# fzi-forschungszentrum-informatik/muvo

Hardware: AMD Instinct MI355X
Metric: world-model training samples/sec (seq_len=10) (higher is better)
Workload: dtype f32 storage/accumulate; large contractions (convolutions, transformer Linear) as bf16x3 split products

## Files before the change

include/muvo_hip.h:

```cpp
#ifndef MUVO_HIP_H
#define MUVO_HIP_H
#include <stdint.h>

#ifdef __cplusplus
extern "C" {
#endif

#define MUVO_OK 0
#define MUVO_ERR_INVALID_ARG (-1)
#define MUVO_ERR_HIP (-2)

#define MUVO_ACT_NONE 0
#define MUVO_ACT_RELU 1
#define MUVO_ACT_LEAKY 2
#define MUVO_ACT_ELU 3
#define MUVO_ACT_TANH 4
#define MUVO_ACT_SIGMOID 5

const char* muvo_last_error(void);
int muvo_abi_version(void);
int muvo_selftest_mfma(void* stream);
int muvo_set_deterministic(int on);
int muvo_reset_accumulators(void);
int muvo_get_deterministic(void);

typedef struct muvo_conv_desc {
  int32_t nd;
  int32_t transposed;
  int32_t N, Cin, Cout;
  int32_t in_sz[3], out_sz[3];
  int32_t ksz[3], stride[3], pad[3], dil[3];
} muvo_conv_desc;

#define MUVO_CONV_F32 0
#define MUVO_CONV_BF16X3 1
#define MUVO_CONV_MODE_DEFAULT MUVO_CONV_BF16X3
int muvo_conv_set_products(int n);
int muvo_conv_get_products(void);
int muvo_conv_set_mode(int mode);
int muvo_conv_get_mode(void);
int muvo_conv_set_bf16x3_min_gflop(double gflop_per_item);
int muvo_linear_bf16x3_pack_floats(int in_f, int out_f, int64_t* fwd_floats, int64_t* dgrad_floats);
int muvo_linear_bf16x3_pack(int in_f, int out_f, const float* w, float* wp_fwd, float* wp_dgrad, void* stream);
int64_t muvo_linear_bf16x3_workspace_bytes(int64_t rows, int features);
int muvo_linear_bf16x3_split(const float* x, int64_t rows, int features, void* ws, void* stream);
int muvo_linear_bf16x3_forward(int64_t rows, int in_f, int out_f, const void* ws_x, const float* wp_fwd, const float* bias,
                               float* y, int act, float slope, void* stream);
int muvo_linear_bf16x3_dgrad(int64_t rows, int in_f, int out_f, const void* ws_dz, const float* wp_dgrad, float* dx,
                             void* stream);
int muvo_linear_bf16x3_wgrad(int64_t rows, int in_f, int out_f, const void* ws_x, const void* ws_dz, float* scratch,
                             float* dw, void* stream);
int64_t muvo_pack_table_item_bytes(void);
int muvo_conv_pack_table_add(void* host_items, int capacity, int* n_items, int64_t* n_blocks, const muvo_conv_desc* d,
                             const float* w, float* wp_fwd, float* wp_dgrad);
int muvo_linear_bf16x3_pack_table_add(void* host_items, int capacity, int* n_items, int64_t* n_blocks, int in_f, int out_f,
                                      const float* w, float* wp_fwd, float* wp_dgrad);
int muvo_pack_table_run(const void* dev_items, int n_items, int64_t n_blocks, void* stream);
int muvo_conv_pack_sizes(const muvo_conv_desc* d, int64_t* fwd_floats, int64_t* dgrad_floats);
int muvo_conv_pack_weights(const muvo_conv_desc* d, const float* w, float* wp_fwd, float* wp_dgrad, void* stream);
int64_t muvo_conv_workspace_bytes(const muvo_conv_desc* d, int op);
int muvo_conv_kernel_family(const muvo_conv_desc* d, int op);
int muvo_conv_kernel_variant(const muvo_conv_desc* d, int op);
int muvo_conv_forward(const muvo_conv_desc* d, const float* x, const float* wp_fwd, const float* bias, float* y, int act,
                      float slope, void* ws, void* stream);
int muvo_conv_dgrad(const muvo_conv_desc* d, const float* dy, const float* wp_dgrad, float* dx, void* ws, int ws_valid,
                    void* stream);
int muvo_conv_forward_head_supported(const muvo_conv_desc* d, int CO);
int muvo_conv_forward_head(const muvo_conv_desc* d, const float* x, const float* wp_fwd, const float* bias, float* y, int act,
                           float slope, void* ws, const float* head_w, const float* head_b, int CO, float* logits, void* stream);
int muvo_conv_forward_moments_supported(const muvo_conv_desc* d);
int muvo_conv_forward_moments(const muvo_conv_desc* d, const float* x, const float* wp_fwd, const float* bias, float* y, int act,
                              float slope, double* moments, void* stream);
int muvo_adain_fwd_moments(const float* x, const float* style, float* y, float* save_mean, float* save_rstd, double* moments,
                           int N, int C, int64_t S, float eps, void* stream);
int muvo_adain_affine(const float* style, double* moments, float* save_mean, float* save_rstd, float* aff, int N, int C, int64_t S,
                      float eps, void* stream);
int muvo_conv_affine_supported(const muvo_conv_desc* d);
int muvo_conv_forward_affine(const muvo_conv_desc* d, const float* x, const float* aff, const float* wp_fwd, const float* bias,
                             float* y, int act, float slope, double* moments, void* stream);
int muvo_conv_wgrad_affine(const muvo_conv_desc* d, const float* x, const float* aff, const float* dy, float* dw, float* dbias,
                           void* stream);
int muvo_grouped_linear_fwd(const float* x, int M, int K, int L, const float* const* W, const float* const* b, float* const* Y,
                            const int* N, void* stream);
int muvo_grouped_linear_bwd(const float* x, int M, int K, int L, const float* const* W, float* const* dY, float* dx,
                            float* const* dW, float* const* db, const int* N, void* stream);
int muvo_bf3_loop_clock(double* shader_mhz, double* us_per_k_step);
int muvo_adain_head_supported(int C, int CO, int64_t S);
int muvo_adain_head_fwd(const float* x, const float* style, float* save_mean, float* save_rstd, double* moments, const float* head_w,
                        const float* head_b, float* logits, int N, int C, int CO, int64_t S, float eps, void* stream);
int muvo_adain_head_bwd(const float* x, const float* style, const float* save_mean, const float* save_rstd, const float* head_w,
                        const float* dlogits, float* dx, float* dstyle, float* dhead_w, float* dhead_b, double* ws, int N, int C,
                        int CO, int64_t S, int act, float slope, void* stream);
int muvo_conv_dgrad_accumulate(const muvo_conv_desc* d, const float* dy, const float* wp_dgrad, float* dx, void* stream);
int muvo_conv_prepare_dy(const muvo_conv_desc* d, const float* y, const float* dy, int act, float slope, void* ws_dy,
                         float* dbias, void* stream);
int muvo_conv_prepare_dy_head_supported(const muvo_conv_desc* d, int CO);
int muvo_conv_prepare_dy_head(const muvo_conv_desc* d, const float* y, const float* dy, const float* dhead, const float* head_w,
                              int CO, int act, float slope, void* ws_dy, float* dbias, float* dhead_w, float* dhead_b, void* stream);
int64_t muvo_split_planes_bytes(int N, int C, int64_t S);
int muvo_split_planes(const float* x, void* ws, int N, int C, int64_t S, const float* y, int act, float slope, float* dbias,
                      void* stream);
int muvo_conv_wgrad(const muvo_conv_desc* d, const float* x, const float* dy, float* dwp_scratch, float* dw, float* dbias,
                    void* ws_x, void* ws_dy, int flags, void* stream);

int muvo_bias_grad_nchw(const float* dy, float* db, int N, int M, int64_t S, void* stream);

typedef struct muvo_gemm_desc {
  int32_t M, N, K;
  int64_t sam, sak, sbk, sbn, scm;
  int32_t B1, B2;
  int64_t a_b1, a_b2, b_b1, b_b2, c_b1, c_b2;
  float alpha;
  int32_t bias_div;
  int32_t act;
  float slope;
  int32_t mode;
} muvo_gemm_desc;
int muvo_gemm(const muvo_gemm_desc* d, const float* A, const float* B, float* C, const float* bias, void* stream);

int muvo_bn_train_fwd(const float* x, const float* gamma, const float* beta, const float* residual, float* y,
                      float* save_mean, float* save_rstd, float* running_mean, float* running_var, double* ws, int N, int C,
                      int64_t S, float eps, float momentum, int res_mode, int relu, void* stream);
int muvo_bn_train_bwd(const float* x, const float* y, const float* dy, const float* gamma, const float* beta,
                      const float* save_mean, const float* save_rstd, float* dx, float* dres, float* dgamma, float* dbeta,
                      double* ws, int N, int C, int64_t S, int mask_mode, void* stream);
int muvo_adain_fwd(const float* x, const float* style, float* y, float* save_mean, float* save_rstd, double* ws, int N,
                   int C, int64_t S, int64_t x_batch_stride, float eps, void* stream);
int muvo_adain_bwd(const float* x, const float* style, const float* dy, const float* save_mean, const float* save_rstd,
                   float* dx, float* dstyle, double* ws, int N, int C, int64_t S, int64_t x_batch_stride, int act,
                   float slope, void* stream);
int muvo_add_dropout_layernorm_fwd(const float* x, const float* a, const float* gamma, const float* beta, float* y,
                                   float* z, float* mean, float* rstd, int rows, int E, float eps, float p, uint64_t seed,
                                   void* stream);
int muvo_add_dropout_layernorm_bwd(const float* dy, const float* z, const float* mean, const float* rstd,
                                   const float* gamma, float* dx, float* da, float* dgamma, float* dbeta, int rows, int E,
                                   float p, uint64_t seed, void* stream);

int muvo_act_fwd(const float* x, float* y, int64_t n, int act, float slope, void* stream);
int muvo_act_bwd(const float* y, const float* dy, float* dx, int64_t n, int act, float slope, void* stream);
int muvo_dropout(const float* x, float* y, int64_t n, float p, uint64_t seed, void* stream);
int muvo_axpby(const float* a, const float* b, float* out, int64_t n, float alpha, float beta, void* stream);
int muvo_copy2d(const float* src, float* dst, int64_t rows, int64_t cols, int64_t ld_src, int64_t ld_dst, int accumulate,
                void* stream);
int muvo_colsum_acc(const float* x, float* out, int64_t rows, int64_t cols, int64_t ld, void* stream);
int muvo_batchsum(const float* x, float* out, int N, int64_t inner, int accumulate, void* stream);
int muvo_nchw_to_tokens(const float* x, const float* pos, const float* temb, int temb_stride, float* tokens, int N, int C,
                        int L, int l0, void* stream);
int muvo_tokens_to_nchw(const float* tokens, float* x, int N, int C, int L, int l0, void* stream);
int muvo_maxpool2d_fwd(const float* x, float* y, uint8_t* idx, int64_t NC, int H, int W, int OH, int OW, int k, int s, int p,
                       void* stream);
int muvo_maxpool2d_bwd(const float* dy, const uint8_t* idx, float* dx, int64_t NC, int H, int W, int OH, int OW, int k, int s,
                       int p, void* stream);
int muvo_avgpool_fwd(const float* x, float* y, int64_t G, int64_t S, void* stream);
int muvo_avgpool_bwd(const float* dy, float* dx, int64_t G, int64_t S, void* stream);
int muvo_upsample3d_x2_fwd(const float* x, float* y, int64_t NC, int D, int H, int W, void* stream);
int muvo_upsample3d_x2_bwd(const float* dy, float* dx, int64_t NC, int D, int H, int W, void* stream);
int muvo_preprocess_image(const uint8_t* img, float* label, float* norm, int64_t NC, int C, int H, int W, int top, int left,
                          int CH, int CW, const float* mean3, const float* std3, void* stream);
int muvo_preprocess_route(const uint8_t* img, float* norm, int64_t NC, int C, int H, int W, int OH, int OW,
                          const float* mean3, const float* std3, void* stream);
int muvo_attention_supported(int L, int DH);
int muvo_attention_fwd(const float* qkv, float* out, float* lse, int L, int N, int H, int DH, float p, uint64_t seed,
                       void* stream);
int muvo_attention_bwd(const float* qkv, const float* out, const float* dout, const float* lse, float* dqkv, int L, int N, int H,
                       int DH, float p, uint64_t seed, void* stream);
int muvo_attention_stream_supported(int L, int DH);
int muvo_attention_stream_blocks(int* bq, int* bk);
int muvo_attention_stream_fwd(const float* qkv, float* out, float* lse, int L, int N, int H, int DH, float p, uint64_t seed,
                              void* stream);
int muvo_attention_stream_bwd(const float* qkv, const float* out, const float* dout, const float* lse, float* dqkv, float* dws,
                              int L, int N, int H, int DH, float p, uint64_t seed, void* stream);
int muvo_rssm_supported(int B, int T, int H, int S, int E, int A, int AD);
int64_t muvo_rssm_transposed_floats(int H, int S, int E, int A);
int64_t muvo_rssm_scratch_floats(int B, int H, int S, int E, int A);
int muvo_rssm_forward(int B, int T, int H, int S, int E, int A, int AD, const float* const* weights, const float* emb,
                      const float* act, const float* noise, uint64_t use_prior_mask, float* const* out7, float* const* keep12,
                      uint32_t* barrier_word, float min_std, void* stream);
int muvo_rssm_backward(int B, int T, int H, int S, int E, int A, int AD, const float* const* weights, float* wt_scratch,
                       const float* noise, uint64_t use_prior_mask, const float* const* kept5, const float* const* upstream7,
                       float* const* grads10, float* scratch, uint32_t* barrier_word, void* stream);
#define MUVO_PIXAUG_STRIDE 16
#define MUVO_ROUTEAUG_STRIDE 8
int muvo_pixel_augment(float* img, float* norm, float* tmp, const float* params, double* gray_sum, int64_t frames, int H, int W,
                       const float* mean3, const float* std3, void* stream);
int muvo_preprocess_route_aug(const uint8_t* img, float* out, const float* params, int B, int S, int C, int H, int W, int OH,
                              int OW, const float* mean3, const float* std3, void* stream);
int muvo_divide_scalar(const float* x, float* y, int64_t n, float divisor, void* stream);
int muvo_resize_bilinear(const float* x, float* y, int64_t NC, int H, int W, int OH, int OW, void* stream);
int muvo_resize_nearest_f32(const float* x, float* y, int64_t NC, int D, int H, int W, int OD, int OH, int OW, void* stream);
int muvo_resize_nearest_u8(const uint8_t* x, uint8_t* y, int64_t NC, int D, int H, int W, int OD, int OH, int OW,
                           void* stream);
int muvo_softmax_dropout_fwd(const float* S, float* P, float* Pd, int64_t rows, int cols, float p, uint64_t seed, void* stream);
int muvo_softmax_dropout_bwd(const float* P, const float* dPd, float* dS, int64_t rows, int cols, float p, uint64_t seed,
                             void* stream);
int muvo_gru_fwd(const float* gi, const float* gh, const float* h, float* hnew, int B, int H, void* stream);
int muvo_gru_bwd(const float* gi, const float* gh, const float* h, const float* dhnew, float* dgi, float* dgh, float* dh,
                 int B, int H, void* stream);
int muvo_rssm_sample_fwd(const float* mu_logsigma, const float* eps, int64_t eps_ld, float* mu, float* sigma, float* sample,
                         int B, int S, float min_std, void* stream);
int muvo_rssm_sample_bwd(const float* mu_logsigma, const float* eps, int64_t eps_ld, const float* dmu, const float* dsigma,
                         const float* dsample, float* dmls, int B, int S, void* stream);

int muvo_spatial_loss_fwd(const float* pred, const float* target, int64_t F, int Ct, int64_t HW, int c0, int c1, int norm,
                          float ignore, float weight, double* stats2, float* loss, void* stream);
int muvo_spatial_loss_bwd(const float* pred, const float* target, float* dpred, int64_t F, int Ct, int64_t HW, int c0, int c1,
                          int norm, float ignore, float weight, const double* stats2, const float* gout, void* stream);
int muvo_spatial_loss_masked_fwd(const float* pred, const float* target, const uint8_t* mask, int64_t F, int Ct, int64_t HW, int c0,
                                 int c1, int norm, float ignore, float weight, double* stats2, float* loss, void* stream);
int muvo_spatial_loss_masked_bwd(const float* pred, const float* target, const uint8_t* mask, float* dpred, int64_t F, int Ct,
                                 int64_t HW, int c0, int c1, int norm, float ignore, float weight, const double* stats2,
                                 const float* gout, void* stream);
int muvo_voxel_loss_stats_doubles(int C);
int muvo_voxel_loss_coef_floats(int C);
int muvo_voxel_loss_fwd(const float* logits, const uint8_t* target, int64_t F, int C, int64_t V, const float* class_w,
                        float weight, double* stats, float* coef, float* loss3, void* stream);
int muvo_voxel_loss_bwd(const float* logits, const uint8_t* target, float* dlogits, int64_t F, int C, int64_t V,
                        const float* class_w, float weight, const float* coef, const float* gout3, void* stream);
int muvo_seg_ce_fwd(const float* logits, const uint8_t* target, const float* class_w, float* loss, int64_t N, int C, int64_t HW,
                    void* stream);
int muvo_seg_ce_bwd(const float* logits, const uint8_t* target, const float* class_w, const float* gloss, float* dlogits, int64_t N,
                    int C, int64_t HW, void* stream);
int muvo_l1_rows_fwd(const float* p, const float* t, int64_t rows, int cols, float weight, float* loss, void* stream);
int muvo_l1_rows_bwd(const float* p, const float* t, float* dp, int64_t rows, int cols, float weight, const float* gout,
                     void* stream);
int muvo_kl_loss_fwd(const float* prior_mu, const float* prior_sigma, const float* post_mu, const float* post_sigma, int B,
                     int T, int S, float weight, float* loss, void* stream);
int muvo_kl_loss_bwd(const float* prior_mu, const float* prior_sigma, const float* post_mu, const float* post_sigma,
                     float* d_prior_mu, float* d_prior_sigma, float* d_post_mu, float* d_post_sigma, int B, int T, int S,
                     float weight, float alpha, const float* gout, void* stream);
int muvo_adamw_step(float* p, const float* g, float* m, float* v, int64_t n, float lr, float beta1, float beta2, float eps,
                    float weight_decay, int step, float grad_scale, void* stream);

int64_t muvo_chamfer_loss_ws_doubles(int64_t F, int64_t n);
int muvo_chamfer_loss_fwd(const float* pred, const float* target, int64_t F, int Cp, int Ct, int64_t n, float weight, double* ws,
                          int32_t* idx_pt, int32_t* idx_tp, float* loss, void* stream);
int muvo_chamfer_loss_bwd(const float* pred, const float* target, const int32_t* idx_pt, const int32_t* idx_tp, float* dpred, int64_t F,
                          int Cp, int Ct, int64_t n, float weight, const float* gout, void* stream);

int muvo_ssim_frames(const float* pred, const float* target, const float* window, double* sums, int N, int C, int H, int W,
// ... 149 lines not shown
```

muvo_amd/csrc/conv_gemm.hip:

```cpp
#include "common.h"
#include "conv_vox.h"
#include "conv_pw.h"
#include "conv_plan.h"
#include "conv_bf3.h"

typedef __bf16 wg_bf16x8 __attribute__((ext_vector_type(8)));
__device__ __forceinline__ void wg_split8(const float (&v)[8], wg_bf16x8& hi, wg_bf16x8& lo) {
  typedef __bf16 b2 __attribute__((ext_vector_type(2)));
  typedef float f2 __attribute__((ext_vector_type(2)));
  unsigned h[4], l[4];
#pragma unroll
  for (int p = 0; p < 4; ++p) {
    const b2 hh = __builtin_convertvector((f2){v[2 * p], v[2 * p + 1]}, b2);
    h[p] = __builtin_bit_cast(unsigned, hh);
    const float h0 = __uint_as_float(h[p] << 16), h1 = __uint_as_float(h[p] & 0xffff0000u);
    const b2 ll = __builtin_convertvector((f2){v[2 * p] - h0, v[2 * p + 1] - h1}, b2);
    l[p] = __builtin_bit_cast(unsigned, ll);
  }
  typedef unsigned u4 __attribute__((ext_vector_type(4)));
  hi = __builtin_bit_cast(wg_bf16x8, (u4){h[0], h[1], h[2], h[3]});
  lo = __builtin_bit_cast(wg_bf16x8, (u4){l[0], l[1], l[2], l[3]});
}

template <int BM, int BN, int WM, int WN, int RUN>
// ... 894 lines not shown
  if (rc) return rc;
  MUVO_CHECK_ARG(wp_fwd && y && ws, "conv_forward_planes: null pointer");
  MUVO_CHECK_ARG(!pw_applicable(d) && !vox_fwd_ok(d), "conv_forward_planes: this shape does not read split planes");
  bool all_bf3 = pl.nfwd > 0;
  for (int i = 0; i < pl.nfwd; ++i) all_bf3 = all_bf3 && pl.fwd[i].bf3;
  MUVO_CHECK_ARG(all_bf3, "conv_forward_planes: ws_valid needs every phase on the bf16x3 kernels (muvo_conv_kernel_family == 1)");
  return run_phases(pl.fwd, pl.nfwd, x, wp_fwd, bias, y, act, slope, ws, (hipStream_t)stream, true);
}

int muvo_conv_forward_head_supported(const muvo_conv_desc* d, int CO) {
  if (check_desc(d) || CO < 1 || CO > 4) return 0;
  static const int on = getenv("MUVO_CONV_HEAD_FWD") ? atoi(getenv("MUVO_CONV_HEAD_FWD")) : 1;
  if (!on || muvo_det() || conv_mode() != 1 || pw_applicable(d) || vox_fwd_ok(d)) return 0;
  ConvPlan pl;
  if (build_plan(d, &pl) != MUVO_OK || pl.nfwd < 1) return 0;
  for (int i = 0; i < pl.nfwd; ++i) {
    const ConvPhase& g = pl.fwd[i];
    if (!g.bf3 || !bf3_fwd_uses_pp(g) || phase_ksplit(g) > 1) return 0;
    if (g.Msub != d->Cout || g.Msub % 64 != 0 || g.M % 64 != 0 || (long)CO * g.Msub > 1024) return 0;
    if ((long)g.N * g.out_sN * 4 >= 0x7fffff00L) return 0;
  }
  return 1;
}
int muvo_conv_forward_head(const muvo_conv_desc* d, const float* x, const float* wp_fwd, const float* bias, float* y, int act,
                           float slope, void* ws, const float* head_w, const float* head_b, int CO, float* logits, void* stream) {
  ConvPlan pl;
  int rc = build_plan(d, &pl);
  if (rc) return rc;
  MUVO_CHECK_ARG(x && wp_fwd && y && head_w && logits, "conv_forward_head: null pointer");
  MUVO_CHECK_ARG(muvo_conv_forward_head_supported(d, CO), "conv_forward_head: shape not served by the eight-wave bf16x3 tiles");
  hipStream_t st = (hipStream_t)stream;
  if (d->Cout > 64) {
    const long S_out = (long)d->out_sz[0] * d->out_sz[1] * d->out_sz[2];
    if (hipMemsetAsync(logits, 0, sizeof(float) * (size_t)d->N * CO * S_out, st) != hipSuccess) {
      muvo_set_error("conv_forward_head: memset of the logits failed");
      return MUVO_ERR_HIP;
    }
  }
  bf3_set_fused_head(head_w, head_b, logits, CO);
  rc = run_phases(pl.fwd, pl.nfwd, x, wp_fwd, bias, y, act, slope, ws, st);
  bf3_set_fused_head(nullptr, nullptr, nullptr, 0);
  return rc;
}

int muvo_conv_forward_moments_supported(const muvo_conv_desc* d) {
  if (check_desc(d)) return 0;
  if (muvo_det()) return 0;
  return (!pw_applicable(d) && vox_fwd_ok(d) && vox_uses_bf3(d, 0)) ? 1 : 0;
}
int muvo_conv_forward_moments(const muvo_conv_desc* d, const float* x, const float* wp_fwd, const float* bias, float* y, int act,
                              float slope, double* moments, void* stream) {
  ConvPlan pl;
  int rc = build_plan(d, &pl);
  if (rc) return rc;
  MUVO_CHECK_ARG(x && wp_fwd && y && moments, "conv_forward_moments: null pointer");
  MUVO_CHECK_ARG(muvo_conv_forward_moments_supported(d), "conv_forward_moments: only the bf16x3 voxel kernels produce output moments");
  return vox_forward(d, x, wp_fwd, bias, y, act, slope, (hipStream_t)stream, true, moments);
}

int muvo_conv_affine_supported(const muvo_conv_desc* d) {
  if (check_desc(d)) return 0;
  return (conv_mode() == 1 && !pw_applicable(d) && vox_fwd_ok(d) && vox_uses_bf3(d, 0) && vox_wgrad_applicable(d) &&
          vox_wgrad_uses_bf3(d) && vox_affine_ok(d)) ? 1 : 0;
}
int muvo_conv_forward_affine(const muvo_conv_desc* d, const float* x, const float* aff, const float* wp_fwd, const float* bias,
                             float* y, int act, float slope, double* moments, void* stream) {
  ConvPlan pl;
  int rc = build_plan(d, &pl);
  if (rc) return rc;
  MUVO_CHECK_ARG(x && aff && wp_fwd && y, "conv_forward_affine: null pointer");
  MUVO_CHECK_ARG(muvo_conv_affine_supported(d), "conv_forward_affine: shape not served by the bf16x3 voxel kernels");
  return vox_forward(d, x, wp_fwd, bias, y, act, slope, (hipStream_t)stream, true, moments, aff);
}
int muvo_conv_wgrad_affine(const muvo_conv_desc* d, const float* x, const float* aff, const float* dy, float* dw, float* dbias,
                           void* stream) {
  ConvPlan pl;
  int rc = build_plan(d, &pl, 0, false);
  if (rc) return rc;
  MUVO_CHECK_ARG(x && aff && dy && dw, "conv_wgrad_affine: null pointer");
  MUVO_CHECK_ARG(muvo_conv_affine_supported(d), "conv_wgrad_affine: shape not served by the bf16x3 voxel kernels");
  return vox_wgrad(d, x, dy, dw, dbias, (hipStream_t)stream, true, aff);
}

int muvo_conv_dgrad(const muvo_conv_desc* d, const float* dy, const float* wp_dgrad, float* dx, void* ws, int ws_valid,
                    void* stream) {
  ConvPlan pl;
  int rc = build_plan(d, &pl);
  if (rc) return rc;
  MUVO_CHECK_ARG(dy && wp_dgrad && dx, "conv_dgrad: null pointer");
  if (pw_applicable(d)) return pw_dgrad(d, dy, wp_dgrad, dx, (hipStream_t)stream);
  if (vox_dgrad_ok(d)) return vox_dgrad(d, dy, wp_dgrad, dx, (hipStream_t)stream, vox_uses_bf3(d, 1));
  return run_phases(pl.dgr, pl.ndgr, dy, wp_dgrad, nullptr, dx, MUVO_ACT_NONE, 0.f, ws, (hipStream_t)stream, ws_valid != 0);
}

int muvo_conv_dgrad_accumulate(const muvo_conv_desc* d, const float* dy, const float* wp_dgrad, float* dx, void* stream) {
  int rc = check_desc(d);
  if (rc) return rc;
  MUVO_CHECK_ARG(dy && wp_dgrad && dx, "conv_dgrad_accumulate: null pointer");
  MUVO_CHECK_ARG(pw_applicable(d), "conv_dgrad_accumulate: only the 1x1 head kernels (muvo_conv_kernel_family == 3) accumulate");
  return pw_dgrad_acc(d, dy, wp_dgrad, dx, (hipStream_t)stream);
}

int muvo_conv_prepare_dy(const muvo_conv_desc* d, const float* y, const float* dy, int act, float slope, void* ws_dy,
                         float* dbias, void* stream) {
  int rc = check_desc(d);
  if (rc) return rc;
  MUVO_CHECK_ARG(dy && ws_dy && (y || act == MUVO_ACT_NONE), "conv_prepare_dy: null pointer");
  const long S_out = (long)d->out_sz[0] * d->out_sz[1] * d->out_sz[2];
  return bf3_split_input(dy, ws_dy, d->N, d->Cout, S_out, (hipStream_t)stream, act == MUVO_ACT_NONE ? nullptr : y, act, slope,
                         dbias);
}

int muvo_conv_prepare_dy_head(const muvo_conv_desc* d, const float* y, const float* dy, const float* dhead, const float* head_w,
                              int CO, int act, float slope, void* ws_dy, float* dbias, float* dhead_w, float* dhead_b, void* stream) {
  int rc = check_desc(d);
  if (rc) return rc;
  MUVO_CHECK_ARG(dhead && head_w && ws_dy && CO >= 1 && CO <= 4 && (y || act == MUVO_ACT_NONE), "conv_prepare_dy_head: bad args");
  const long S_out = (long)d->out_sz[0] * d->out_sz[1] * d->out_sz[2];
  MUVO_CHECK_ARG(dhead_w == nullptr || (y != nullptr && act != MUVO_ACT_NONE),
                 "conv_prepare_dy_head: the fused head weight gradient needs the activation output y");
  return bf3_split_input(dy, ws_dy, d->N, d->Cout, S_out, (hipStream_t)stream, act == MUVO_ACT_NONE ? nullptr : y, act, slope,
                         dbias, dhead, head_w, CO, dhead_w, dhead_b);
}
int muvo_conv_prepare_dy_head_supported(const muvo_conv_desc* d, int CO) {
  if (check_desc(d)) return 0;
  const long S_out = (long)d->out_sz[0] * d->out_sz[1] * d->out_sz[2];
  return CO >= 1 && CO <= 4 && S_out % 4 == 0 && S_out >= 1024;
}

static double bf3_wgrad_min_gflop() {
  static const char* e = getenv("MUVO_BF16X3_WGRAD_MIN_GFLOP");
  static const double env_v = e ? atof(e) : -1.0;
  if (env_v >= 0.0) return env_v;
  if (bf3_default_policy()) return 0.05;
  return bf3_min_gflop() < 0.5 ? bf3_min_gflop() : 0.5;
}

static const int g_bf3_wgrad_min_m = getenv("MUVO_BF3_WGRAD_MIN_M") ? atoi(getenv("MUVO_BF3_WGRAD_MIN_M")) : 32;
static bool wgrad_uses_bf3(const ConvPlan& pf) {
  if (conv_mode() != 1) return false;
  const bool dflt = bf3_default_policy() && !getenv("MUVO_BF16X3_WGRAD_MIN_GFLOP");
  double total = 0.0;
  int taps = 0;
  for (int i = 0; i < pf.nfwd; ++i) {
    const ConvPhase& g = pf.fwd[i];
    const double gflop = 2.0 * g.Msub * g.T * g.C * (double)g.SD * g.SH * g.SW * 1e-9;
    if (g.Msub < g_bf3_wgrad_min_m || g.C < 32 || g.Msub % 16 != 0 && g.nmerge > 1) return false;
    static const int allow32 = getenv("MUVO_BF3_WGRAD_32X32") ? atoi(getenv("MUVO_BF3_WGRAD_32X32")) : 1;
    if (g.Msub <= 32 && g.C < 64 && !allow32) return false;
    if (!dflt && gflop < bf3_wgrad_min_gflop()) return false;
    total += gflop * g.nmerge;
    taps += g.T * g.nmerge;
  }
  if (dflt && (total < bf3_wgrad_min_gflop() || taps <= 1)) return false;
  return pf.nfwd > 0;
}

int muvo_conv_wgrad(const muvo_conv_desc* d, const float* x, const float* dy, float* dwp_scratch, float* dw, float* dbias,
                    void* ws_x, void* ws_dy, int flags, void* stream) {
  ConvPlan pl;
  int rc = build_plan(d, &pl, 0, false);
  if (rc) return rc;
  MUVO_CHECK_ARG(x && dy && dwp_scratch && dw, "conv_wgrad: null pointer");
  hipStream_t st = (hipStream_t)stream;
  if (pw_applicable(d)) return pw_wgrad(d, x, dy, dw, dbias, st);
  if (vox_wgrad_ok(d)) return vox_wgrad(d, x, dy, dw, dbias, st, vox_wgrad_uses_bf3(d));
// ... 202 lines not shown
```

muvo_amd/csrc/conv_vox.h:

```cpp
#pragma once
#include "common.h"

bool vox_fwd_applicable(const muvo_conv_desc* d);
bool vox_dgrad_applicable(const muvo_conv_desc* d);
bool vox_wgrad_applicable(const muvo_conv_desc* d);
long vox_pack_floats(const muvo_conv_desc* d);
bool vox_bf3_shape_ok(const muvo_conv_desc* d, int dgrad);
int vox_pack(const muvo_conv_desc* d, const float* w, float* wp, int dgrad, hipStream_t st, bool bf3);
int vox_forward(const muvo_conv_desc* d, const float* x, const float* wp, const float* bias, float* y, int act, float slope,
                hipStream_t st, bool bf3, double* moments = nullptr, const float* aff = nullptr);
bool vox_affine_ok(const muvo_conv_desc* d);
int vox_dgrad(const muvo_conv_desc* d, const float* dy, const float* wp, float* dx, hipStream_t st, bool bf3);
bool vox_bf3_wgrad_shape_ok(const muvo_conv_desc* d);
bool vox_wgrad_ps_only(const muvo_conv_desc* d);
int vox_wgrad(const muvo_conv_desc* d, const float* x, const float* dz, float* dw, float* dbias, hipStream_t st, bool bf3,
              const float* aff = nullptr);
```

muvo_amd/csrc/conv_vox.hip:

```cpp
#include "common.h"
#include "conv_vox.h"
#include <type_traits>

struct VoxArgs {
  int N, Cin, Cout, X, Y;
  int ytiles, xgroups;
  int XYZ;
  long sN_in, sN_out;
  double* moments;
  int xcd_order;
  const float* aff;
  unsigned* ticket;
};
static int vox_xcd_order() {
  static const int v = getenv("MUVO_VOX_XCD") ? atoi(getenv("MUVO_VOX_XCD")) : 1;
  return v;
}

__device__ __forceinline__ float dpp_wave_shr1(float v) {
  return __int_as_float(__builtin_amdgcn_update_dpp(0, __float_as_int(v), 0x138, 0xf, 0xf, true));
}
__device__ __forceinline__ float dpp_wave_shl1(float v) {
  return __int_as_float(__builtin_amdgcn_update_dpp(0, __float_as_int(v), 0x130, 0xf, 0xf, true));
}

template <int CQ, int TY, int Z>
__global__ void __launch_bounds__(256)
vox_conv_kernel(const VoxArgs a, const float* __restrict__ in, const float* __restrict__ wp,
                const float* __restrict__ bias, float* __restrict__ out, int act, float slope) {
  extern __shared__ __attribute__((aligned(16))) float s_w[];
  constexpr int SUB = 64 / Z;
  constexpr int R = TY + 2;
  const int tid = threadIdx.x, lane = tid & 63, wave = tid >> 6;
  {
    const int nw4 = 27 * a.Cin * a.Cout / 4;
    for (int i = tid; i < nw4; i += 256) ((float4*)s_w)[i] = ((const float4*)wp)[i];
  }
  __syncthreads();
  const long wid = (long)blockIdx.x * 4 + wave;
  const long nwaves = (long)a.N * a.xgroups * a.ytiles;
  if (wid >= nwaves) return;
  const int yt = (int)(wid % a.ytiles);
  const long t0 = wid / a.ytiles;
  const int xg = (int)(t0 % a.xgroups), n = (int)(t0 / a.xgroups);
  const int sub = lane / Z, z = lane % Z;
  const int x = xg * SUB + sub;
  const int y0 = yt * TY;
  const bool xok = x < a.X;
  const int YZ = a.Y * Z;
  const float* inn = in + (size_t)n * a.sN_in;

  f32x4 acc[TY][CQ];
#pragma unroll
  for (int g = 0; g < TY; ++g)
#pragma unroll
    for (int q = 0; q < CQ; ++q) acc[g][q] = (f32x4){0.f, 0.f, 0.f, 0.f};

  auto load_rows = [&](int it, float* v) {
    const int ci = it / 3, tx = it - 3 * ci;
    const int xin = x + tx - 1;
    const bool ok = xok && (unsigned)xin < (unsigned)a.X;
    const float* p = inn + (size_t)ci * a.XYZ;
    const int off = xin * YZ + z;
#pragma unroll
    for (int r = 0; r < R; ++r) {
      const int y = y0 - 1 + r;
      float val = 0.f;
      if (ok && (unsigned)y < (unsigned)a.Y) val = p[off + y * Z];
      v[r] = val;
    }
  };

  const int total = 3 * a.Cin;
  const int wl = (lane & 3) * CQ;
  const int wstride = a.Cin * 4 * CQ;
  float cur[R], nxt[R];
  load_rows(0, cur);
  for (int it = 0; it < total; ++it) {
    const int ci = it / 3, tx = it - 3 * ci;
    if (it + 1 < total) load_rows(it + 1, nxt);
    float lf[R], rt[R];
#pragma unroll
    for (int r = 0; r < R; ++r) {
      const float l = dpp_wave_shr1(cur[r]), rr = dpp_wave_shl1(cur[r]);
      lf[r] = z > 0 ? l : 0.f;
      rt[r] = z < Z - 1 ? rr : 0.f;
    }
    const float* wb = s_w + (size_t)(tx * 9 * a.Cin + ci) * 4 * CQ + wl;
#pragma unroll
    for (int ty = 0; ty < 3; ++ty) {
#pragma unroll
      for (int tz = 0; tz < 3; ++tz) {
        const float* wq = wb + (ty * 3 + tz) * wstride;
        float w[CQ];
        if constexpr (CQ == 2) {
          const float2 t = *(const float2*)wq;
// ... 328 lines not shown
  float msum[4] = {0.f, 0.f, 0.f, 0.f}, msq[4] = {0.f, 0.f, 0.f, 0.f};
  float bv[4];
#pragma unroll
  for (int i = 0; i < 4; ++i) bv[i] = (bias != nullptr && co0 + 4 * g + i < a.Cout) ? bias[co0 + 4 * g + i] : 0.f;
  const __amdgpu_buffer_rsrc_t rs_out = __builtin_amdgcn_make_buffer_rsrc((void*)(out + (long)n * a.sN_out), 0,
                                                                          (int)((long)a.Cout * a.XYZ * 4), 0x00020000);

  int fdx[NSTEP], foff[NSTEP];
#pragma unroll
  for (int s = 0; s < NSTEP; ++s) {
    int tap = s * TPS + g;
    if (tap > 26) tap = 26;
    const int dx = tap / 9 - 1, dy = (tap / 3) % 3 - 1, dz = tap % 3 - 1;
    fdx[s] = dx;
    foff[s] = (wave + 1 + dy) * COLS + (v + 1 + dz);
  }

  stage_load(xs - 1); stage_store((xs - 1 + 3) % 3);
  stage_load(xs); stage_store(xs % 3);
  stage_load(xs + 1);
  vox_dummy_stores<4 * ZT>(rs_out);
  __syncthreads();
  for (int x = xs; x < xe; ++x) {
    stage_store((x + 1) % 3);
    __syncthreads();
    if (x + 1 < xe) stage_load(x + 2);
    const vu32x4* P[3] = {vsm + ((x - 1 + 3) % 3) * PLANE, vsm + (x % 3) * PLANE, vsm + ((x + 1) % 3) * PLANE};
    const vu32x4* fb[NSTEP];
#pragma unroll
    for (int s = 0; s < NSTEP; ++s) fb[s] = (fdx[s] < 0 ? P[0] : (fdx[s] == 0 ? P[1] : P[2])) + foff[s];
    const int gy = y0 + wave;
#pragma unroll
    for (int zt = 0; zt < ZT; ++zt) {
      vf32x4 acc = {0.f, 0.f, 0.f, 0.f};
#pragma unroll
      for (int s = 0; s < NSTEP; ++s) {
        const vbf16x8 bh = __builtin_bit_cast(vbf16x8, fb[s][zt * 16]);
        const vbf16x8 bl = __builtin_bit_cast(vbf16x8, fb[s][zt * 16 + CG * ROWS * COLS]);
        acc = __builtin_amdgcn_mfma_f32_16x16x32_bf16(wl[s], bh, acc, 0, 0, 0);
        acc = __builtin_amdgcn_mfma_f32_16x16x32_bf16(wh[s], bl, acc, 0, 0, 0);
        acc = __builtin_amdgcn_mfma_f32_16x16x32_bf16(wh[s], bh, acc, 0, 0, 0);
      }
      const unsigned ooff = (unsigned)(((long)x * YZ + (long)gy * Z + zt * 16 + v) * 4);
#pragma unroll
      for (int i = 0; i < 4; ++i) {
        const int co = co0 + 4 * g + i;
        const bool ok = gy < a.Y && co < a.Cout;
        const unsigned off = ok ? ooff + (unsigned)co * xyz4 : 0x7fffff00u;
        float r = acc[i] + bv[i];
        if constexpr (GENERIC) {
          if (accum) r += __uint_as_float(__builtin_amdgcn_raw_buffer_load_b32(rs_out, off, 0, 0));
          r = act_apply(r, act, slope);
        } else {
          r = vox_act_simple(r, act, slope);
        }
        __builtin_amdgcn_raw_buffer_store_b32(__float_as_uint(r), rs_out, off, 0, 0);
        r = ok ? r : 0.f;
        msum[i] += r;
        msq[i] += r * r;
      }
    }
    __syncthreads();
  }
  if (a.moments) {
#pragma unroll
    for (int i = 0; i < 4; ++i)
#pragma unroll
      for (int o = 1; o < 16; o <<= 1) { msum[i] += __shfl_xor(msum[i], o, 64); msq[i] += __shfl_xor(msq[i], o, 64); }
    float* red = (float*)vsm;
    if (v == 0)
#pragma unroll
      for (int i = 0; i < 4; ++i) { red[((wave * 4 + g) * 4 + i) * 2] = msum[i]; red[((wave * 4 + g) * 4 + i) * 2 + 1] = msq[i]; }
    __syncthreads();
    if (tid < 32) {
      const int c = tid >> 1, k = tid & 1;
      double t = 0.0;
      for (int w = 0; w < TY; ++w) t += (double)red[((w * 4 + (c >> 2)) * 4 + (c & 3)) * 2 + k];
      if (co0 + c < a.Cout) atomicAdd(&a.moments[((long)n * a.Cout + co0 + c) * 2 + k], t);
    }
  }
}

constexpr int VOX_PS_TY = 8;
template <int Z, int TY, bool CO8, bool GENERIC>
__global__ void __launch_bounds__(64 * TY, 1)
vox_bf3_ps_kernel(const VoxArgs a, const float* __restrict__ in, const vu32x4* __restrict__ wp, const float* __restrict__ bias,
                  float* __restrict__ out, int act, float slope, int xseg, int accum) {
  static_assert(TY == VOX_PS_TY, "one workgroup of eight waves per CU");
  constexpr int CK = 16, CG = 2, PSTEPS = 5, ZT = Z / 16, NF = CO8 ? 2 * PSTEPS : 3 * PSTEPS, NACC = CO8 ? 2 : 3;
  constexpr int ROWS = TY + 2, COLS = Z + 2;
  constexpr int PLANE = 2 * CG * ROWS * COLS;
  constexpr int NTASK = CG * ROWS * Z, TPT = (NTASK + 64 * TY - 1) / (64 * TY);
  extern __shared__ vu32x4 vsm[];
  const int tid = threadIdx.x, lane = tid & 63, wave = tid >> 6;
  const int nseg = (a.X + xseg - 1) / xseg;
  int bid = a.xcd_order ? xcd_swizzle(blockIdx.x, gridDim.x) : (int)blockIdx.x;
  const int seg = bid % nseg; bid /= nseg;
  const int ytile = bid % a.ytiles, n = bid / a.ytiles;
  const int y0 = ytile * TY, xs = seg * xseg, xe = xs + xseg < a.X ? xs + xseg : a.X;
  const long YZ = (long)a.Y * Z;
  const float* inb = in + (long)n * a.sN_in;
  const int co0 = blockIdx.y * 16;

  vbf16x8 wh[NF], wl[NF];
  const vu32x4* wpb = wp + (size_t)blockIdx.y * NF * 2 * 64;
#pragma unroll
  for (int f = 0; f < NF; ++f) {
    wh[f] = __builtin_bit_cast(vbf16x8, wpb[(f * 2) * 64 + lane]);
    wl[f] = __builtin_bit_cast(vbf16x8, wpb[(f * 2 + 1) * 64 + lane]);
  }
  for (int i = tid; i < 2 * PLANE; i += 64 * TY) vsm[i] = vu32x4{0u, 0u, 0u, 0u};
  __syncthreads();

  float stg[TPT][8];
  unsigned stg_ok = 0u;
  __shared__ float s_aff[2 * CK];
  if (a.aff) {
    if (tid < 2 * CK) s_aff[tid] = a.aff[(long)n * a.Cin * 2 + tid];
    __syncthreads();
  }
  const __amdgpu_buffer_rsrc_t rs_in = __builtin_amdgcn_make_buffer_rsrc((void*)inb, 0, (int)((long)CK * a.XYZ * 4), 0x00020000);
  const unsigned xyz4 = (unsigned)a.XYZ * 4u;
  auto stage_load_task = [&](int k, int x) {
    const int t = tid + k * 64 * TY;
    const int z = t % Z, r = (t / Z) % ROWS, cg = t / (Z * ROWS);
    const int gy = y0 - 1 + r;
    const bool ok = t < NTASK && x >= 0 && x < a.X && gy >= 0 && gy < a.Y;
    stg_ok = (stg_ok & ~(1u << k)) | ((unsigned)ok << k);
    const unsigned off = ok ? (unsigned)(((long)(cg * 8) * a.XYZ + (long)x * YZ + (long)gy * Z + z) * 4) : 0x7fffff00u;
#pragma unroll
    for (int e = 0; e < 8; ++e)
      stg[k][e] = __uint_as_float(__builtin_amdgcn_raw_buffer_load_b32(rs_in, off + (unsigned)e * xyz4, 0, 0));
  };
  auto stage_load = [&](int x) {
#pragma unroll
    for (int k = 0; k < TPT; ++k) stage_load_task(k, x);
  };
  auto stage_store_task = [&](int k, int slot) {
    vu32x4* P = vsm + slot * PLANE;
    {
      const int t = tid + k * 64 * TY;
      if (t >= NTASK) return;
      const int z = t % Z, r = (t / Z) % ROWS, cg = t / (Z * ROWS);
      if (a.aff) {
        const bool ok = (stg_ok >> k) & 1u;
#pragma unroll
        for (int e = 0; e < 8; ++e) {
          const float sc = s_aff[(cg * 8 + e) * 2], sh = s_aff[(cg * 8 + e) * 2 + 1];
          stg[k][e] = ok ? stg[k][e] * sc + sh : 0.f;
        }
      }
      unsigned h[4], l[4];
#pragma unroll
      for (int q = 0; q < 4; ++q) vox_split2(stg[k][2 * q], stg[k][2 * q + 1], h[q], l[q]);
      P[(cg * ROWS + r) * COLS + z + 1] = vu32x4{h[0], h[1], h[2], h[3]};
      P[((CG + cg) * ROWS + r) * COLS + z + 1] = vu32x4{l[0], l[1], l[2], l[3]};
    }
  };
  auto stage_store = [&](int slot) {
#pragma unroll
    for (int k = 0; k < TPT; ++k) stage_store_task(k, slot);
  };

  const int v = lane & 15, g = lane >> 4;
  float msum[4] = {0.f, 0.f, 0.f, 0.f}, msq[4] = {0.f, 0.f, 0.f, 0.f};
  float bv[4];
#pragma unroll
  for (int i = 0; i < 4; ++i) bv[i] = (bias != nullptr && co0 + 4 * g + i < a.Cout) ? bias[co0 + 4 * g + i] : 0.f;
  const __amdgpu_buffer_rsrc_t rs_out = __builtin_amdgcn_make_buffer_rsrc((void*)(out + (long)n * a.sN_out), 0,
                                                                          (int)((long)a.Cout * a.XYZ * 4), 0x00020000);
  int foff[PSTEPS];
#pragma unroll
  for (int s = 0; s < PSTEPS; ++s) {
    int tp = s * 2 + (g >> 1);
    if (tp > 8) tp = 8;
    const int dy = tp / 3 - 1, dz = tp % 3 - 1;
    foff[s] = ((g & 1) * ROWS + (wave + 1 + dy)) * COLS + (v + 1 + dz);
  }
  vf32x4 acc[NACC][ZT];
#pragma unroll
  for (int j = 0; j < NACC; ++j)
#pragma unroll
    for (int zt = 0; zt < ZT; ++zt) acc[j][zt] = vf32x4{0.f, 0.f, 0.f, 0.f};

  stage_load(xs - 1); stage_store((xs - 1) & 1);
  stage_load(xs);
  vox_dummy_stores<4 * ZT>(rs_out);
  __syncthreads();
  const int gy = y0 + wave;
  for (int p = xs - 1; p <= xe; ++p) {
    constexpr bool ACC_PRE = GENERIC && (CO8 || Z <= 32);
    float accv[ZT][4];
    if constexpr (ACC_PRE) {
      if (accum) {
        const int xo = p - 1;
        const bool xok = xo >= xs && xo < xe;
#pragma unroll
        for (int zt = 0; zt < ZT; ++zt) {
          const unsigned ooff = (unsigned)(((long)xo * YZ + (long)gy * Z + zt * 16 + v) * 4);
#pragma unroll
          for (int i = 0; i < 4; ++i) {
            const int co = co0 + 4 * g + i;
            const bool ok = xok && gy < a.Y && co < a.Cout && (!CO8 || g < 2);
            accv[zt][i] = __uint_as_float(__builtin_amdgcn_raw_buffer_load_b32(rs_out, ok ? ooff + (unsigned)co * xyz4 : 0x7fffff00u, 0, 0));
          }
        }
      }
    }
    constexpr bool PIPE = CO8 || Z <= 32;
    if constexpr (!PIPE) {
      stage_store((p + 1) & 1);
      if (p + 2 <= xe) stage_load(p + 2);
    }
    const vu32x4* P = vsm + (p & 1) * PLANE;
#pragma unroll
    for (int zt = 0; zt < ZT; ++zt) {
#pragma unroll
      for (int s = 0; s < PSTEPS; ++s) {
        const vbf16x8 bh = __builtin_bit_cast(vbf16x8, P[foff[s] + zt * 16]);
        const vbf16x8 bl = __builtin_bit_cast(vbf16x8, P[foff[s] + zt * 16 + CG * ROWS * COLS]);
        if constexpr (CO8) {
          acc[1][zt] = __builtin_amdgcn_mfma_f32_16x16x32_bf16(wl[s], bh, acc[1][zt], 0, 0, 0);
          acc[1][zt] = __builtin_amdgcn_mfma_f32_16x16x32_bf16(wh[s], bl, acc[1][zt], 0, 0, 0);
          acc[1][zt] = __builtin_amdgcn_mfma_f32_16x16x32_bf16(wh[s], bh, acc[1][zt], 0, 0, 0);
          acc[0][zt] = __builtin_amdgcn_mfma_f32_16x16x32_bf16(wl[PSTEPS + s], bh, acc[0][zt], 0, 0, 0);
          acc[0][zt] = __builtin_amdgcn_mfma_f32_16x16x32_bf16(wh[PSTEPS + s], bl, acc[0][zt], 0, 0, 0);
          acc[0][zt] = __builtin_amdgcn_mfma_f32_16x16x32_bf16(wh[PSTEPS + s], bh, acc[0][zt], 0, 0, 0);
        } else {
#pragma unroll
          for (int dxi = 0; dxi < 3; ++dxi) {
            const int f = dxi * PSTEPS + s, j = 2 - dxi;
            acc[j][zt] = __builtin_amdgcn_mfma_f32_16x16x32_bf16(wl[f], bh, acc[j][zt], 0, 0, 0);
            acc[j][zt] = __builtin_amdgcn_mfma_f32_16x16x32_bf16(wh[f], bl, acc[j][zt], 0, 0, 0);
            acc[j][zt] = __builtin_amdgcn_mfma_f32_16x16x32_bf16(wh[f], bh, acc[j][zt], 0, 0, 0);
          }
        }
      }
      if constexpr (PIPE) {
#pragma unroll
        for (int k = 0; k < TPT; ++k)
          if ((k < ZT ? k : ZT - 1) == zt) {
            stage_store_task(k, (p + 1) & 1);
            if (p + 2 <= xe) stage_load_task(k, p + 2);
          }
        __builtin_amdgcn_sched_barrier(0);
      }
    }
    const int xo = p - 1;
    const bool xok = xo >= xs && xo < xe;
#pragma unroll
    for (int zt = 0; zt < ZT; ++zt) {
      const unsigned ooff = (unsigned)(((long)xo * YZ + (long)gy * Z + zt * 16 + v) * 4);
#pragma unroll
      for (int i = 0; i < 4; ++i) {
        const int co = co0 + 4 * g + i;
        const bool ok = xok && gy < a.Y && co < a.Cout && (!CO8 || g < 2);
        const unsigned off = ok ? ooff + (unsigned)co * xyz4 : 0x7fffff00u;
        float r = acc[0][zt][i] + bv[i];
        if constexpr (GENERIC) {
          if constexpr (ACC_PRE) { if (accum) r += accv[zt][i]; }
          else if (accum) r += __uint_as_float(__builtin_amdgcn_raw_buffer_load_b32(rs_out, off, 0, 0));
          r = act_apply(r, act, slope);
        } else {
          r = vox_act_simple(r, act, slope);
        }
        __builtin_amdgcn_raw_buffer_store_b32(__float_as_uint(r), rs_out, off, 0, 0);
        r = ok ? r : 0.f;
        msum[i] += r;
// ... 157 lines not shown
  const int row = wave / ZH, z0 = (wave % ZH) * 32;
  const int j = lane & 15, kg = lane >> 4;
  const int a_off = j * DCO + row * DROW + (z0 + kg * 8) * 2;
  const int b_off = (j & (CI - 1)) * XCI + 16 + (z0 + kg * 8) * 2;
  const int sel = j >> 3;

  xload(xs - 1); xstore((xs - 1 + 4) & 3);
  xload(xs); xstore(xs & 3);
  xload(xs + 1); xstore((xs + 1) & 3);
  dload(xs); dstore(xs & 1);
  xload(xs + 2);
  dload(xs + 1);
  __syncthreads();
  for (int px = xs; px < xe; ++px) {
    const char* A = dzb + (px & 1) * DBUF + a_off;
    const vbf16x8 ah = __builtin_bit_cast(vbf16x8, *(const vu32x4*)A);
    const vbf16x8 al = __builtin_bit_cast(vbf16x8, *(const vu32x4*)(A + DHL));
#pragma unroll
    for (int cb = 0; cb < NCOMB; ++cb) {
      int c = 2 * cb + sel;
      if (c > 8) c = 8;
      const int dx = c / 3, dy = c - 3 * dx;
      const char* R = xring + ((px + dx - 1 + 4) & 3) * XSLOT + b_off + (row + dy) * XROW;
      vu32x4 w[2];
      unsigned pw[2], nw[2];
#pragma unroll
      for (int hl = 0; hl < 2; ++hl) {
        w[hl] = *(const vu32x4*)(R + hl * XHL);
        pw[hl] = *(const unsigned*)(R + hl * XHL - 4);
        nw[hl] = *(const unsigned*)(R + hl * XHL + 16);
      }
      vbf16x8 bm[2], bz[2], bp[2];
#pragma unroll
      for (int hl = 0; hl < 2; ++hl) {
        const vu32x4 q = w[hl];
        bz[hl] = __builtin_bit_cast(vbf16x8, q);
        const vu32x4 m = {__builtin_amdgcn_alignbyte(q.x, pw[hl], 2), __builtin_amdgcn_alignbyte(q.y, q.x, 2),
                          __builtin_amdgcn_alignbyte(q.z, q.y, 2), __builtin_amdgcn_alignbyte(q.w, q.z, 2)};
        bm[hl] = __builtin_bit_cast(vbf16x8, m);
        const vu32x4 pl = {__builtin_amdgcn_alignbyte(q.y, q.x, 2), __builtin_amdgcn_alignbyte(q.z, q.y, 2),
                           __builtin_amdgcn_alignbyte(q.w, q.z, 2), __builtin_amdgcn_alignbyte(nw[hl], q.w, 2)};
        bp[hl] = __builtin_bit_cast(vbf16x8, pl);
      }
      const int t0 = cb * TPC;
      acc[t0] = __builtin_amdgcn_mfma_f32_16x16x32_bf16(al, bm[0], acc[t0], 0, 0, 0);
      acc[t0] = __builtin_amdgcn_mfma_f32_16x16x32_bf16(ah, bm[1], acc[t0], 0, 0, 0);
      acc[t0] = __builtin_amdgcn_mfma_f32_16x16x32_bf16(ah, bm[0], acc[t0], 0, 0, 0);
      acc[t0 + 1] = __builtin_amdgcn_mfma_f32_16x16x32_bf16(al, bz[0], acc[t0 + 1], 0, 0, 0);
      acc[t0 + 1] = __builtin_amdgcn_mfma_f32_16x16x32_bf16(ah, bz[1], acc[t0 + 1], 0, 0, 0);
      acc[t0 + 1] = __builtin_amdgcn_mfma_f32_16x16x32_bf16(ah, bz[0], acc[t0 + 1], 0, 0, 0);
      acc[t0 + 2] = __builtin_amdgcn_mfma_f32_16x16x32_bf16(al, bp[0], acc[t0 + 2], 0, 0, 0);
      acc[t0 + 2] = __builtin_amdgcn_mfma_f32_16x16x32_bf16(ah, bp[1], acc[t0 + 2], 0, 0, 0);
      acc[t0 + 2] = __builtin_amdgcn_mfma_f32_16x16x32_bf16(ah, bp[0], acc[t0 + 2], 0, 0, 0);
      static_assert(XPT + DPT + 1 <= NCOMB, "one staging piece per combination");
      if (cb < XPT) xstore_task(cb, (px + 2) & 3);
      else if (cb < XPT + DPT) dstore_task(cb - XPT, (px + 1) & 1);
      else if (cb == XPT + DPT) { xload(px + 3); dload(px + 2); }
      __builtin_amdgcn_sched_barrier(0);
    }
    __syncthreads();
  }
  float* red = (float*)wsm;
  for (int i = tid; i < NT * 256; i += 512) red[i] = 0.f;
  __syncthreads();
#pragma unroll
  for (int t = 0; t < NT; ++t)
#pragma unroll
    for (int r = 0; r < 4; ++r) atomicAdd(red + (t * 16 + 4 * kg + r) * 16 + j, acc[t][r]);
  __syncthreads();
  for (int i = tid; i < NT * 256; i += 512) {
    const int col = i & 15, t = i >> 8;
    const int co = (i >> 4) & 15;
    const int tz = t % TPC;
    const int comb = 2 * (t / TPC) + (col >> 3);
    const int ci = col & 7;
    const int tap = comb <= 8 && tz >= 0 ? comb * 3 + tz : -1;
    const float vsum = red[i];
    if (tap >= 0 && co < a.Cout && ci0 + ci < a.Cin && vsum != 0.f) atomicAdd(dw + ((long)co * a.Cin + ci0 + ci) * 27 + tap, vsum);
  }
  if (blockIdx.y == 0 && dbias && tid < a.Cout) atomicAdd(dbias + tid, dbsum[tid]);
}

constexpr int VOX_WGPS_SW = 4;
template <int Z, int CI, bool CO8, int SW = 0>
__global__ void __launch_bounds__(512 + 64 * SW)
vox_bf3_wgrad_ps_kernel(const VoxArgs a, const float* __restrict__ x, const float* __restrict__ dz, float* __restrict__ dw,
                        float* __restrict__ dbias, int xseg) {
  static_assert(CI == 16 || CO8, "8 input channels: the quadrant tiles hold 8 produced channels");
  constexpr bool QUAD = CI == 8;
  constexpr int ZH = Z >= 32 ? Z / 32 : 1, RW = Z >= 32 ? 1 : 32 / Z, WROWS = 8 / ZH * RW, ROWS = WROWS + 2;
  constexpr int XROW = (Z + 16) * 2;
  constexpr int XCI = ROWS * XROW + 16;
  constexpr int XHL = CI * XCI, XSLOT = 2 * XHL;
  constexpr int NTH = 512 + 64 * SW, NS = SW > 0 ? 64 * SW : 512;
  constexpr int XT = CI * ROWS * (Z / 8), XPT = (XT + NS - 1) / NS;
  constexpr int TPC = QUAD ? 1 : (CO8 ? 2 : 3), NT = 9 * TPC;
  static_assert(SW > 0 || XPT <= 2, "staging pieces: one per dy group, then the loads");
  static_assert(2 * XSLOT >= NT * 1024, "the reduction reuses the x planes");
  extern __shared__ char wsm[];
  char* xring = wsm;
  float* dbsum = (float*)(wsm + 2 * XSLOT);
  const int tid = threadIdx.x, lane = tid & 63, wave = tid >> 6;
  const bool stager = SW > 0 && wave >= 8;
  const int stid = SW > 0 ? tid - 512 : tid;
  const int nseg = (a.X + xseg - 1) / xseg;
  int bid = a.xcd_order ? xcd_swizzle(blockIdx.x, gridDim.x) : (int)blockIdx.x;
  const int seg = bid % nseg; bid /= nseg;
  const int ytile = bid % a.ytiles, n = bid / a.ytiles;
  const int y0 = ytile * WROWS, xs = seg * xseg, xe = xs + xseg < a.X ? xs + xseg : a.X;
  const int ci0 = blockIdx.y * CI;
  const long YZ = (long)a.Y * Z;
  const float* xb = x + (long)n * a.sN_in + (long)ci0 * a.XYZ;
  const int co_base = blockIdx.z * 16;
  const float* db = dz + (long)n * a.sN_out;
  for (int i = tid; i < (2 * XSLOT + 64) / 16; i += NTH) ((uint4*)wsm)[i] = uint4{0u, 0u, 0u, 0u};
  __syncthreads();

  constexpr unsigned OOB = 0x7fffff00u;
  const int nci = a.Cin - ci0 < CI ? a.Cin - ci0 : CI;
  const __amdgpu_buffer_rsrc_t rs_x = __builtin_amdgcn_make_buffer_rsrc((void*)xb, 0, (int)((long)nci * a.XYZ * 4), 0x00020000);
  const __amdgpu_buffer_rsrc_t rs_d = __builtin_amdgcn_make_buffer_rsrc((void*)db, 0, (int)((long)a.Cout * a.XYZ * 4), 0x00020000);
  vu32x4 xraw[XPT][2];
  unsigned xok = 0u;
  float xas[XPT], xab[XPT];
  int xlds[XPT];
  long xg[XPT];
  bool xrow_ok[XPT];
#pragma unroll
  for (int k = 0; k < XPT; ++k) {
    const int t = stid >= 0 ? stid + k * NS : XT;
    const int z8 = t % (Z / 8), rr = (t / (Z / 8)) % ROWS, ci = t / ((Z / 8) * ROWS);
    const int gy = y0 - 1 + rr;
    const bool have = a.aff != nullptr && t < XT && ci0 + ci < a.Cin;
    xas[k] = have ? a.aff[((long)n * a.Cin + ci0 + ci) * 2] : 1.f;
    xab[k] = have ? a.aff[((long)n * a.Cin + ci0 + ci) * 2 + 1] : 0.f;
    xlds[k] = t < XT ? ci * XCI + rr * XROW + 16 + z8 * 16 : -1;
    xrow_ok[k] = t < XT && gy >= 0 && gy < a.Y;
    xg[k] = (long)ci * a.XYZ + (long)gy * Z + z8 * 8;
  }
  auto xload_task = [&](int k, int px) {
    const bool ok = xrow_ok[k] && px >= 0 && px < a.X;
    xok = (xok & ~(1u << k)) | ((unsigned)ok << k);
    const unsigned off = ok ? (unsigned)((xg[k] + (long)px * YZ) * 4) : OOB;
    xraw[k][0] = __builtin_amdgcn_raw_buffer_load_b128(rs_x, off, 0, 0);
    xraw[k][1] = __builtin_amdgcn_raw_buffer_load_b128(rs_x, off + 16u, 0, 0);
  };
  auto xload = [&](int px) {
#pragma unroll
    for (int k = 0; k < XPT; ++k) xload_task(k, px);
  };
  auto split8 = [&](const float (&v)[8], vu32x4& h, vu32x4& l) {
    unsigned hh[4], ll[4];
#pragma unroll
    for (int q = 0; q < 4; ++q) vox_split2(v[2 * q], v[2 * q + 1], hh[q], ll[q]);
    h = vu32x4{hh[0], hh[1], hh[2], hh[3]};
    l = vu32x4{ll[0], ll[1], ll[2], ll[3]};
  };
  auto xstore_task = [&](int k, int slot) {
    if (xlds[k] < 0) return;
    float v[8] = {__uint_as_float(xraw[k][0].x), __uint_as_float(xraw[k][0].y), __uint_as_float(xraw[k][0].z), __uint_as_float(xraw[k][0].w),
                  __uint_as_float(xraw[k][1].x), __uint_as_float(xraw[k][1].y), __uint_as_float(xraw[k][1].z), __uint_as_float(xraw[k][1].w)};
    if (a.aff) {
      const bool ok = (xok >> k) & 1u;
#pragma unroll
      for (int e = 0; e < 8; ++e) v[e] = ok ? v[e] * xas[k] + xab[k] : 0.f;
    }
    vu32x4 h, l;
    split8(v, h, l);
    char* dst = xring + slot * XSLOT + xlds[k];
    *(vu32x4*)dst = h;
    *(vu32x4*)(dst + XHL) = l;
  };

  const int j = lane & 15, kg = lane >> 4;
  const int row = (wave / ZH) * RW + (Z >= 32 ? 0 : kg / (Z / 8));
  const int zl = Z >= 32 ? (wave % ZH) * 32 + kg * 8 : (kg % (Z / 8)) * 8;
  const int aco = co_base + (CO8 ? (j & 7) : j);
  const bool a_shift = CO8 && j >= 8;
  const bool a_last = zl + 8 >= Z;
  const bool a_ok = y0 + row < a.Y && aco < a.Cout;
  const long a_g = (long)aco * a.XYZ + (long)(y0 + row) * Z + zl;
  vu32x4 araw[2];
  unsigned anext = 0u;
  auto aload = [&](int px) {
    const bool ok = a_ok && px >= xs && px < xe;
    const unsigned off = ok ? (unsigned)((a_g + (long)px * YZ) * 4) : OOB;
    araw[0] = __builtin_amdgcn_raw_buffer_load_b128(rs_d, off, 0, 0);
    araw[1] = __builtin_amdgcn_raw_buffer_load_b128(rs_d, off + 16u, 0, 0);
    if constexpr (CO8) anext = __builtin_amdgcn_raw_buffer_load_b32(rs_d, ok && !a_last ? off + 32u : OOB, 0, 0);
  };
  float dbacc = 0.f;
  auto asplit = [&](vu32x4& h, vu32x4& l) {
    float v[8] = {__uint_as_float(araw[0].x), __uint_as_float(araw[0].y), __uint_as_float(araw[0].z), __uint_as_float(araw[0].w),
                  __uint_as_float(araw[1].x), __uint_as_float(araw[1].y), __uint_as_float(araw[1].z), __uint_as_float(araw[1].w)};
    dbacc += ((v[0] + v[1]) + (v[2] + v[3])) + ((v[4] + v[5]) + (v[6] + v[7]));
    if constexpr (CO8) {
      const float nx = __uint_as_float(anext);
#pragma unroll
      for (int e = 0; e < 7; ++e) v[e] = a_shift ? v[e + 1] : v[e];
      v[7] = a_shift ? nx : v[7];
    }
    split8(v, h, l);
  };

  vf32x4 acc[NT];
#pragma unroll
  for (int t = 0; t < NT; ++t) acc[t] = vf32x4{0.f, 0.f, 0.f, 0.f};
  const int b_off = (j & (CI - 1)) * XCI + 16 + zl * 2;
  const bool b_shift = QUAD && j >= 8;
  vu32x4 Ah[3] = {}, Al[3] = {};

  const int niter = xe - xs + 2;
  if (stager) {
    xload(xs - 1);
#pragma unroll
    for (int k = 0; k < XPT; ++k) xstore_task(k, 0);
    xload(xs);
    __syncthreads();
    for (int it = 0; it < niter; ++it) {
      if (it + 1 < niter) {
#pragma unroll
        for (int k = 0; k < XPT; ++k) xstore_task(k, (it + 1) & 1);
        if (it + 2 < niter) xload(xs + 1 + it);
      }
      __syncthreads();
    }
  } else {
  if (SW == 0) {
    xload(xs - 1);
#pragma unroll
    for (int k = 0; k < XPT; ++k) xstore_task(k, 0);
    xload(xs);
  }
  aload(xs);
  __syncthreads();
  for (int it = 0; it < niter; ++it) {
    const int P = xs - 1 + it;
    Ah[2] = Ah[1]; Al[2] = Al[1]; Ah[1] = Ah[0]; Al[1] = Al[0];
    asplit(Ah[0], Al[0]);
    aload(P + 2);
    const bool xin = P >= 0 && P < a.X;
    const bool dok[3] = {it < niter - 2, it >= 1 && it < niter - 1, it >= 2};
    const char* S = xring + (it & 1) * XSLOT + b_off + row * XROW;
#pragma unroll
    for (int dy = 0; dy < 3; ++dy) {
      if (xin) {
        const char* R = S + dy * XROW;
        vbf16x8 bm[2], bz[2], bp[2];
// ... 302 lines not shown
      else { dxi = 2; live = live && (lane & 15) < 8; }
    } else {
      dxi = f / 5;
    }
    const int tap = dxi * 9 + tp;
    float val = 0.f;
    if (live && m < rows) val = dgrad ? w[((size_t)c * Cin + m) * 27 + (26 - tap)] : w[((size_t)m * Cin + c) * 27 + tap];
    unsigned hu, lu;
    vox_split_rne(val, hu, lu);
    wp[((size_t)(((half * nrb + rb) * NF + f) * 2) * 64 + lane) * 8 + e] = (unsigned short)hu;
    wp[((size_t)(((half * nrb + rb) * NF + f) * 2 + 1) * 64 + lane) * 8 + e] = (unsigned short)lu;
  }
}

static bool vox_geometry_ok(const muvo_conv_desc* d, bool z16 = false) {
  if (d->nd != 3 || d->transposed) return false;
  for (int a = 0; a < 3; ++a)
    if (d->ksz[a] != 3 || d->stride[a] != 1 || d->pad[a] != 1 || d->dil[a] != 1) return false;
  const int Z = d->in_sz[2];
  if (Z != 64 && Z != 32 && !(z16 && Z == 16)) return false;
  if (d->Cin % 4 || d->Cout % 4) return false;
  if ((long)d->in_sz[0] * d->in_sz[1] * Z * (long)(d->Cin > d->Cout ? d->Cin : d->Cout) * 4 >= 0x7fffff00l) return false;
  return true;
}
bool vox_fwd_applicable(const muvo_conv_desc* d) {
  return vox_geometry_ok(d) && (d->Cout == 8 || d->Cout == 16) && 27l * d->Cin * d->Cout * 4 <= 64 * 1024;
}
bool vox_dgrad_applicable(const muvo_conv_desc* d) {
  return vox_geometry_ok(d) && (d->Cin == 8 || d->Cin == 16) && 27l * d->Cin * d->Cout * 4 <= 64 * 1024;
}
bool vox_wgrad_applicable(const muvo_conv_desc* d) {
  return vox_geometry_ok(d) && d->Cout % 8 == 0 && d->Cin % 8 == 0 && d->Cout <= 32 && d->Cin <= 64;
}
static bool vox_bf3_two_rows(int ck, int cp) { return cp == 8 && ck == 8; }
static bool vox_bf3_ps(int red, int cp) { return (red == 16 || red == 32 || red == 64) && (cp == 8 || cp == 16 || cp == 32); }
bool vox_bf3_shape_ok(const muvo_conv_desc* d, int dgrad) {
  const int ck = dgrad ? d->Cout : d->Cin, cp = dgrad ? d->Cin : d->Cout;
  if (vox_geometry_ok(d, true) && (d->in_sz[2] == 16 || ck == 64)) return vox_bf3_ps(ck, cp);
  if (!vox_geometry_ok(d)) return false;
  return (ck == 8 || ck == 16 || ck == 32) && (cp == 8 || cp == 16 || cp == 32);
}
constexpr int VOX_BF3_STEPS = 7;
long vox_pack_floats(const muvo_conv_desc* d) {
  const int blocks_f = (d->Cin / 16 > 0 ? d->Cin / 16 : 1) * cdiv(d->Cout, 16), blocks_d = (d->Cout / 16 > 0 ? d->Cout / 16 : 1) * cdiv(d->Cin, 16);
  const int blocks = blocks_f > blocks_d ? blocks_f : blocks_d;
  const long plain = 27l * d->Cin * d->Cout, bf3 = 15l * 2 * 64 * 4 * (blocks > 4 ? blocks : 4);
  return plain > bf3 ? plain : bf3;
}

int vox_pack(const muvo_conv_desc* d, const float* w, float* wp, int dgrad, hipStream_t st, bool bf3) {
  const int red = dgrad ? d->Cout : d->Cin, cp = dgrad ? d->Cin : d->Cout;
  if (bf3 && vox_bf3_ps(red, cp)) {
    const int co8 = cp <= 8 ? 1 : 0;
    hipLaunchKernelGGL(vox_bf3_ps_pack_kernel, dim3(cdiv((red / 16) * cdiv(cp, 16) * (co8 ? 10 : 15) * 512, 256)), dim3(256), 0, st, w,
                       (unsigned short*)wp, d->Cin, d->Cout, dgrad, co8);
    MUVO_CHECK_LAUNCH("vox_bf3_ps_pack_kernel");
    return MUVO_OK;
  }
  if (bf3 && vox_bf3_two_rows(red, cp)) {
    hipLaunchKernelGGL(vox_bf3_pack2_kernel, dim3(36), dim3(256), 0, st, w, (unsigned short*)wp, d->Cin, d->Cout, dgrad);
    MUVO_CHECK_LAUNCH("vox_bf3_pack2_kernel");
    return MUVO_OK;
  }
  if (bf3) {
    MUVO_CHECK_ARG(red == 8, "vox_pack: no bf16x3 voxel kernel for %d reduction / %d produced channels", red, cp);
    hipLaunchKernelGGL(vox_bf3_pack_kernel, dim3(cdiv(cdiv(cp, 16) * VOX_BF3_STEPS * 512, 256)), dim3(256), 0, st, w, (unsigned short*)wp,
                       d->Cin, d->Cout, dgrad, 8, VOX_BF3_STEPS);
    MUVO_CHECK_LAUNCH("vox_bf3_pack_kernel");
    return MUVO_OK;
  }
  const int total = 27 * d->Cin * d->Cout;
  hipLaunchKernelGGL(vox_pack_kernel, dim3(cdiv(total, 256)), dim3(256), 0, st, w, wp, d->Cin, d->Cout, dgrad);
  MUVO_CHECK_LAUNCH("vox_pack_kernel");
  return MUVO_OK;
}

static VoxArgs vox_args(const muvo_conv_desc* d, int Cin, int Cout, int rows, int Z, int cin_total, const float* aff) {
  VoxArgs a{};
  a.xcd_order = vox_xcd_order();
  a.aff = aff;
  a.N = d->N; a.Cin = Cin; a.Cout = Cout; a.X = d->in_sz[0]; a.Y = d->in_sz[1];
  a.ytiles = cdiv(a.Y, rows);
  a.XYZ = a.X * a.Y * Z;
  a.sN_in = (long)(cin_total ? cin_total : Cin) * a.XYZ; a.sN_out = (long)Cout * a.XYZ;
  return a;
}

static int vox_blocks_target(int wgrad) {
  static const int f = getenv("MUVO_VOX_BLOCKS") ? atoi(getenv("MUVO_VOX_BLOCKS")) : 128;
  static const int w = getenv("MUVO_VOX_WGRAD_BLOCKS") ? atoi(getenv("MUVO_VOX_WGRAD_BLOCKS")) : 128;
  return wgrad ? w : f;
}
static int vox_xseg(const VoxArgs& a, int factor, int wgrad) {
  int xseg = a.X;
  while ((long)a.N * a.ytiles * cdiv(a.X, xseg) * factor < vox_blocks_target(wgrad) && xseg > 12) xseg = cdiv(xseg, 2);
  return xseg;
}

template <class... K>
static int vox_raise_lds(bool& done, const char* what, size_t lds, K... kernels) {
  if (done) return MUVO_OK;
  if (((hipFuncSetAttribute((const void*)kernels, hipFuncAttributeMaxDynamicSharedMemorySize, (int)lds) != hipSuccess) || ...)) {
    muvo_set_error("%s: cannot raise the dynamic LDS limit to %zu bytes", what, lds);
    return MUVO_ERR_HIP;
  }
  done = true;
  return MUVO_OK;
}

template <bool Z16 = false, class F>
static int vox_with_z(int Z, F&& f) {
  if (Z == 64) return f(std::integral_constant<int, 64>{});
  if (Z == 32) return f(std::integral_constant<int, 32>{});
  if constexpr (Z16) {
    if (Z == 16) return f(std::integral_constant<int, 16>{});
  }
  muvo_set_error("vox_conv: no kernel for z lines of %d voxels", Z);
  return MUVO_ERR_INVALID_ARG;
}
template <class F>
static int vox_with_bool(bool b, F&& f) { return b ? f(std::true_type{}) : f(std::false_type{}); }

template <int CQ, int TY, int Z>
static int launch_vox_conv(const muvo_conv_desc* d, int Cin, int Cout, const float* in, const float* wp, const float* bias,
                           float* out, int act, float slope, hipStream_t st) {
  VoxArgs a = vox_args(d, Cin, Cout, TY, Z, 0, nullptr);
  a.xgroups = cdiv(a.X, 64 / Z);
  const long nwaves = (long)a.N * a.xgroups * a.ytiles;
  const size_t lds = (size_t)27 * Cin * Cout * sizeof(float);
  hipLaunchKernelGGL((vox_conv_kernel<CQ, TY, Z>), dim3(cdiv(nwaves, 4)), dim3(256), lds, st, a, in, wp, bias, out, act, slope);
  MUVO_CHECK_LAUNCH("vox_conv_kernel");
  return MUVO_OK;
}

template <int Z>
static int launch_vox_bf3(const muvo_conv_desc* d, int Cout, const float* in, const float* wp, const float* bias, float* out, int act,
                          float slope, hipStream_t st, double* moments, const float* aff) {
  constexpr int CK = 8, TY = 8;
  VoxArgs a = vox_args(d, CK, Cout, TY, Z, 0, aff);
  a.moments = moments;
  const int xseg = vox_xseg(a, 1, 0);
  constexpr size_t lds = (size_t)3 * 2 * (TY + 2) * (Z + 2) * 16;
  static bool lds_raised = false;
  if (int rc = vox_raise_lds(lds_raised, "vox_bf3", lds, vox_bf3_kernel<CK, Z, TY, false>, vox_bf3_kernel<CK, Z, TY, true>)) return rc;
  const dim3 grid((unsigned)((long)a.N * a.ytiles * cdiv(a.X, xseg)), cdiv(Cout, 16));
  return vox_with_bool(act > MUVO_ACT_LEAKY, [&](auto generic) -> int {
    hipLaunchKernelGGL((vox_bf3_kernel<CK, Z, TY, decltype(generic)::value>), grid, dim3(64 * TY), lds, st, a, in, (const vu32x4*)wp, bias, out,
                       act, slope, xseg,  0);
    MUVO_CHECK_LAUNCH("vox_bf3_kernel");
    return MUVO_OK;
  });
}

template <int Z>
static int launch_vox_bf3_2row(const muvo_conv_desc* d, const float* in, const float* wp, const float* bias, float* out, int act,
                               float slope, hipStream_t st, double* moments, const float* aff) {
  constexpr int CK = 8, TY = 16;
  VoxArgs a = vox_args(d, CK, 8, TY, Z, 0, aff);
  a.moments = moments;
  const int xseg = vox_xseg(a, 1, 0);
  constexpr size_t lds = (size_t)3 * 2 * (TY + 2) * (Z + 2) * 16;
  static_assert(lds <= 160 * 1024, "LDS budget");
  static bool lds_raised = false;
  if (int rc = vox_raise_lds(lds_raised, "vox_bf3_2row", lds, vox_bf3_2row_kernel<Z, CK, false>, vox_bf3_2row_kernel<Z, CK, true>)) return rc;
  const dim3 grid((unsigned)((long)a.N * a.ytiles * cdiv(a.X, xseg)));
  return vox_with_bool(act > MUVO_ACT_LEAKY, [&](auto generic) -> int {
    hipLaunchKernelGGL((vox_bf3_2row_kernel<Z, CK, decltype(generic)::value>), grid, dim3(32 * TY), lds, st, a, in, (const vu32x4*)wp, bias, out,
                       act, slope, xseg);
    MUVO_CHECK_LAUNCH("vox_bf3_2row_kernel");
    return MUVO_OK;
  });
}

template <int Z, bool CO8>
static int launch_vox_bf3_ps(const muvo_conv_desc* d, int Cout, const float* in, const float* wp, const float* bias, float* out, int act,
                             float slope, hipStream_t st, int cin_total, int accum, double* moments, const float* aff) {
  constexpr int TY = VOX_PS_TY;
  VoxArgs a = vox_args(d, 16, Cout, TY, Z, cin_total, aff);
  a.moments = moments;
  const int xseg = vox_xseg(a, 1, 0);
  constexpr size_t lds = (size_t)2 * 2 * 2 * (TY + 2) * (Z + 2) * 16;
  static bool lds_raised = false;
  if (int rc = vox_raise_lds(lds_raised, "vox_bf3_ps", lds, vox_bf3_ps_kernel<Z, TY, CO8, false>, vox_bf3_ps_kernel<Z, TY, CO8, true>)) return rc;
  const dim3 grid((unsigned)((long)a.N * a.ytiles * cdiv(a.X, xseg)), cdiv(Cout, 16));
  return vox_with_bool(accum || act > MUVO_ACT_LEAKY, [&](auto generic) -> int {
    hipLaunchKernelGGL((vox_bf3_ps_kernel<Z, TY, CO8, decltype(generic)::value>), grid, dim3(64 * TY), lds, st, a, in, (const vu32x4*)wp, bias, out,
                       act, slope, xseg, accum);
    MUVO_CHECK_LAUNCH("vox_bf3_ps_kernel");
    return MUVO_OK;
  });
}

static int vox_conv_dispatch(const muvo_conv_desc* d, int Cin, int Cout, const float* in, const float* wp, const float* bias,
                             float* out, int act, float slope, hipStream_t st, bool bf3, double* moments, const float* aff) {
  if (moments && !bf3) { muvo_set_error("vox_conv: output moments need the bf16x3 kernels"); return MUVO_ERR_INVALID_ARG; }
  const int Z = d->in_sz[2];
  if (bf3 && vox_bf3_ps(Cin, Cout)) {
    const long XYZ = (long)d->in_sz[0] * d->in_sz[1] * Z;
    const size_t wstep = (size_t)cdiv(Cout, 16) * (Cout <= 8 ? 10 : 15) * 2 * 64 * 4;
    const int npass = Cin / 16, cin_total = npass > 1 ? Cin : 0;
    return vox_with_z<true>(Z, [&](auto z) -> int {
      constexpr int ZC = decltype(z)::value;
      return vox_with_bool(Cout <= 8, [&](auto co8) -> int {
        for (int ps = 0; ps < npass; ++ps) {
          const bool last = ps == npass - 1;
          const int rc = launch_vox_bf3_ps<ZC, decltype(co8)::value>(d, Cout, in + (size_t)ps * 16 * XYZ, wp + ps * wstep, last ? bias : nullptr, out,
                                                                     last ? act : MUVO_ACT_NONE, last ? slope : 0.f, st, cin_total, ps > 0,
                                                                     last ? moments : nullptr, aff);
          if (rc) return rc;
        }
        return MUVO_OK;
      });
    });
  }
  if (bf3 && vox_bf3_two_rows(Cin, Cout))
    return vox_with_z(Z, [&](auto z) -> int { return launch_vox_bf3_2row<decltype(z)::value>(d, in, wp, bias, out, act, slope, st, moments, aff); });
  if (bf3 && Cin == 8)
    return vox_with_z(Z, [&](auto z) -> int { return launch_vox_bf3<decltype(z)::value>(d, Cout, in, wp, bias, out, act, slope, st, moments, aff); });
  if (Cout == 8) return vox_with_z(Z, [&](auto z) -> int { return launch_vox_conv<2, 6, decltype(z)::value>(d, Cin, Cout, in, wp, bias, out, act, slope, st); });
  if (Cout == 16) return vox_with_z(Z, [&](auto z) -> int { return launch_vox_conv<4, 4, decltype(z)::value>(d, Cin, Cout, in, wp, bias, out, act, slope, st); });
  muvo_set_error("vox_conv: unsupported shape Cout=%d Z=%d", Cout, Z);
  return MUVO_ERR_INVALID_ARG;
}

int vox_forward(const muvo_conv_desc* d, const float* x, const float* wp, const float* bias, float* y, int act, float slope,
                hipStream_t st, bool bf3, double* moments, const float* aff) {
  if (aff && !vox_affine_ok(d)) { muvo_set_error("vox_forward: no affine staging for this shape"); return MUVO_ERR_INVALID_ARG; }
  return vox_conv_dispatch(d, d->Cin, d->Cout, x, wp, bias, y, act, slope, st, bf3 || aff != nullptr, moments, aff);
}
bool vox_affine_ok(const muvo_conv_desc* d) {
  return vox_fwd_applicable(d) && vox_bf3_shape_ok(d, 0) && vox_bf3_wgrad_shape_ok(d) && (d->Cin == 8 || d->Cin == 16);
}
int vox_dgrad(const muvo_conv_desc* d, const float* dy, const float* wp, float* dx, hipStream_t st, bool bf3) {
  return vox_conv_dispatch(d, d->Cout, d->Cin, dy, wp, nullptr, dx, MUVO_ACT_NONE, 0.f, st, bf3, nullptr, nullptr);
}

template <int RQB, int CQR, int Z, int TYB>
static int launch_vox_wgrad(const muvo_conv_desc* d, const float* x, const float* dz, float* dw, float* dbias,
                            hipStream_t st) {
  constexpr int CQB = 2;
  VoxArgs a = vox_args(d, d->Cin, d->Cout, TYB, Z, 0, nullptr);
  const int nqc = d->Cout / (4 * CQB), nrc = d->Cin / (4 * RQB);
  int xsplit = 1;
  while ((long)a.N * a.ytiles * xsplit * nqc * nrc < 1536 && a.X / (xsplit * 2) >= 8) xsplit *= 2;
  constexpr size_t lds = sizeof(float) * (3 * RQB * (TYB + 2) * (Z + 2) * 4 + 2 * CQB * TYB * Z * 4);
  static bool lds_raised = false;
  if (int rc = vox_raise_lds(lds_raised, "vox_wgrad", lds, vox_wgrad_kernel<RQB, CQR, Z, TYB>)) return rc;
  dim3 grid(a.N * a.ytiles * xsplit, nqc * nrc);
  a.ticket = muvo_det_ticket(st);
  hipLaunchKernelGGL((vox_wgrad_kernel<RQB, CQR, Z, TYB>), grid, dim3(768), lds, st, a, x, dz, dw, dbias, xsplit, nqc);
  MUVO_CHECK_LAUNCH("vox_wgrad_kernel");
  return MUVO_OK;
}

bool vox_wgrad_ps_only(const muvo_conv_desc* d) {
  return vox_geometry_ok(d, true) && (d->in_sz[2] == 16 || d->Cout == 32) && d->Cin % 16 == 0 && d->Cin <= 64 &&
         (d->Cout == 8 || d->Cout == 16 || d->Cout == 32);
}
bool vox_bf3_wgrad_shape_ok(const muvo_conv_desc* d) {
  if (vox_wgrad_ps_only(d)) return true;
  return vox_wgrad_applicable(d) && (d->Cin == 8 || d->Cin % 16 == 0) && d->Cin <= 64 && (d->Cout == 8 || d->Cout == 16);
}

template <int Z>
static int launch_vox_bf3_wgrad(const muvo_conv_desc* d, const float* x, const float* dz, float* dw, float* dbias, hipStream_t st,
                                const float* aff) {
  constexpr int CI = 8;
  constexpr int ZH = Z / 32, WROWS = 8 / ZH, ROWS = WROWS + 2;
  constexpr size_t lds = (size_t)4 * 2 * CI * (ROWS * (Z + 16) * 2 + 16) + (size_t)2 * 2 * 16 * (WROWS * Z * 2 + 16) + 64;
  static_assert(lds <= 160 * 1024, "LDS budget");
  static_assert(lds >= 15 * 256 * 4 + 64, "the reduction reuses the rings");
  const VoxArgs a = vox_args(d, d->Cin, d->Cout, WROWS, Z, 0, aff);
  const int xseg = vox_xseg(a, a.Cin / CI, 1);
  static bool lds_raised = false;
  if (int rc = vox_raise_lds(lds_raised, "vox_bf3_wgrad", lds, vox_bf3_wgrad_kernel<Z, CI, false>)) return rc;
  dim3 grid((unsigned)((long)a.N * a.ytiles * cdiv(a.X, xseg)), a.Cin / CI);
  hipLaunchKernelGGL((vox_bf3_wgrad_kernel<Z, CI, false>), grid, dim3(512), lds, st, a, x, dz, dw, dbias, xseg);
  MUVO_CHECK_LAUNCH("vox_bf3_wgrad_kernel");
  return MUVO_OK;
}

template <int Z, int CI, bool CO8>
static int launch_vox_bf3_wgrad_ps(const muvo_conv_desc* d, const float* x, const float* dz, float* dw, float* dbias, hipStream_t st,
                                   const float* aff) {
  constexpr int SW = (CI == 16 && CO8) ? VOX_WGPS_SW : 0;
  constexpr int ZH = Z >= 32 ? Z / 32 : 1, RW = Z >= 32 ? 1 : 32 / Z, WROWS = 8 / ZH * RW, ROWS = WROWS + 2;
  constexpr size_t lds = (size_t)2 * 2 * CI * (ROWS * (Z + 16) * 2 + 16) + 64;
  const VoxArgs a = vox_args(d, d->Cin, d->Cout, WROWS, Z, 0, aff);
  const int xseg = vox_xseg(a, (a.Cin / CI) * cdiv(a.Cout, 16), 1);
  static bool lds_raised = false;
  if (int rc = vox_raise_lds(lds_raised, "vox_bf3_wgrad_ps", lds, vox_bf3_wgrad_ps_kernel<Z, CI, CO8, SW>)) return rc;
  dim3 grid((unsigned)((long)a.N * a.ytiles * cdiv(a.X, xseg)), a.Cin / CI, cdiv(a.Cout, 16));
  hipLaunchKernelGGL((vox_bf3_wgrad_ps_kernel<Z, CI, CO8, SW>), grid, dim3(512 + 64 * SW), lds, st, a, x, dz, dw, dbias, xseg);
  MUVO_CHECK_LAUNCH("vox_bf3_wgrad_ps_kernel");
  return MUVO_OK;
}

int vox_wgrad(const muvo_conv_desc* d, const float* x, const float* dz, float* dw, float* dbias, hipStream_t st, bool bf3,
              const float* aff) {
  if (aff && !vox_affine_ok(d)) { muvo_set_error("vox_wgrad: no affine staging for this shape"); return MUVO_ERR_INVALID_ARG; }
  if (aff) bf3 = true;
  const int Z = d->in_sz[2];
  if (bf3) {
    if (Z == 16 && !vox_wgrad_ps_only(d)) { muvo_set_error("vox_wgrad: 16-voxel z lines need the plane-streaming kernel"); return MUVO_ERR_INVALID_ARG; }
    const bool co8 = d->Cout <= 8;
    if (d->Cin != 8)
      return vox_with_z<true>(Z, [&](auto z) -> int {
        constexpr int ZC = decltype(z)::value;
        return vox_with_bool(co8, [&](auto c) -> int { return launch_vox_bf3_wgrad_ps<ZC, 16, decltype(c)::value>(d, x, dz, dw, dbias, st, aff); });
      });
    if (co8) return vox_with_z(Z, [&](auto z) -> int { return launch_vox_bf3_wgrad_ps<decltype(z)::value, 8, true>(d, x, dz, dw, dbias, st, aff); });
    return vox_with_z(Z, [&](auto z) -> int { return launch_vox_bf3_wgrad<decltype(z)::value>(d, x, dz, dw, dbias, st, aff); });
  }
  const bool r4 = d->Cin % 16 == 0;
  return vox_with_z(Z, [&](auto z) -> int {
    constexpr int ZC = decltype(z)::value, TYB = ZC == 64 ? 4 : 8;
    return r4 ? launch_vox_wgrad<4, 2, ZC, TYB>(d, x, dz, dw, dbias, st) : launch_vox_wgrad<2, 1, ZC, TYB>(d, x, dz, dw, dbias, st);
  });
}
```

muvo_amd/csrc/elementwise.hip:

```cpp
#include "common.h"

#define GRID_STRIDE(i, n) for (long i = blockIdx.x * (long)blockDim.x + threadIdx.x; i < (n); i += (long)gridDim.x * blockDim.x)

__global__ void act_bwd_kernel(const float* __restrict__ y, const float* __restrict__ dy, float* __restrict__ dx, long n,
                               int act, float slope) {
  GRID_STRIDE(i, n) dx[i] = dy[i] * act_grad_from_out(y[i], act, slope);
}
__global__ void act_fwd_kernel(const float* __restrict__ x, float* __restrict__ y, long n, int act, float slope) {
  GRID_STRIDE(i, n) y[i] = act_apply(x[i], act, slope);
}
__global__ void dropout_kernel(const float* __restrict__ x, float* __restrict__ y, long n, float p, uint64_t seed) {
  GRID_STRIDE(i, n) y[i] = x[i] * dropout_scale(seed, (uint64_t)i, p);
}
__global__ void axpby_kernel(const float* __restrict__ a, const float* __restrict__ b, float* __restrict__ out, long n,
                             float alpha, float beta) {
  GRID_STRIDE(i, n) out[i] = alpha * a[i] + (b ? beta * b[i] : 0.f);
}
__global__ void copy2d_kernel(const float* __restrict__ src, float* __restrict__ dst, long rows, long cols, long lds,
                              long ldd, int accumulate) {
  const long n = rows * cols;
  GRID_STRIDE(i, n) {
    const long r = i / cols, c = i - r * cols;
    if (accumulate) dst[r * ldd + c] += src[r * lds + c];
    else dst[r * ldd + c] = src[r * lds + c];
// ... 440 lines not shown
                                                                     int H, int W, int dseg) {
  const int OH = 2 * H, OW = 2 * W;
  const int j = threadIdx.x, h = threadIdx.y;
  const long nc = blockIdx.y;
  const int d0 = blockIdx.x * dseg, d1 = min(d0 + dseg, D);
  float wb[4];
  up2_bwd_weights(h, H, wb);
  const bool left = j > 0, right = 8 * j + 8 < OW;
  const float* gp = dy + nc * (2L * D) * OH * OW;
  const long ps = (long)OH * OW;
  auto contrib = [&](int a) -> float4 {
    if (a < 0 || a >= 2 * D) return make_float4(0.f, 0.f, 0.f, 0.f);
    return up2_plane_contrib(gp + (long)a * ps, OH, OW, h, j, wb, W, left, right);
  };
  float4 pm1 = contrib(2 * d0 - 1), p0 = contrib(2 * d0);
  for (int d = d0; d < d1; ++d) {
    const float4 p1 = contrib(2 * d + 1), p2 = contrib(2 * d + 2);
    float wa[4];
    up2_bwd_weights(d, D, wa);
    float4 o;
    o.x = (wa[0] * pm1.x + wa[1] * p0.x) + (wa[2] * p1.x + wa[3] * p2.x);
    o.y = (wa[0] * pm1.y + wa[1] * p0.y) + (wa[2] * p1.y + wa[3] * p2.y);
    o.z = (wa[0] * pm1.z + wa[1] * p0.z) + (wa[2] * p1.z + wa[3] * p2.z);
    o.w = (wa[0] * pm1.w + wa[1] * p0.w) + (wa[2] * p1.w + wa[3] * p2.w);
    *((float4*)(dx + ((nc * D + d) * H + h) * (long)W) + j) = o;
    pm1 = p1; p0 = p2;
  }
}

__global__ void __launch_bounds__(256) upsample3d_x2_bwd_row_kernel(const float* __restrict__ dy, float* __restrict__ dx, int D,
                                                                    int H, int W, int dseg) {
  const int OH = 2 * H, OW = 2 * W, OQ = W / 2;
  const int f = threadIdx.x % OQ;
  const int hr = blockIdx.x * (256 / OQ) + threadIdx.x / OQ;
  const bool live = hr < H;
  const int h = live ? hr : H - 1;
  const long nc = blockIdx.z;
  const int d0 = blockIdx.y * dseg, d1 = min(d0 + dseg, D);
  float wb[4];
  up2_bwd_weights(h, H, wb);
  const float w1a = f > 0 ? 0.75f : 1.f, w2b = 2 * f + 1 < W - 1 ? 0.75f : 1.f, w2a = 2 * f < W - 1 ? 0.75f : 1.f;
  const float* gp = dy + nc * (2L * D) * OH * OW + 4 * f;
  const long ps = (long)OH * OW;
  auto load_rows = [&](int a, float4 (&g)[4]) {
    const int ac = a < 0 ? 0 : (a >= 2 * D ? 2 * D - 1 : a);
    const float* plane = gp + (long)ac * ps;
#pragma unroll
    for (int ib = 0; ib < 4; ++ib) {
      int r = 2 * h - 1 + ib;
      r = r < 0 ? 0 : (r > OH - 1 ? OH - 1 : r);
      g[ib] = *(const float4*)(plane + (long)r * OW);
    }
  };
  auto reduce_rows = [&](int a, const float4 (&g)[4]) -> float2 {
    float2 acc = make_float2(0.f, 0.f);
    const float pw = (a < 0 || a >= 2 * D) ? 0.f : 1.f;
#pragma unroll
    for (int ib = 0; ib < 4; ++ib) {
      const float lft = __shfl_up(g[ib].w, 1), rgt = __shfl_down(g[ib].x, 1);
      const float gl = f > 0 ? lft : 0.f, gr = f < OQ - 1 ? rgt : 0.f;
      const float wgt = wb[ib] * pw;
      acc.x += wgt * ((0.25f * gl + w1a * g[ib].x) + (w2a * g[ib].y + 0.25f * g[ib].z));
      acc.y += wgt * ((0.25f * g[ib].y + 0.75f * g[ib].z) + (w2b * g[ib].w + 0.25f * gr));
    }
    return acc;
  };
  float4 ga[4], gb[4];
  load_rows(2 * d0 - 1, ga); load_rows(2 * d0, gb);
  float2 pm1 = reduce_rows(2 * d0 - 1, ga), p0 = reduce_rows(2 * d0, gb);
  load_rows(2 * d0 + 1, ga); load_rows(2 * d0 + 2, gb);
  for (int d = d0; d < d1; ++d) {
    const float2 p1 = reduce_rows(2 * d + 1, ga), p2 = reduce_rows(2 * d + 2, gb);
    if (d + 1 < d1) { load_rows(2 * d + 3, ga); load_rows(2 * d + 4, gb); }
    float wa[4];
    up2_bwd_weights(d, D, wa);
    float2 o;
    o.x = (wa[0] * pm1.x + wa[1] * p0.x) + (wa[2] * p1.x + wa[3] * p2.x);
    o.y = (wa[0] * pm1.y + wa[1] * p0.y) + (wa[2] * p1.y + wa[3] * p2.y);
    *((float2*)(dx + ((nc * D + d) * H + h) * (long)W) + f) = o;
    pm1 = p1; p0 = p2;
  }
}

__global__ void preprocess_image_kernel(const uint8_t* __restrict__ img, float* __restrict__ label,
                                        float* __restrict__ norm, long NC, int C, int H, int W, int top, int left, int CH,
                                        int CW, float m0, float m1, float m2, float s0, float s1, float s2) {
  const long n = NC * CH * CW;
  GRID_STRIDE(i, n) {
    const int x = (int)(i % CW);
    long r = i / CW;
    const int y = (int)(r % CH);
    const long nc = r / CH;
    const int c = (int)(nc % C);
    const float v = (float)img[(nc * H + (y + top)) * W + (x + left)] / 255.f;
    if (label) label[i] = v;
    const float m = c == 0 ? m0 : (c == 1 ? m1 : m2), s = c == 0 ? s0 : (c == 1 ? s1 : s2);
    norm[i] = (v - m) / s;
  }
}
__global__ void preprocess_route_kernel(const uint8_t* __restrict__ img, float* __restrict__ norm, long NC, int C, int H,
                                        int W, int OH, int OW, float m0, float m1, float m2, float s0, float s1, float s2) {
  const long n = NC * OH * OW;
  const float sh = (float)H / (float)OH, sw = (float)W / (float)OW;
  GRID_STRIDE(i, n) {
    const int x = (int)(i % OW);
    long r = i / OW;
    const int y = (int)(r % OH);
    const long nc = r / OH;
    const int c = (int)(nc % C);
    int sy = (int)floorf((float)y * sh); if (sy > H - 1) sy = H - 1;
    int sx = (int)floorf((float)x * sw); if (sx > W - 1) sx = W - 1;
    const float v = (float)img[(nc * H + sy) * W + sx] / 255.f;
    const float m = c == 0 ? m0 : (c == 1 ? m1 : m2), s = c == 0 ? s0 : (c == 1 ? s1 : s2);
    norm[i] = (v - m) / s;
  }
}
__global__ void scale_kernel(const float* __restrict__ x, float* __restrict__ y, long n, float inv) {
  GRID_STRIDE(i, n) y[i] = x[i] / inv;
}
__global__ void resize_bilinear_kernel(const float* __restrict__ x, float* __restrict__ y, long NC, int H, int W, int OH,
                                       int OW) {
  const long n = NC * OH * OW;
  const float sh = (float)H / (float)OH, sw = (float)W / (float)OW;
  GRID_STRIDE(i, n) {
    const int ox = (int)(i % OW);
    long r = i / OW;
    const int oy = (int)(r % OH);
    const long nc = r / OH;
    float fy = sh * ((float)oy + 0.5f) - 0.5f; if (fy < 0.f) fy = 0.f;
    float fx = sw * ((float)ox + 0.5f) - 0.5f; if (fx < 0.f) fx = 0.f;
    const int y0 = (int)fy, x0 = (int)fx;
    const int y1 = y0 + (y0 < H - 1 ? 1 : 0), x1 = x0 + (x0 < W - 1 ? 1 : 0);
    const float ly = fy - (float)y0, lx = fx - (float)x0;
    const float hy = 1.f - ly, hx = 1.f - lx;
    const float* xp = x + nc * H * W;
    y[i] = hy * (hx * xp[y0 * W + x0] + lx * xp[y0 * W + x1]) + ly * (hx * xp[y1 * W + x0] + lx * xp[y1 * W + x1]);
  }
}
template <typename T>
__global__ void resize_nearest_kernel(const T* __restrict__ x, T* __restrict__ y, long NC, int D, int H, int W, int OD,
                                      int OH, int OW) {
  const long n = NC * OD * OH * OW;
  const float sd = (float)D / (float)OD, sh = (float)H / (float)OH, sw = (float)W / (float)OW;
  GRID_STRIDE(i, n) {
    const int ox = (int)(i % OW);
    long r = i / OW;
    const int oy = (int)(r % OH);
    r /= OH;
    const int oz = (int)(r % OD);
    const long nc = r / OD;
    int z = (int)floorf((float)oz * sd); if (z > D - 1) z = D - 1;
    int yy = (int)floorf((float)oy * sh); if (yy > H - 1) yy = H - 1;
    int xx = (int)floorf((float)ox * sw); if (xx > W - 1) xx = W - 1;
    y[i] = x[((nc * D + z) * H + yy) * W + xx];
  }
}

#define SOFTMAX_MAXV 17
template <int MAXV>
__global__ void __launch_bounds__(256) softmax_dropout_fwd_kernel(const float* __restrict__ S, float* __restrict__ P,
                                                                  float* __restrict__ Pd, long rows, int cols, float p,
                                                                  uint64_t seed) {
  const int lane = threadIdx.x & 63;
  const long row = blockIdx.x * 4L + (threadIdx.x >> 6);
  if (row >= rows) return;
  float v[MAXV];
// ... 248 lines not shown
                       int s, int p, void* stream) {
  MUVO_CHECK_ARG(dy && dx && idx && NC > 0 && NC <= 2147483647L, "maxpool2d_bwd: bad args");
  MUVO_CHECK_ARG((k == 3 && s == 2 && p == 1) || (k == 2 && s == 2 && p == 0), "maxpool2d: only 3x3 s2 p1 and 2x2 s2 p0 are on the path");
  MUVO_CHECK_ARG(cdiv(H, 4) <= 65535, "maxpool2d_bwd: image too tall");
  dim3 grid(cdiv(W, 256), cdiv(H, 4), (unsigned)NC), block(64, 4);
  static const bool v8 = !getenv("MUVO_MAXPOOL_BWD_V8") || atoi(getenv("MUVO_MAXPOOL_BWD_V8")) != 0;
  if (k == 3 && v8 && W % 8 == 0 && OW % 4 == 0 && 2 * OW == W && 2 * OH == H && ((((uintptr_t)dy) | ((uintptr_t)dx)) & 15) == 0 &&
      (((uintptr_t)idx) & 3) == 0) {
    hipLaunchKernelGGL(maxpool3s2_bwd_v8_kernel, dim3(cdiv(W / 8, 64), cdiv(H / 2, 4), (unsigned)NC), block, 0, ST, dy, idx, dx, H, W, OH, OW);
  } else if (k == 3) hipLaunchKernelGGL((maxpool2d_bwd_t_kernel<3, 2, 1>), grid, block, 0, ST, dy, idx, dx, H, W, OH, OW);
  else hipLaunchKernelGGL((maxpool2d_bwd_t_kernel<2, 2, 0>), grid, block, 0, ST, dy, idx, dx, H, W, OH, OW);
  MUVO_CHECK_LAUNCH("maxpool2d_bwd");
  return MUVO_OK;
}
int muvo_avgpool_fwd(const float* x, float* y, int64_t G, int64_t S, void* stream) {
  MUVO_CHECK_ARG(x && y && G > 0 && S > 0, "avgpool_fwd: bad args");
  hipLaunchKernelGGL(avgpool_fwd_kernel, dim3(cdiv(G, 4)), dim3(256), 0, ST, x, y, (long)G, (long)S);
  MUVO_CHECK_LAUNCH("avgpool_fwd");
  return MUVO_OK;
}
int muvo_avgpool_bwd(const float* dy, float* dx, int64_t G, int64_t S, void* stream) {
  MUVO_CHECK_ARG(dy && dx && G > 0 && S > 0, "avgpool_bwd: bad args");
  hipLaunchKernelGGL(avgpool_bwd_kernel, dim3(ew_grid(G * S)), dim3(256), 0, ST, dy, dx, (long)G, (long)S);
  MUVO_CHECK_LAUNCH("avgpool_bwd");
  return MUVO_OK;
}
int muvo_upsample3d_x2_fwd(const float* x, float* y, int64_t NC, int D, int H, int W, void* stream) {
  MUVO_CHECK_ARG(x && y && NC > 0 && D > 0 && H > 0 && W > 0, "upsample3d_fwd: bad args");
  const int q8 = W / 4;
  const int oq = W / 2;
  if (W % 4 == 0 && oq <= 64 && (oq & (oq - 1)) == 0 && D + 1 <= 65535 && NC <= 65535) {
    dim3 grid(cdiv((long)(H + 1) * oq, 256), D + 1, (unsigned)NC);
    hipLaunchKernelGGL(upsample3d_x2_fwd_row_kernel, grid, dim3(256), 0, ST, x, y, D, H, W);
    MUVO_CHECK_LAUNCH("upsample3d_fwd_row");
    return MUVO_OK;
  }
  if (W % 4 == 0 && q8 <= 64 && (q8 & (q8 - 1)) == 0 && 2 * D <= 65535 && NC <= 65535) {
    dim3 grid(cdiv((long)2 * H * q8, 256), 2 * D, (unsigned)NC);
    hipLaunchKernelGGL(upsample3d_x2_fwd_vec8_kernel, grid, dim3(256), 0, ST, x, y, D, H, W);
    MUVO_CHECK_LAUNCH("upsample3d_fwd_vec8");
    return MUVO_OK;
  }
  if (W % 2 == 0 && 2 * D <= 65535 && NC <= 65535) {
    dim3 grid(cdiv((long)2 * H * (2 * W / 4), 256), 2 * D, (unsigned)NC);
    hipLaunchKernelGGL(upsample3d_x2_fwd_vec_kernel, grid, dim3(256), 0, ST, x, y, D, H, W);
    MUVO_CHECK_LAUNCH("upsample3d_fwd_vec");
    return MUVO_OK;
  }
  hipLaunchKernelGGL(upsample3d_x2_fwd_kernel, dim3(ew_grid(NC * D * H * W * 8)), dim3(256), 0, ST, x, y, (long)NC, D, H, W);
  MUVO_CHECK_LAUNCH("upsample3d_fwd");
  return MUVO_OK;
}
int muvo_upsample3d_x2_bwd(const float* dy, float* dx, int64_t NC, int D, int H, int W, void* stream) {
  MUVO_CHECK_ARG(dy && dx && NC > 0 && D > 0 && H > 0 && W > 0, "upsample3d_bwd: bad args");
  static const int walk = getenv("MUVO_UPSAMPLE_WALK") ? atoi(getenv("MUVO_UPSAMPLE_WALK")) : 2;
  const int oq = W / 2;
  if (walk == 2 && W % 4 == 0 && oq <= 64 && (oq & (oq - 1)) == 0 && NC <= 65535 && (((uintptr_t)dy | (uintptr_t)dx) & 15) == 0) {
    const int rgroups = cdiv(H, 256 / oq);
    int segs = 1;
    while ((long)NC * rgroups * segs < 4096 && segs * 16 <= D) segs *= 2;
    const int dseg = cdiv(D, segs);
    hipLaunchKernelGGL(upsample3d_x2_bwd_row_kernel, dim3(rgroups, cdiv(D, dseg), (unsigned)NC), dim3(256), 0, ST, dy, dx, D, H, W, dseg);
    MUVO_CHECK_LAUNCH("upsample3d_bwd_row");
    return MUVO_OK;
  }
  if (walk && W % 4 == 0 && (W / 4) * H <= 1024 && (W / 4) * H >= 128 && NC <= 65535 && (((uintptr_t)dy | (uintptr_t)dx) & 15) == 0) {
    int segs = 1;
    while ((long)NC * segs < 1024 && segs * 8 <= D) segs *= 2;
    const int dseg = cdiv(D, segs);
    hipLaunchKernelGGL(upsample3d_x2_bwd_walk_kernel, dim3(cdiv(D, dseg), (unsigned)NC), dim3(W / 4, H), 0, ST, dy, dx, D, H, W, dseg);
    MUVO_CHECK_LAUNCH("upsample3d_bwd_walk");
    return MUVO_OK;
  }
  if (W % 4 == 0 && D <= 65535 && NC <= 65535) {
    dim3 grid(cdiv((long)H * (W / 4), 256), D, (unsigned)NC);
    hipLaunchKernelGGL(upsample3d_x2_bwd_vec_kernel, grid, dim3(256), 0, ST, dy, dx, D, H, W);
    MUVO_CHECK_LAUNCH("upsample3d_bwd_vec");
    return MUVO_OK;
  }
  hipLaunchKernelGGL(upsample3d_x2_bwd_kernel, dim3(ew_grid(NC * D * H * W)), dim3(256), 0, ST, dy, dx, (long)NC, D, H, W);
  MUVO_CHECK_LAUNCH("upsample3d_bwd");
  return MUVO_OK;
}
int muvo_preprocess_image(const uint8_t* img, float* label, float* norm, int64_t NC, int C, int H, int W, int top, int left,
                          int CH, int CW, const float* mean3, const float* std3, void* stream) {
  MUVO_CHECK_ARG(img && norm && mean3 && std3 && C == 3, "preprocess_image: bad args");
  MUVO_CHECK_ARG(top >= 0 && left >= 0 && top + CH <= H && left + CW <= W, "preprocess_image: crop outside the image");
  hipLaunchKernelGGL(preprocess_image_kernel, dim3(ew_grid(NC * CH * CW)), dim3(256), 0, ST, img, label, norm, (long)NC, C, H,
                     W, top, left, CH, CW, mean3[0], mean3[1], mean3[2], std3[0], std3[1], std3[2]);
  MUVO_CHECK_LAUNCH("preprocess_image");
  return MUVO_OK;
}
int muvo_preprocess_route(const uint8_t* img, float* norm, int64_t NC, int C, int H, int W, int OH, int OW,
                          const float* mean3, const float* std3, void* stream) {
  MUVO_CHECK_ARG(img && norm && mean3 && std3 && C == 3, "preprocess_route: bad args");
  hipLaunchKernelGGL(preprocess_route_kernel, dim3(ew_grid(NC * OH * OW)), dim3(256), 0, ST, img, norm, (long)NC, C, H, W, OH,
                     OW, mean3[0], mean3[1], mean3[2], std3[0], std3[1], std3[2]);
  MUVO_CHECK_LAUNCH("preprocess_route");
  return MUVO_OK;
}
int muvo_divide_scalar(const float* x, float* y, int64_t n, float divisor, void* stream) {
  MUVO_CHECK_ARG(x && y && n > 0 && divisor != 0.f, "divide_scalar: bad args");
  hipLaunchKernelGGL(scale_kernel, dim3(ew_grid(n)), dim3(256), 0, ST, x, y, (long)n, divisor);
  MUVO_CHECK_LAUNCH("divide_scalar");
  return MUVO_OK;
}
int muvo_resize_bilinear(const float* x, float* y, int64_t NC, int H, int W, int OH, int OW, void* stream) {
  MUVO_CHECK_ARG(x && y && NC > 0 && H > 0 && W > 0 && OH > 0 && OW > 0, "resize_bilinear: bad args");
  hipLaunchKernelGGL(resize_bilinear_kernel, dim3(ew_grid(NC * OH * OW)), dim3(256), 0, ST, x, y, (long)NC, H, W, OH, OW);
  MUVO_CHECK_LAUNCH("resize_bilinear");
  return MUVO_OK;
}
int muvo_resize_nearest_f32(const float* x, float* y, int64_t NC, int D, int H, int W, int OD, int OH, int OW, void* stream) {
  MUVO_CHECK_ARG(x && y && NC > 0, "resize_nearest_f32: bad args");
  hipLaunchKernelGGL((resize_nearest_kernel<float>), dim3(ew_grid(NC * OD * OH * OW)), dim3(256), 0, ST, x, y, (long)NC, D, H,
                     W, OD, OH, OW);
  MUVO_CHECK_LAUNCH("resize_nearest_f32");
  return MUVO_OK;
}
int muvo_resize_nearest_u8(const uint8_t* x, uint8_t* y, int64_t NC, int D, int H, int W, int OD, int OH, int OW,
                           void* stream) {
  MUVO_CHECK_ARG(x && y && NC > 0, "resize_nearest_u8: bad args");
  hipLaunchKernelGGL((resize_nearest_kernel<uint8_t>), dim3(ew_grid(NC * OD * OH * OW)), dim3(256), 0, ST, x, y, (long)NC, D,
                     H, W, OD, OH, OW);
  MUVO_CHECK_LAUNCH("resize_nearest_u8");
  return MUVO_OK;
}
int muvo_softmax_dropout_fwd(const float* S, float* P, float* Pd, int64_t rows, int cols, float p, uint64_t seed,
                             void* stream) {
  MUVO_CHECK_ARG(S && P && rows > 0 && cols > 0 && cols <= 64 * SOFTMAX_MAXV, "softmax_fwd: bad args (cols=%d, max %d)", cols, 64 * SOFTMAX_MAXV);
  if (cols <= 512)
    hipLaunchKernelGGL((softmax_dropout_fwd_kernel<8>), dim3(cdiv(rows, 4)), dim3(256), 0, ST, S, P, Pd, (long)rows, cols, p, seed);
  else
    hipLaunchKernelGGL((softmax_dropout_fwd_kernel<SOFTMAX_MAXV>), dim3(cdiv(rows, 4)), dim3(256), 0, ST, S, P, Pd, (long)rows, cols, p, seed);
  MUVO_CHECK_LAUNCH("softmax_fwd");
  return MUVO_OK;
}
int muvo_softmax_dropout_bwd(const float* P, const float* dPd, float* dS, int64_t rows, int cols, float p, uint64_t seed,
                             void* stream) {
  MUVO_CHECK_ARG(P && dPd && dS && rows > 0 && cols > 0 && cols <= 64 * SOFTMAX_MAXV, "softmax_bwd: bad args");
  if (cols <= 512)
    hipLaunchKernelGGL((softmax_dropout_bwd_kernel<8>), dim3(cdiv(rows, 4)), dim3(256), 0, ST, P, dPd, dS, (long)rows, cols, p, seed);
  else
    hipLaunchKernelGGL((softmax_dropout_bwd_kernel<SOFTMAX_MAXV>), dim3(cdiv(rows, 4)), dim3(256), 0, ST, P, dPd, dS, (long)rows, cols, p, seed);
  MUVO_CHECK_LAUNCH("softmax_bwd");
  return MUVO_OK;
}
int muvo_gru_fwd(const float* gi, const float* gh, const float* h, float* hnew, int B, int H, void* stream) {
  MUVO_CHECK_ARG(gi && gh && h && hnew && B > 0 && H > 0, "gru_fwd: bad args");
  hipLaunchKernelGGL(gru_fwd_kernel, dim3(ew_grid((long)B * H)), dim3(256), 0, ST, gi, gh, h, hnew, B, H);
  MUVO_CHECK_LAUNCH("gru_fwd");
  return MUVO_OK;
}
int muvo_gru_bwd(const float* gi, const float* gh, const float* h, const float* dhnew, float* dgi, float* dgh, float* dh,
                 int B, int H, void* stream) {
  MUVO_CHECK_ARG(gi && gh && h && dhnew && dgi && dgh && dh && B > 0 && H > 0, "gru_bwd: bad args");
  hipLaunchKernelGGL(gru_bwd_kernel, dim3(ew_grid((long)B * H)), dim3(256), 0, ST, gi, gh, h, dhnew, dgi, dgh, dh, B, H);
  MUVO_CHECK_LAUNCH("gru_bwd");
  return MUVO_OK;
}
int muvo_rssm_sample_fwd(const float* mu_logsigma, const float* eps, int64_t eps_ld, float* mu, float* sigma, float* sample,
                         int B, int S, float min_std, void* stream) {
  MUVO_CHECK_ARG(mu_logsigma && mu && sigma && sample && B > 0 && S > 0, "rssm_sample_fwd: bad args");
  hipLaunchKernelGGL(rssm_sample_fwd_kernel, dim3(ew_grid((long)B * S)), dim3(256), 0, ST, mu_logsigma, eps, (long)eps_ld, mu,
                     sigma, sample, B, S, min_std);
  MUVO_CHECK_LAUNCH("rssm_sample_fwd");
// ... 101 lines not shown
```

muvo_amd/models/common.py:

```python
import math

import torch
import torch.nn as nn

from muvo_amd import nn as hnn
from muvo_amd import ops
from muvo_amd.models.resnet import ResNet18Features


class RouteEncode(nn.Module):
    def __init__(self, out_channels, backbone='resnet18'):
        super().__init__()
        assert backbone == 'resnet18'
        self.backbone = ResNet18Features(in_chans=3, out_indices=(4,))
        self.out_channels = out_channels
        self.fc = hnn.Linear(512, out_channels)

    def forward(self, route):
        x = self.backbone(route)[0]
        return self.fc(ops.global_avg_pool(x))


class Policy(nn.Module):
    def __init__(self, in_channels):
# ... 16 lines not shown
class DecoderDS(nn.Module):
    def __init__(self, feature_info, out_channels):
        super().__init__()
        self.conv1 = _conv_bn_relu(feature_info[0]['num_chs'], out_channels)
        self.downsample_skip_convs = nn.ModuleList(
            _conv_bn_relu(feature_info[i]['num_chs'], out_channels) for i in range(1, len(feature_info)))
        self.out_channels = out_channels

    def feat_consumers(self):
        return [(self.conv1[0],)] + [(c[0],) for c in self.downsample_skip_convs]

    def forward(self, xs):
        x = self.conv1[1](self.conv1[0](xs[0]), relu=True, from_conv=True)
        for i, conv in enumerate(self.downsample_skip_convs):
            stride = xs[i].shape[-1] // xs[i + 1].shape[-1]
            pooled = ops.max_pool2d(x, stride)
            x = conv[1](conv[0](xs[i + 1]), residual=pooled, res_mode=2, relu=True, from_conv=True)
        return x


class Decoder(nn.Module):

    def __init__(self, feature_info, out_channels):
        super().__init__()
        n_upsample_skip_convs = len(feature_info) - 1
        self.conv1 = _conv_bn_relu(feature_info[-1]['num_chs'], out_channels)
        self.upsample_skip_convs = nn.ModuleList(
            _conv_bn_relu(feature_info[-i]['num_chs'], out_channels) for i in range(2, n_upsample_skip_convs + 2))
        self.out_channels = out_channels

    def forward(self, xs):
        x = self.conv1[1](self.conv1[0](xs[-1]), relu=True)
        for i, conv in enumerate(self.upsample_skip_convs):
            up = ops.interpolate_bilinear(x, xs[-(i + 2)].shape[-2:])
            x = conv[1](conv[0](xs[-(i + 2)]), residual=up, res_mode=2, relu=True)
        return x


class StyleBank:

    def __init__(self, latent, modules, styles):
        self.latent = latent
        self.shape = latent.shape
        self._styles = {id(m): s for m, s in zip(modules, styles)}

    def style_of(self, norm):
        return self._styles[id(norm)]

    @staticmethod
    def build(decoder, w):
        if isinstance(w, StyleBank):
            return w
        norms = decoder.__dict__.get('_adain_layers')
        if norms is None:
            norms = [m for m in decoder.modules() if isinstance(m, (AdaptiveInstanceNorm3d, AdaptiveInstanceNorm))]
            decoder.__dict__['_adain_layers'] = norms
        linears = [m.latent_affine for m in norms]
        if not norms or not ops.grouped_linear_supported(w, linears):
            return w
        return StyleBank(w, norms, ops.grouped_linear(w, linears))


def _style(norm, style):
    return style.style_of(norm) if isinstance(style, StyleBank) else norm.latent_affine(style)


class AdaptiveInstanceNorm3d(nn.Module):
    def __init__(self, latent_n_channels, out_channels, epsilon=1e-8):
        super().__init__()
        self.out_channels = out_channels
        self.epsilon = epsilon
        self.latent_affine = hnn.Linear(latent_n_channels, 2 * out_channels)

    def forward(self, x, style, pre_act=ops.ACT_NONE, pre_slope=0.0, moments=None):
        return ops.adain(x, _style(self, style), self.epsilon, style.shape[0], pre_act, pre_slope, moments)


class ConvInstanceNorm3d(nn.Module):
    def __init__(self, in_channels, out_channels, latent_n_channels):
        super().__init__()
        self.conv_act = nn.Sequential(hnn.Conv3d(in_channels, out_channels, 3, 1, 1), hnn.Placeholder())
        self.adaptive_norm = AdaptiveInstanceNorm3d(latent_n_channels, out_channels)

    def forward(self, x, w, lazy=None, next_conv=None):
        moments = ops.conv_moments_buffer(x, self.conv_act[0].geom)
        x = self.conv_act[0](x, act=ops.ACT_LEAKY, slope=0.2, act_bwd_fused=True, moments=moments, lazy=lazy)
        if next_conv is not None and ops.conv_affine_supported(x, next_conv.geom, moments):
            an = self.adaptive_norm
            y, raw, aff = ops.adain_lazy(x, _style(an, w), an.epsilon, ops.ACT_LEAKY, 0.2, moments)
            return y, (raw, aff)
        y = self.adaptive_norm(x, w, pre_act=ops.ACT_LEAKY, pre_slope=0.2, moments=moments)
        return y if next_conv is None else (y, None)

    def forward_with_head(self, x, w, head_conv, lazy=None):
        moments = ops.conv_moments_buffer(x, self.conv_act[0].geom)
        x = self.conv_act[0](x, act=ops.ACT_LEAKY, slope=0.2, act_bwd_fused=True, moments=moments, lazy=lazy)
        if ops.adain_head_supported(x, head_conv.weight, moments):
            an = self.adaptive_norm
            return ops.adain_head(x, _style(an, w), head_conv.weight, head_conv.bias, an.epsilon, moments, ops.ACT_LEAKY, 0.2)
        return head_conv(self.adaptive_norm(x, w, pre_act=ops.ACT_LEAKY, pre_slope=0.2, moments=moments))


class AdaptiveInstanceNorm(nn.Module):

    def __init__(self, latent_n_channels, out_channels, epsilon=1e-8):
        super().__init__()
        self.out_channels = out_channels
        self.epsilon = epsilon
        self.latent_affine = hnn.Linear(latent_n_channels, 2 * out_channels)

    def forward(self, x, style, pre_act=ops.ACT_NONE, pre_slope=0.0):
        x5 = x.unsqueeze(-3)
        y = ops.adain(x5, _style(self, style), self.epsilon, style.shape[0], pre_act, pre_slope)
        return y.squeeze(2)


class ConvInstanceNorm(nn.Module):

    def __init__(self, in_channels, out_channels, latent_n_channels):
        super().__init__()
        self.conv_act = nn.Sequential(hnn.Conv2d(in_channels, out_channels, 3, 1, 1), hnn.Placeholder())
        self.adaptive_norm = AdaptiveInstanceNorm(latent_n_channels, out_channels)

    def forward(self, x, w):
        x = self.conv_act[0](x, act=ops.ACT_LEAKY, slope=0.2, act_bwd_fused=True)
        return self.adaptive_norm(x, w, pre_act=ops.ACT_LEAKY, pre_slope=0.2)


class DecoderBlock(nn.Module):

    def __init__(self, in_channels, out_channels, latent_n_channels, upsample=False):
        super().__init__()
        self.upsample = upsample
        self.conv1 = ConvInstanceNorm(in_channels, out_channels, latent_n_channels)
        self.conv2 = ConvInstanceNorm(out_channels, out_channels, latent_n_channels)

    def forward(self, x, w):
        if self.upsample:
            x = ops.interpolate_bilinear(x, (2 * x.shape[-2], 2 * x.shape[-1]))
        return self.conv2(self.conv1(x, w), w)


class SegmentationHead(nn.Module):

    def __init__(self, in_channels, n_classes, downsample_factor):
        super().__init__()
        self.downsample_factor = downsample_factor
        self.segmentation_head = nn.Sequential(hnn.Conv2d(in_channels, n_classes, 1, 1, 0))
        self.instance_offset_head = nn.Sequential(hnn.Conv2d(in_channels, 2, 1, 1, 0))
        self.instance_center_head = nn.Sequential(hnn.Conv2d(in_channels, 1, 1, 1, 0), hnn.Placeholder())

    def forward(self, x):
        f = self.downsample_factor
        return {f'bev_segmentation_{f}': self.segmentation_head[0](x),
                f'bev_instance_offset_{f}': self.instance_offset_head[0](x),
                f'bev_instance_center_{f}': self.instance_center_head[0](x, act=ops.ACT_SIGMOID)}


class BevDecoder(nn.Module):

    def __init__(self, latent_n_channels, semantic_n_channels, constant_size=(3, 3), head='bev'):
        super().__init__()
        assert head == 'bev'
        n = 512
        self.constant_tensor = nn.Parameter(torch.randn((n, *constant_size), dtype=torch.float32))
        self.first_norm = AdaptiveInstanceNorm(latent_n_channels, out_channels=n)
        self.first_conv = ConvInstanceNorm(n, n, latent_n_channels)
        self.middle_conv = nn.ModuleList(DecoderBlock(n, n, latent_n_channels, upsample=True) for _ in range(3))
        self.conv1 = DecoderBlock(n, 256, latent_n_channels, upsample=True)
        self.head_4 = SegmentationHead(256, semantic_n_channels, downsample_factor=4)
        self.conv2 = DecoderBlock(256, 128, latent_n_channels, upsample=True)
        self.head_2 = SegmentationHead(128, semantic_n_channels, downsample_factor=2)
        self.conv3 = DecoderBlock(128, 64, latent_n_channels, upsample=True)
        self.head_1 = SegmentationHead(64, semantic_n_channels, downsample_factor=1)

    def forward(self, w):
        w = StyleBank.build(self, w)
        x = self.first_norm(self.constant_tensor, w)
        x = self.first_conv(x, w)
        for module in self.middle_conv:
            x = module(x, w)
        x = self.conv1(x, w)
        output_4 = self.head_4(x)
        x = self.conv2(x, w)
        output_2 = self.head_2(x)
        x = self.conv3(x, w)
        output_1 = self.head_1(x)
        return {**output_4, **output_2, **output_1}


class DecoderBlock3d(nn.Module):
    def __init__(self, in_channels, out_channels, latent_n_channels, upsample=False):
        super().__init__()
        self.upsample = upsample
        self.conv1 = ConvInstanceNorm3d(in_channels, out_channels, latent_n_channels)
        self.conv2 = ConvInstanceNorm3d(out_channels, out_channels, latent_n_channels)

    def forward(self, x, w, head_conv=None):
        if self.upsample:
            x = ops.upsample3d_x2(x)
        y, lazy = self.conv1(x, w, next_conv=self.conv2.conv_act[0])
        if head_conv is not None:
            return self.conv2.forward_with_head(y, w, head_conv, lazy=lazy)
        return self.conv2(y, w, lazy=lazy)


class _Head(nn.Module):

    def __init__(self, attr, key, conv, downsample_factor):
        super().__init__()
        self.downsample_factor = downsample_factor
        self._attr, self._key = attr, key
        setattr(self, attr, nn.Sequential(conv))

    def forward(self, x):
        return {f'{self._key}_{self.downsample_factor}': getattr(self, self._attr)[0](x)}

    def branch(self, x):
        m = getattr(self, self._attr)[0]
        x, y = ops.head_branch(x, m.weight, m.bias, m.geom, m._packed)
        return x, {f'{self._key}_{self.downsample_factor}': y}


def RGBHead(in_channels, n_classes, downsample_factor):
    return _Head('rgb_head', 'rgb', hnn.Conv2d(in_channels, n_classes, 1, 1, 0), downsample_factor)


def LidarReHead(in_channels, n_classes, downsample_factor):
    return _Head('lidar_re_head', 'lidar_reconstruction', hnn.Conv2d(in_channels, n_classes, 1, 1, 0), downsample_factor)


def LidarSegHead(in_channels, n_classes, downsample_factor):
    return _Head('seg_head', 'lidar_segmentation', hnn.Conv2d(in_channels, n_classes, 1, 1, 0), downsample_factor)


def SemHead(in_channels, n_classes, downsample_factor):
    return _Head('sem_head', 'semantic_image', hnn.Conv2d(in_channels, n_classes, 1, 1, 0), downsample_factor)


def DepthHead(in_channels, n_classes, downsample_factor):
    return _Head('depth_head', 'depth', hnn.Conv2d(in_channels, n_classes, 1, 1, 0), downsample_factor)


def VoxelSemHead(in_channels, n_classes, downsample_factor):
    return _Head('segmentation_head', 'voxel', hnn.Conv3d(in_channels, n_classes, 1, 1, 0), downsample_factor)


class VoxelDecoder1(nn.Module):
    def __init__(self, latent_n_channels, semantic_n_channels, feature_channels=512, constant_size=(3, 3, 1)):
        super().__init__()
        n = feature_channels
        self.constant_tensor = nn.Parameter(torch.randn((2 * n, *constant_size), dtype=torch.float32))
        self.first_norm = AdaptiveInstanceNorm3d(latent_n_channels, out_channels=2 * n)
        self.first_conv = ConvInstanceNorm3d(2 * n, n, latent_n_channels)
        self.middle_conv = nn.ModuleList(DecoderBlock3d(n, n, latent_n_channels, upsample=True) for _ in range(3))
        self.conv1 = DecoderBlock3d(n, n // 2, latent_n_channels, upsample=True)
        self.head_4 = VoxelSemHead(n // 2, semantic_n_channels, downsample_factor=4)
        self.conv2 = DecoderBlock3d(n // 2, n // 4, latent_n_channels, upsample=True)
        self.head_2 = VoxelSemHead(n // 4, semantic_n_channels, downsample_factor=2)
        self.conv3 = DecoderBlock3d(n // 4, n // 8, latent_n_channels, upsample=True)
        self.head_1 = VoxelSemHead(n // 8, semantic_n_channels, downsample_factor=1)

    def forward(self, w):
        w = StyleBank.build(self, w)
        x = self.first_norm(self.constant_tensor, w)
        x = self.first_conv(x, w)
        for module in self.middle_conv:
            x = module(x, w)
        x = self.conv1(x, w)
        x, output_4 = self.head_4.branch(x)
        x = self.conv2(x, w)
        x, output_2 = self.head_2.branch(x)
        h1 = self.head_1
        output_1 = {f'{h1._key}_{h1.downsample_factor}': self.conv3(x, w, head_conv=getattr(h1, h1._attr)[0])}
        return {**output_4, **output_2, **output_1}


class _Seed1x1ConvTFn(torch.autograd.Function):

    @staticmethod
    def forward(ctx, x, weight, bias, act):
        x = x.contiguous()
        n, ci = x.shape[0], x.shape[1]
        co, kh, kw = weight.shape[1:]
# ... 86 lines not shown
```

muvo_amd/ops.py:

```python
import collections
import contextlib
import ctypes as C
import math
import os
import threading
import weakref

import torch

_HERE = os.path.dirname(os.path.abspath(__file__))
_LIB_PATH = os.environ.get('MUVO_HIP_LIB') or os.path.join(_HERE, 'libmuvo_hip.so')
_lib = None
_lock = threading.Lock()

ACT_NONE, ACT_RELU, ACT_LEAKY, ACT_ELU, ACT_TANH, ACT_SIGMOID = 0, 1, 2, 3, 4, 5


class ConvDesc(C.Structure):
    _fields_ = [('nd', C.c_int32), ('transposed', C.c_int32), ('N', C.c_int32), ('Cin', C.c_int32), ('Cout', C.c_int32),
                ('in_sz', C.c_int32 * 3), ('out_sz', C.c_int32 * 3), ('ksz', C.c_int32 * 3), ('stride', C.c_int32 * 3),
                ('pad', C.c_int32 * 3), ('dil', C.c_int32 * 3)]


class GemmDesc(C.Structure):
    _fields_ = [('M', C.c_int32), ('N', C.c_int32), ('K', C.c_int32),
                ('sam', C.c_int64), ('sak', C.c_int64), ('sbk', C.c_int64), ('sbn', C.c_int64), ('scm', C.c_int64),
                ('B1', C.c_int32), ('B2', C.c_int32),
                ('a_b1', C.c_int64), ('a_b2', C.c_int64), ('b_b1', C.c_int64), ('b_b2', C.c_int64),
                ('c_b1', C.c_int64), ('c_b2', C.c_int64),
                ('alpha', C.c_float), ('bias_div', C.c_int32), ('act', C.c_int32), ('slope', C.c_float),
                ('mode', C.c_int32)]


EXPORTS = [
    'muvo_last_error', 'muvo_abi_version', 'muvo_selftest_mfma', 'muvo_set_deterministic', 'muvo_get_deterministic', 'muvo_reset_accumulators',
    'muvo_conv_set_products', 'muvo_conv_get_products',
    'muvo_conv_set_mode', 'muvo_conv_get_mode', 'muvo_conv_set_bf16x3_min_gflop', 'muvo_conv_pack_sizes', 'muvo_conv_workspace_bytes', 'muvo_conv_kernel_family', 'muvo_conv_kernel_variant', 'muvo_conv_pack_weights', 'muvo_conv_forward', 'muvo_conv_dgrad', 'muvo_conv_prepare_dy', 'muvo_conv_wgrad', 'muvo_bias_grad_nchw',
    'muvo_gemm',
    'muvo_pack_table_item_bytes', 'muvo_conv_pack_table_add', 'muvo_linear_bf16x3_pack_table_add', 'muvo_pack_table_run',
    'muvo_linear_bf16x3_pack_floats', 'muvo_linear_bf16x3_pack', 'muvo_linear_bf16x3_workspace_bytes', 'muvo_linear_bf16x3_split',
    'muvo_linear_bf16x3_forward', 'muvo_linear_bf16x3_dgrad', 'muvo_linear_bf16x3_wgrad',
    'muvo_bn_train_fwd', 'muvo_bn_train_bwd', 'muvo_adain_fwd', 'muvo_adain_bwd',
    'muvo_add_dropout_layernorm_fwd', 'muvo_add_dropout_layernorm_bwd',
    'muvo_act_fwd', 'muvo_act_bwd', 'muvo_dropout', 'muvo_axpby', 'muvo_copy2d', 'muvo_colsum_acc', 'muvo_batchsum',
    'muvo_nchw_to_tokens', 'muvo_tokens_to_nchw', 'muvo_maxpool2d_fwd', 'muvo_maxpool2d_bwd', 'muvo_avgpool_fwd',
    'muvo_avgpool_bwd', 'muvo_upsample3d_x2_fwd', 'muvo_upsample3d_x2_bwd', 'muvo_preprocess_image',
    'muvo_preprocess_route', 'muvo_divide_scalar', 'muvo_resize_bilinear', 'muvo_resize_nearest_f32',
    'muvo_resize_nearest_u8', 'muvo_softmax_dropout_fwd', 'muvo_softmax_dropout_bwd', 'muvo_gru_fwd', 'muvo_gru_bwd',
    'muvo_rssm_sample_fwd', 'muvo_rssm_sample_bwd',
    'muvo_spatial_loss_fwd', 'muvo_spatial_loss_bwd', 'muvo_spatial_loss_masked_fwd', 'muvo_spatial_loss_masked_bwd', 'muvo_voxel_loss_stats_doubles', 'muvo_voxel_loss_coef_floats',
    'muvo_voxel_loss_fwd', 'muvo_voxel_loss_bwd', 'muvo_l1_rows_fwd', 'muvo_l1_rows_bwd', 'muvo_kl_loss_fwd',
    'muvo_kl_loss_bwd', 'muvo_adamw_step', 'muvo_chamfer_loss_ws_doubles', 'muvo_chamfer_loss_fwd', 'muvo_chamfer_loss_bwd',
    'muvo_ssim_frames', 'muvo_sqdiff_frames', 'muvo_chamfer_sums', 'muvo_ssc_counts', 'muvo_seg_confusion', 'muvo_seg_confusion_index',
    'muvo_frustum_cells', 'muvo_frustum_pool_fwd', 'muvo_frustum_pool_bwd', 'muvo_depth_expectation',
    'muvo_resize_bilinear_bwd', 'muvo_softmax_channel_fwd', 'muvo_softmax_channel_bwd',
    'muvo_range_projection', 'muvo_voxel_grid', 'muvo_seg_ce_fwd', 'muvo_seg_ce_bwd', 'muvo_ssim_maps', 'muvo_ssim_bwd',
    'muvo_instance_labels', 'muvo_pixel_augment', 'muvo_preprocess_route_aug',
    'muvo_split_planes_bytes', 'muvo_split_planes', 'muvo_attention_supported', 'muvo_attention_fwd', 'muvo_attention_bwd',
    'muvo_conv_dgrad_accumulate', 'muvo_conv_forward_moments_supported', 'muvo_conv_forward_moments', 'muvo_adain_fwd_moments',
    'muvo_adain_head_supported', 'muvo_adain_head_fwd', 'muvo_adain_head_bwd', 'muvo_bf3_loop_clock',
    'muvo_grouped_linear_fwd', 'muvo_grouped_linear_bwd', 'muvo_conv_prepare_dy_head', 'muvo_conv_prepare_dy_head_supported',
    'muvo_conv_forward_head_supported', 'muvo_conv_forward_head',
    'muvo_adain_affine', 'muvo_conv_affine_supported', 'muvo_conv_forward_affine', 'muvo_conv_wgrad_affine',
    'muvo_fake_allreduce', 'muvo_resize_bilinear_aa', 'muvo_bn_train_fwd_planes', 'muvo_bn_train_bwd_planes', 'muvo_conv_forward_planes',
    'muvo_stem_conv_supported', 'muvo_stem_conv_forward', 'muvo_stem_conv_wgrad',
    'muvo_rssm_supported', 'muvo_rssm_transposed_floats', 'muvo_rssm_scratch_floats', 'muvo_rssm_forward', 'muvo_rssm_backward',
    'muvo_voxelize_scratch_bytes', 'muvo_voxelize_frames',
    'muvo_birdview_decode_frames', 'muvo_label_components_frames', 'muvo_depth_semantic_decode_frames',
    'muvo_range_projection_frames', 'muvo_voxel_grid_frames',
    'muvo_attention_stream_supported', 'muvo_attention_stream_blocks', 'muvo_attention_stream_fwd', 'muvo_attention_stream_bwd',
    'muvo_voxel_rows_scratch_bytes', 'muvo_voxel_rows_logits', 'muvo_voxel_rows_grid', 'muvo_voxel_rows_write', 'muvo_image_u8',
    'muvo_panel_image', 'muvo_panel_logits', 'muvo_panel_labels', 'muvo_panel_fill', 'muvo_panel_bars', 'muvo_panel_scatter',
    'muvo_panel_voxel_top_logits', 'muvo_panel_voxel_top_grid',
    'muvo_icp_state_doubles', 'muvo_icp_ws_doubles', 'muvo_icp_init', 'muvo_icp_iterate',
    'muvo_flow_max_pairs', 'muvo_flow_workspace_bytes', 'muvo_flow_farneback', 'muvo_flow_colour_ws_bytes', 'muvo_flow_colour',
    'muvo_flow_epe_ws_doubles', 'muvo_flow_epe',
    'muvo_raycast_brick_words', 'muvo_raycast_bricks_grid', 'muvo_raycast_bricks_logits', 'muvo_raycast', 'muvo_panel_voxel_view',
    'muvo_ray_iou_ws_doubles', 'muvo_ray_iou_counts',
]


def lib():
    global _lib
    if _lib is None:
        with _lock:
            if _lib is None:
                if not os.path.exists(_LIB_PATH):
                    raise RuntimeError(f'{_LIB_PATH} not found: build it with `python -m muvo_amd.build` '
                                       '(there is no fallback path)')
                L = C.CDLL(_LIB_PATH)
                L.muvo_last_error.restype = C.c_char_p
                L.muvo_conv_workspace_bytes.restype = C.c_int64
                L.muvo_linear_bf16x3_workspace_bytes.restype = C.c_int64
                L.muvo_pack_table_item_bytes.restype = C.c_int64
                L.muvo_split_planes_bytes.restype = C.c_int64
                L.muvo_rssm_transposed_floats.restype = C.c_int64
                L.muvo_rssm_scratch_floats.restype = C.c_int64
                L.muvo_voxelize_scratch_bytes.restype = C.c_int64
                L.muvo_voxel_rows_scratch_bytes.restype = C.c_int64
                L.muvo_chamfer_loss_ws_doubles.restype = C.c_int64
                L.muvo_icp_state_doubles.restype = C.c_int64
                L.muvo_icp_ws_doubles.restype = C.c_int64
                for name in ('muvo_flow_max_pairs', 'muvo_flow_workspace_bytes', 'muvo_flow_colour_ws_bytes', 'muvo_flow_epe_ws_doubles',
                             'muvo_raycast_brick_words', 'muvo_ray_iou_ws_doubles'):
                    getattr(L, name).restype = C.c_int64
                for name in EXPORTS:
                    getattr(L, name)
                _lib = L
    return _lib


def _ck(rc):
    if rc != 0:
        msg = lib().muvo_last_error().decode()
        reset_accumulators()
        raise RuntimeError(f'muvo_hip error {rc}: {msg}')


_MOMENT_BUFS = []


def reset_accumulators():
    try:
        if _lib is not None:
            _lib.muvo_reset_accumulators()
        live = []
        for r in _MOMENT_BUFS:
            t = r()
            if t is not None:
                t.zero_()
                live.append(r)
        _MOMENT_BUFS[:] = live
    except Exception:
        pass


def _st():
    return C.c_void_p(torch._C._cuda_getCurrentRawStream(torch.cuda.current_device()))


def _p(t):
    if t is None:
        return C.c_void_p(0)
    assert t.is_cuda and t.is_contiguous(), 'muvo_hip ops need contiguous device tensors'
    return C.c_void_p(t.data_ptr())


def _f(t):
    assert t is None or t.dtype == torch.float32
    return _p(t)


def _i64(v):
    return C.c_int64(int(v))


def _fl(v):
    return C.c_float(float(v))


_weight_epoch = [0]
# ... 952 lines not shown

    @staticmethod
    def _split_dy(ctx, plan, x, y, dy, head, use_act, planes):
        L, d, bias = lib(), C.byref(plan.desc), ctx.bias
        act = ctx.act if use_act else ACT_NONE
        if head is None:
            _ck(L.muvo_conv_prepare_dy(d, _f(y) if use_act else None, _f(dy), act, _fl(ctx.slope), _p(planes),
                                       _f(grad_of(bias)) if bias is not None else None, _st()))
            return dy, planes
        gl, head_w, head_b, head_wgrad = head
        co = head_w.shape[0]
        ride = use_act and head_w.requires_grad
        if not ride:
            head_wgrad()
        _ck(L.muvo_conv_prepare_dy_head(d, _f(y) if use_act else None, _f(dy) if dy is not None else None,
                                        _f(gl.contiguous()), _f(head_w.contiguous().view(co, -1)), co, act, _fl(ctx.slope),
                                        _p(planes), _f(grad_of(bias)) if bias is not None else None,
                                        _f(grad_of(head_w)) if ride else None,
                                        _f(grad_of(head_b)) if (ride and head_b is not None) else None, _st()))
        if dy is None:
            dy = y if y is not None else x
        return dy, planes

    @staticmethod
    def _data_grad(ctx, plan, x, dz, planes, fused_dy, dy_ws):
        wp = _packed_weight(plan, ctx.packed, ctx.weight, 1)
        dx = torch.empty(x.shape, device=dz.device, dtype=torch.float32)
        e1 = _bracket(plan, 'dgrad') if KERNEL_TIMING is not None else None
        if planes is None and (plan.ws_dgrad_dy > 0 or plan.ws_wgrad_dy > 0):
            planes = dy_ws.get(plan.dy_planes_floats)
        _ck(lib().muvo_conv_dgrad(C.byref(plan.desc), _f(dz), _f(wp), _f(dx), _p(planes), 1 if fused_dy else 0, _st()))
        if e1 is not None:
            e1.record()
        return dx, planes

    @staticmethod
    def _weight_grad(ctx, plan, x, y, dz, ws_dy, dy_is_split, fused_dy, dy_ws):
        bias = ctx.bias
        gw = grad_of(ctx.weight)
        db = grad_of(bias) if (bias is not None and not fused_dy) else None
        ws_x = ctx.ws_x
        x_ph = getattr(ctx, 'x_is_placeholder', False)
        xptr = ws_x if x_ph else x
        flags = (1 if ws_x is not None else 0) | (2 if (dy_is_split and plan.ws_wgrad_dy > 0) else 0)
        with _on_wgrad_stream(dy_ws.wst, x.device, (xptr, y, dz, ws_x, ctx.aff), dy_ws.slot):
            ws = scratch_zeroed('wgrad', plan.pack_fwd, x.device)
            e1 = _bracket(plan, 'wgrad') if KERNEL_TIMING is not None else None
            if ws_x is None and plan.ws_wgrad_x:
                ws_x = scratch('conv_ws', (plan.ws_wgrad_x + 3) // 4, x.device)
            if plan.ws_wgrad_dy and ws_dy is None:
                ws_dy = scratch('conv_ws_dy', (plan.ws_wgrad_dy + 3) // 4, x.device)
            if ctx.aff is not None:
                _ck(lib().muvo_conv_wgrad_affine(C.byref(plan.desc), _f(x), _f(ctx.aff), _f(dz), _f(gw), _f(db), _st()))
            else:
                assert not x_ph or (flags & 1)
                _ck(lib().muvo_conv_wgrad(C.byref(plan.desc), _f(xptr), _f(dz), _f(ws), _f(gw), _f(db), _p(ws_x), _p(ws_dy),
                                          flags, _st()))
            if e1 is not None:
                e1.record()


def conv(x, weight, bias, geom, packed, act=ACT_NONE, slope=0.0, act_bwd_fused=False, moments=None, lazy=None):
    if lazy is not None:
        return ConvFn.apply(x, weight, bias, geom, packed, act, slope, act_bwd_fused, moments, lazy[0], lazy[1])
    y = ConvFn.apply(x, weight, bias, geom, packed, act, slope, act_bwd_fused, moments)
    if (BN_PLANES and bias is None and act == ACT_NONE and moments is None and x.requires_grad and weight.requires_grad
            and torch.is_grad_enabled() and geom.plan_for(x).dy_planes):
        y._muvo_dy_planes_ok = True
    return y


CONV_AFFINE = os.environ.get('MUVO_CONV_AFFINE', '1') != '0'


def conv_affine_supported(x, geom, moments):
    if not CONV_AFFINE or moments is None or x.dim() != 5 or not (x.requires_grad and torch.is_grad_enabled()):
        return False
    return geom.plan_for(x).supports('muvo_conv_affine_supported')


CONV_MOMENTS = os.environ.get('MUVO_CONV_MOMENTS', '1') != '0'


def conv_moments_buffer(x, geom):
    if not CONV_MOMENTS or not geom.plan_for(x).supports('muvo_conv_forward_moments_supported'):
        return None
    n = x.shape[0]
    cache = geom.__dict__.setdefault('_moments', {})
    buf = cache.get((n, x.device))
    if buf is None:
        buf = cache[(n, x.device)] = torch.zeros(n, geom.cout, 2, device=x.device, dtype=torch.float64)
        _MOMENT_BUFS.append(weakref.ref(buf))
    return buf


def _grad_is_private(g):
    return g._base is None and g._use_count() <= 2


class HeadBranchFn(torch.autograd.Function):

    @staticmethod
    def forward(ctx, x, weight, bias, geom, packed):
        y = ConvFn.forward(ctx, x, weight, bias, geom, packed, ACT_NONE, 0.0)
        return x.view_as(x), y

    @staticmethod
    def backward(ctx, gx, gy):
        x, _ = ctx.saved_tensors
        weight, bias = ctx.weight, ctx.bias
        if gy is None:
            return (gx,) + (None,) * 4
        plan = ctx.geom.plan_for(x)
        L, d = lib(), C.byref(plan.desc)
        gy = gy.contiguous()
        dx = None
        if ctx.needs_input_grad[0]:
            wp = _packed_weight(plan, ctx.packed, weight, 1)
            if gx is not None and gx.is_contiguous() and _grad_is_private(gx):
                dx = gx
                _ck(L.muvo_conv_dgrad_accumulate(d, _f(gy), _f(wp), _f(dx), _st()))
            else:
                dx = torch.empty_like(x)
                _ck(L.muvo_conv_dgrad(d, _f(gy), _f(wp), _f(dx), None, 0, _st()))
                if gx is not None:
                    dx = dx + gx
        if weight.requires_grad:
            ws = scratch_zeroed('wgrad', plan.pack_fwd, x.device)
            _ck(L.muvo_conv_wgrad(d, _f(x), _f(gy), _f(ws), _f(grad_of(weight)), _f(grad_of(bias)) if bias is not None else None,
                                  None, None, 0, _st()))
        return (dx,) + (None,) * 4


class ConvHeadFn(torch.autograd.Function):

    @staticmethod
    def forward(ctx, x, weight, bias, geom, packed, act, slope, head_w, head_b, head_geom, head_packed):
        plan = geom.plan_for(x)
        co = head_geom.cout
        fused = plan.supports('muvo_conv_forward_head_supported', co)
        logits = None
        if fused:
            logits = torch.empty((plan.n, co) + plan.oshape[2:], device=x.device, dtype=torch.float32)
            ctx._head_fwd = (head_w.contiguous().view(co, -1), head_b, logits)
        y = ConvFn.forward(ctx, x, weight, bias, geom, packed, act, slope)
        ctx._head_fwd = None
        ctx.save_for_backward(x, y)
        ctx.head = (head_w, head_b, head_geom)
        ctx.set_materialize_grads(False)
        if not fused:
            hplan = head_geom.plan_for(y)
            hwp = _packed_weight(hplan, head_packed, head_w, 0)
            logits = torch.empty(hplan.oshape, device=x.device, dtype=torch.float32)
            _ck(lib().muvo_conv_forward(C.byref(hplan.desc), _f(y), _f(hwp), _f(head_b), _f(logits), ACT_NONE, _fl(0.0), None, _st()))
        return y, logits

    @staticmethod
    def backward(ctx, gy, gl):
        if gl is None:
            if gy is None:
                return (None,) * 11
            return ConvFn._backward(ctx, gy, None)[:7] + (None,) * 4
        x, y = ctx.saved_tensors
        head_w, head_b, head_geom = ctx.head
        hplan = head_geom.plan_for(y)
        gl = gl.contiguous()

        def head_wgrad():
# ... 459 lines not shown
        _ck(lib().muvo_nchw_to_tokens(_f(dx), None, None, 0, _f(dtok), n, c, l, l0, _st()))
        return dtok, None, None, None


def untoken(tok, l0, h, w):
    return UntokenFn.apply(tok, l0, h, w)


class MaxPool2dFn(torch.autograd.Function):
    @staticmethod
    def forward(ctx, x, k, s, p):
        x = x.contiguous()
        n, c, h, w = x.shape
        oh, ow = (h + 2 * p - k) // s + 1, (w + 2 * p - k) // s + 1
        y = torch.empty(n, c, oh, ow, device=x.device, dtype=torch.float32)
        idx = torch.empty(n, c, oh, ow, device=x.device, dtype=torch.uint8)
        _ck(lib().muvo_maxpool2d_fwd(_f(x), _f(y), _p(idx), _i64(n * c), h, w, oh, ow, k, s, p, _st()))
        ctx.dims = (n, c, h, w, oh, ow, k, s, p)
        ctx.save_for_backward(idx)
        return y

    @staticmethod
    def backward(ctx, dy):
        (idx,) = ctx.saved_tensors
        n, c, h, w, oh, ow, k, s, p = ctx.dims
        dy = dy.contiguous()
        dx = torch.empty(n, c, h, w, device=dy.device, dtype=torch.float32)
        _ck(lib().muvo_maxpool2d_bwd(_f(dy), _p(idx), _f(dx), _i64(n * c), h, w, oh, ow, k, s, p, _st()))
        return dx, None, None, None


def max_pool2d(x, k, s=None, p=0):
    return MaxPool2dFn.apply(x, k, s or k, p)


class GlobalAvgPoolFn(torch.autograd.Function):
    @staticmethod
    def forward(ctx, x):
        x = x.contiguous()
        n, c = x.shape[:2]
        s = x.numel() // (n * c)
        y = torch.empty(n, c, device=x.device, dtype=torch.float32)
        _ck(lib().muvo_avgpool_fwd(_f(x), _f(y), _i64(n * c), _i64(s), _st()))
        ctx.shape = x.shape
        return y

    @staticmethod
    def backward(ctx, dy):
        dy = dy.contiguous()
        shape = ctx.shape
        dx = torch.empty(shape, device=dy.device, dtype=torch.float32)
        g = shape[0] * shape[1]
        _ck(lib().muvo_avgpool_bwd(_f(dy), _f(dx), _i64(g), _i64(dx.numel() // g), _st()))
        return dx


def global_avg_pool(x):
    return GlobalAvgPoolFn.apply(x)


class Upsample3dFn(torch.autograd.Function):
    @staticmethod
    def forward(ctx, x):
        x = x.contiguous()
        n, c, d, h, w = x.shape
        y = torch.empty(n, c, 2 * d, 2 * h, 2 * w, device=x.device, dtype=torch.float32)
        _ck(lib().muvo_upsample3d_x2_fwd(_f(x), _f(y), _i64(n * c), d, h, w, _st()))
        ctx.shape = x.shape
        return y

    @staticmethod
    def backward(ctx, dy):
        dy = dy.contiguous()
        n, c, d, h, w = ctx.shape
        dx = torch.empty(ctx.shape, device=dy.device, dtype=torch.float32)
        _ck(lib().muvo_upsample3d_x2_bwd(_f(dy), _f(dx), _i64(n * c), d, h, w, _st()))
        return dx


def upsample3d_x2(x):
    return Upsample3dFn.apply(x)


class AttentionFn(torch.autograd.Function):

    @staticmethod
    def forward(ctx, qkv, nheads, p, seed):
        qkv = qkv.contiguous()
        l, n, e3 = qkv.shape
        e = e3 // 3
        dh = e // nheads
        scale = 1.0 / (dh ** 0.5)
        dev = qkv.device
        S = torch.empty(n, nheads, l, l, device=dev, dtype=torch.float32)
        gemm(qkv, qkv, S, l, l, dh, n * e3, 1, 1, n * e3, l, alpha=scale, B1=n, B2=nheads,
             a_b=(e3, dh), b_b=(e3, dh), c_b=(nheads * l * l, l * l), b_off=e)
        P = torch.empty_like(S)
        Pd = torch.empty_like(S) if p > 0 else None
        _ck(lib().muvo_softmax_dropout_fwd(_f(S), _f(P), _f(Pd), _i64(n * nheads * l), l, _fl(p), C.c_uint64(seed),
                                           _st()))
        del S
        o = torch.empty(l, n, e, device=dev, dtype=torch.float32)
        pa = Pd if Pd is not None else P
        gemm(pa, qkv, o, l, dh, l, l, 1, n * e3, 1, n * e, B1=n, B2=nheads, a_b=(nheads * l * l, l * l),
             b_b=(e3, dh), c_b=(e, dh), b_off=2 * e)
        ctx.dims = (l, n, e, nheads, dh, scale, p, seed)
        ctx.save_for_backward(qkv, P)
        return o

    @staticmethod
    def backward(ctx, do):
        qkv, P = ctx.saved_tensors
        l, n, e, nheads, dh, scale, p, seed = ctx.dims
        e3 = 3 * e
        do = do.contiguous()
        dev = do.device
        dqkv = torch.empty_like(qkv)
        if p > 0:
            Pd = torch.empty_like(P)
            _ck(lib().muvo_dropout(_f(P), _f(Pd), _i64(P.numel()), _fl(p), C.c_uint64(seed), _st()))
        else:
            Pd = P
        bP = (nheads * l * l, l * l)
        gemm(Pd, do, dqkv, l, dh, l, 1, l, n * e, 1, n * e3, B1=n, B2=nheads, a_b=bP, b_b=(e, dh), c_b=(e3, dh),
             c_off=2 * e)
        dPd = torch.empty_like(P)
        gemm(do, qkv, dPd, l, l, dh, n * e, 1, 1, n * e3, l, B1=n, B2=nheads, a_b=(e, dh), b_b=(e3, dh), c_b=bP,
             b_off=2 * e)
        dS = dPd
        _ck(lib().muvo_softmax_dropout_bwd(_f(P), _f(dPd), _f(dS), _i64(n * nheads * l), l, _fl(p), C.c_uint64(seed),
                                           _st()))
        gemm(dS, qkv, dqkv, l, dh, l, l, 1, n * e3, 1, n * e3, alpha=scale, B1=n, B2=nheads, a_b=bP, b_b=(e3, dh),
             c_b=(e3, dh), b_off=e)
        gemm(dS, qkv, dqkv, l, dh, l, 1, l, n * e3, 1, n * e3, alpha=scale, B1=n, B2=nheads, a_b=bP, b_b=(e3, dh),
             c_b=(e3, dh), c_off=e)
        return dqkv, None, None, None


class FlashAttentionFn(torch.autograd.Function):

    @staticmethod
    def forward(ctx, qkv, nheads, p, seed):
        qkv = qkv.contiguous()
        l, n, e3 = qkv.shape
        e = e3 // 3
        o = torch.empty(l, n, e, device=qkv.device, dtype=torch.float32)
        lse = torch.empty(n * nheads, l, device=qkv.device, dtype=torch.float32)
        _ck(lib().muvo_attention_fwd(_f(qkv), _f(o), _f(lse), l, n, nheads, e // nheads, _fl(p), C.c_uint64(seed), _st()))
        ctx.dims = (l, n, nheads, e // nheads, p, seed)
        ctx.save_for_backward(qkv, o, lse)
        return o

    @staticmethod
    def backward(ctx, do):
        qkv, o, lse = ctx.saved_tensors
        l, n, nheads, dh, p, seed = ctx.dims
        dqkv = torch.empty_like(qkv)
        _ck(lib().muvo_attention_bwd(_f(qkv), _f(o), _f(do.contiguous()), _f(lse), _f(dqkv), l, n, nheads, dh, _fl(p),
                                     C.c_uint64(seed), _st()))
        return dqkv, None, None, None


class StreamAttentionFn(torch.autograd.Function):

    @staticmethod
    def forward(ctx, qkv, nheads, p, seed):
# ... 1069 lines not shown
```

Measured before the change: 26.23.

## Fuse x-axis trilinear upsample into voxel conv forward and wgrad kernels

For decoder blocks that upsample before a 3D conv, only the y/z upsampling is materialized. The x-axis interpolation is folded into the bf16x3 voxel conv forward and weight-gradient kernels, which load the two neighbouring low-resolution x planes and blend them with 0.25/0.75 weights while staging. This avoids writing and rereading the full 2x upsampled tensor in both forward and backward. It adds extra loads per staged plane and more register pressure in the kernels, and it applies only to specific channel and Z shapes.

Measured after the change: 26.35 (median of 6 runs). About the same (+0.5%).

```diff
diff --git a/include/muvo_hip.h b/include/muvo_hip.h
--- a/include/muvo_hip.h
+++ b/include/muvo_hip.h
@@ -80,6 +80,10 @@
                              float* y, int act, float slope, double* moments, void* stream);
 int muvo_conv_wgrad_affine(const muvo_conv_desc* d, const float* x, const float* aff, const float* dy, float* dw, float* dbias,
                            void* stream);
+int muvo_conv_upx_supported(const muvo_conv_desc* d);
+int muvo_conv_forward_upx(const muvo_conv_desc* d, const float* xyz, const float* wp_fwd, const float* bias, float* y, int act,
+                          float slope, double* moments, void* stream);
+int muvo_conv_wgrad_upx(const muvo_conv_desc* d, const float* xyz, const float* dy, float* dw, float* dbias, void* stream);
 int muvo_grouped_linear_fwd(const float* x, int M, int K, int L, const float* const* W, const float* const* b, float* const* Y,
                             const int* N, void* stream);
 int muvo_grouped_linear_bwd(const float* x, int M, int K, int L, const float* const* W, float* const* dY, float* dx,
@@ -155,6 +159,8 @@
 int muvo_avgpool_bwd(const float* dy, float* dx, int64_t G, int64_t S, void* stream);
 int muvo_upsample3d_x2_fwd(const float* x, float* y, int64_t NC, int D, int H, int W, void* stream);
 int muvo_upsample3d_x2_bwd(const float* dy, float* dx, int64_t NC, int D, int H, int W, void* stream);
+int muvo_upsample3d_yz_fwd(const float* x, float* y, int64_t NC, int D, int H, int W, void* stream);
+int muvo_upsample3d_yz_bwd(const float* dy, float* dx, int64_t NC, int D, int H, int W, void* stream);
 int muvo_preprocess_image(const uint8_t* img, float* label, float* norm, int64_t NC, int C, int H, int W, int top, int left,
                           int CH, int CW, const float* mean3, const float* std3, void* stream);
 int muvo_preprocess_route(const uint8_t* img, float* norm, int64_t NC, int C, int H, int W, int OH, int OW,
diff --git a/muvo_amd/csrc/conv_gemm.hip b/muvo_amd/csrc/conv_gemm.hip
--- a/muvo_amd/csrc/conv_gemm.hip
+++ b/muvo_amd/csrc/conv_gemm.hip
@@ -1000,6 +1000,29 @@
   return vox_wgrad(d, x, dy, dw, dbias, (hipStream_t)stream, true, aff);
 }
 
+int muvo_conv_upx_supported(const muvo_conv_desc* d) {
+  if (check_desc(d)) return 0;
+  return (conv_mode() == 1 && !muvo_det() && !pw_applicable(d) && vox_fwd_ok(d) && vox_uses_bf3(d, 0) && vox_wgrad_ok(d) &&
+          vox_wgrad_uses_bf3(d) && vox_upx_shape_ok(d)) ? 1 : 0;
+}
+int muvo_conv_forward_upx(const muvo_conv_desc* d, const float* xyz, const float* wp_fwd, const float* bias, float* y, int act,
+                          float slope, double* moments, void* stream) {
+  ConvPlan pl;
+  int rc = build_plan(d, &pl);
+  if (rc) return rc;
+  MUVO_CHECK_ARG(xyz && wp_fwd && y, "conv_forward_upx: null pointer");
+  MUVO_CHECK_ARG(muvo_conv_upx_supported(d), "conv_forward_upx: shape not served by the bf16x3 voxel kernels");
+  return vox_forward_upx(d, xyz, wp_fwd, bias, y, act, slope, (hipStream_t)stream, moments);
+}
+int muvo_conv_wgrad_upx(const muvo_conv_desc* d, const float* xyz, const float* dy, float* dw, float* dbias, void* stream) {
+  ConvPlan pl;
+  int rc = build_plan(d, &pl, 0, false);
+  if (rc) return rc;
+  MUVO_CHECK_ARG(xyz && dy && dw, "conv_wgrad_upx: null pointer");
+  MUVO_CHECK_ARG(muvo_conv_upx_supported(d), "conv_wgrad_upx: shape not served by the bf16x3 voxel kernels");
+  return vox_wgrad_upx(d, xyz, dy, dw, dbias, (hipStream_t)stream);
+}
+
 int muvo_conv_dgrad(const muvo_conv_desc* d, const float* dy, const float* wp_dgrad, float* dx, void* ws, int ws_valid,
                     void* stream) {
   ConvPlan pl;
diff --git a/muvo_amd/csrc/conv_vox.h b/muvo_amd/csrc/conv_vox.h
--- a/muvo_amd/csrc/conv_vox.h
+++ b/muvo_amd/csrc/conv_vox.h
@@ -15,3 +15,7 @@
 bool vox_wgrad_ps_only(const muvo_conv_desc* d);
 int vox_wgrad(const muvo_conv_desc* d, const float* x, const float* dz, float* dw, float* dbias, hipStream_t st, bool bf3,
               const float* aff = nullptr);
+bool vox_upx_shape_ok(const muvo_conv_desc* d);
+int vox_forward_upx(const muvo_conv_desc* d, const float* xyz, const float* wp, const float* bias, float* y, int act, float slope,
+                    hipStream_t st, double* moments);
+int vox_wgrad_upx(const muvo_conv_desc* d, const float* xyz, const float* dz, float* dw, float* dbias, hipStream_t st);
diff --git a/muvo_amd/csrc/conv_vox.hip b/muvo_amd/csrc/conv_vox.hip
--- a/muvo_amd/csrc/conv_vox.hip
+++ b/muvo_amd/csrc/conv_vox.hip
@@ -11,7 +11,12 @@
   int xcd_order;
   const float* aff;
   unsigned* ticket;
+  int Xin, XYZin;
 };
+__device__ __forceinline__ int vox_upx_pair(int x, int X) {
+  const int xa = x < 0 ? 0 : (x < X ? x : X - 1);
+  return (xa + 1) >> 1;
+}
 static int vox_xcd_order() {
   static const int v = getenv("MUVO_VOX_XCD") ? atoi(getenv("MUVO_VOX_XCD")) : 1;
   return v;
@@ -506,7 +511,7 @@
 }
 
 constexpr int VOX_PS_TY = 8;
-template <int Z, int TY, bool CO8, bool GENERIC>
+template <int Z, int TY, bool CO8, bool GENERIC, bool UPX = false>
 __global__ void __launch_bounds__(64 * TY, 1)
 vox_bf3_ps_kernel(const VoxArgs a, const float* __restrict__ in, const vu32x4* __restrict__ wp, const float* __restrict__ bias,
                   float* __restrict__ out, int act, float slope, int xseg, int accum) {
@@ -537,28 +542,51 @@
   __syncthreads();
 
   float stg[TPT][8];
+  float stf[UPX ? TPT : 1][8];
   unsigned stg_ok = 0u;
   __shared__ float s_aff[2 * CK];
   if (a.aff) {
     if (tid < 2 * CK) s_aff[tid] = a.aff[(long)n * a.Cin * 2 + tid];
     __syncthreads();
   }
-  const __amdgpu_buffer_rsrc_t rs_in = __builtin_amdgcn_make_buffer_rsrc((void*)inb, 0, (int)((long)CK * a.XYZ * 4), 0x00020000);
+  const long XYZI = UPX ? a.XYZin : a.XYZ;
+  const __amdgpu_buffer_rsrc_t rs_in = __builtin_amdgcn_make_buffer_rsrc((void*)inb, 0, (int)((long)CK * XYZI * 4), 0x00020000);
   const unsigned xyz4 = (unsigned)a.XYZ * 4u;
-  auto stage_load_task = [&](int k, int x) {
+  const unsigned xyzi4 = UPX ? (unsigned)a.XYZin * 4u : xyz4;
+  auto stage_load_task = [&](int k, int x, bool first = false) {
     const int t = tid + k * 64 * TY;
     const int z = t % Z, r = (t / Z) % ROWS, cg = t / (Z * ROWS);
     const int gy = y0 - 1 + r;
     const bool ok = t < NTASK && x >= 0 && x < a.X && gy >= 0 && gy < a.Y;
     stg_ok = (stg_ok & ~(1u << k)) | ((unsigned)ok << k);
+    if constexpr (UPX) {
+      const bool rok = t < NTASK && gy >= 0 && gy < a.Y;
+      const int q = vox_upx_pair(x, a.X);
+      const int qh = q < a.Xin ? q : a.Xin - 1, ql = q > 0 ? q - 1 : 0;
+      const long base = (long)(cg * 8) * XYZI + (long)gy * Z + z;
+      if (first) {
+        const unsigned offl = rok ? (unsigned)((base + (long)ql * YZ) * 4) : 0x7fffff00u;
+#pragma unroll
+        for (int e = 0; e < 8; ++e)
+          stf[k][e] = __uint_as_float(__builtin_amdgcn_raw_buffer_load_b32(rs_in, offl + (unsigned)e * xyzi4, 0, 0));
+      } else if (x & 1) {
+#pragma unroll
+        for (int e = 0; e < 8; ++e) stf[k][e] = stg[k][e];
+      }
+      const unsigned offh = rok ? (unsigned)((base + (long)qh * YZ) * 4) : 0x7fffff00u;
+#pragma unroll
+      for (int e = 0; e < 8; ++e)
+        stg[k][e] = __uint_as_float(__builtin_amdgcn_raw_buffer_load_b32(rs_in, offh + (unsigned)e * xyzi4, 0, 0));
+    } else {
     const unsigned off = ok ? (unsigned)(((long)(cg * 8) * a.XYZ + (long)x * YZ + (long)gy * Z + z) * 4) : 0x7fffff00u;
 #pragma unroll
     for (int e = 0; e < 8; ++e)
       stg[k][e] = __uint_as_float(__builtin_amdgcn_raw_buffer_load_b32(rs_in, off + (unsigned)e * xyz4, 0, 0));
-  };
-  auto stage_load = [&](int x) {
-#pragma unroll
-    for (int k = 0; k < TPT; ++k) stage_load_task(k, x);
+    }
+  };
+  auto stage_load = [&](int x, bool first = false) {
+#pragma unroll
+    for (int k = 0; k < TPT; ++k) stage_load_task(k, x, first);
   };
   auto stage_store_task = [&](int k, int slot) {
     vu32x4* P = vsm + slot * PLANE;
@@ -575,8 +603,18 @@
         }
       }
       unsigned h[4], l[4];
+      if constexpr (UPX) {
+        float sv[8];
+        const bool ok = (stg_ok >> k) & 1u;
+        const float wlo = (slot & 1) ? 0.75f : 0.25f, whi = 1.f - wlo;
+#pragma unroll
+        for (int e = 0; e < 8; ++e) sv[e] = ok ? __builtin_fmaf(wlo, stf[k][e], whi * stg[k][e]) : 0.f;
+#pragma unroll
+        for (int q = 0; q < 4; ++q) vox_split2(sv[2 * q], sv[2 * q + 1], h[q], l[q]);
+      } else {
 #pragma unroll
       for (int q = 0; q < 4; ++q) vox_split2(stg[k][2 * q], stg[k][2 * q + 1], h[q], l[q]);
+      }
       P[(cg * ROWS + r) * COLS + z + 1] = vu32x4{h[0], h[1], h[2], h[3]};
       P[((CG + cg) * ROWS + r) * COLS + z + 1] = vu32x4{l[0], l[1], l[2], l[3]};
     }
@@ -607,7 +645,7 @@
 #pragma unroll
     for (int zt = 0; zt < ZT; ++zt) acc[j][zt] = vf32x4{0.f, 0.f, 0.f, 0.f};
 
-  stage_load(xs - 1); stage_store((xs - 1) & 1);
+  stage_load(xs - 1, true); stage_store((xs - 1) & 1);
   stage_load(xs);
   vox_dummy_stores<4 * ZT>(rs_out);
   __syncthreads();
@@ -931,7 +969,7 @@
 }
 
 constexpr int VOX_WGPS_SW = 4;
-template <int Z, int CI, bool CO8, int SW = 0>
+template <int Z, int CI, bool CO8, int SW = 0, bool UPX = false>
 __global__ void __launch_bounds__(512 + 64 * SW)
 vox_bf3_wgrad_ps_kernel(const VoxArgs a, const float* __restrict__ x, const float* __restrict__ dz, float* __restrict__ dw,
                         float* __restrict__ dbias, int xseg) {
@@ -959,7 +997,8 @@
   const int y0 = ytile * WROWS, xs = seg * xseg, xe = xs + xseg < a.X ? xs + xseg : a.X;
   const int ci0 = blockIdx.y * CI;
   const long YZ = (long)a.Y * Z;
-  const float* xb = x + (long)n * a.sN_in + (long)ci0 * a.XYZ;
+  const long XYZI = UPX ? a.XYZin : a.XYZ;
+  const float* xb = x + (long)n * a.sN_in + (long)ci0 * XYZI;
   const int co_base = blockIdx.z * 16;
   const float* db = dz + (long)n * a.sN_out;
   for (int i = tid; i < (2 * XSLOT + 64) / 16; i += NTH) ((uint4*)wsm)[i] = uint4{0u, 0u, 0u, 0u};
@@ -967,9 +1006,10 @@
 
   constexpr unsigned OOB = 0x7fffff00u;
   const int nci = a.Cin - ci0 < CI ? a.Cin - ci0 : CI;
-  const __amdgpu_buffer_rsrc_t rs_x = __builtin_amdgcn_make_buffer_rsrc((void*)xb, 0, (int)((long)nci * a.XYZ * 4), 0x00020000);
+  const __amdgpu_buffer_rsrc_t rs_x = __builtin_amdgcn_make_buffer_rsrc((void*)xb, 0, (int)((long)nci * XYZI * 4), 0x00020000);
   const __amdgpu_buffer_rsrc_t rs_d = __builtin_amdgcn_make_buffer_rsrc((void*)db, 0, (int)((long)a.Cout * a.XYZ * 4), 0x00020000);
   vu32x4 xraw[XPT][2];
+  vu32x4 xfar[UPX ? XPT : 1][2];
   unsigned xok = 0u;
   float xas[XPT], xab[XPT];
   int xlds[XPT];
@@ -985,14 +1025,24 @@
     xab[k] = have ? a.aff[((long)n * a.Cin + ci0 + ci) * 2 + 1] : 0.f;
     xlds[k] = t < XT ? ci * XCI + rr * XROW + 16 + z8 * 16 : -1;
     xrow_ok[k] = t < XT && gy >= 0 && gy < a.Y;
-    xg[k] = (long)ci * a.XYZ + (long)gy * Z + z8 * 8;
+    xg[k] = (long)ci * XYZI + (long)gy * Z + z8 * 8;
   }
   auto xload_task = [&](int k, int px) {
     const bool ok = xrow_ok[k] && px >= 0 && px < a.X;
     xok = (xok & ~(1u << k)) | ((unsigned)ok << k);
+    if constexpr (UPX) {
+      const int xn = px >> 1, xf = (px & 1) ? (xn + 1 < a.Xin ? xn + 1 : a.Xin - 1) : (xn > 0 ? xn - 1 : 0);
+      const unsigned offn = ok ? (unsigned)((xg[k] + (long)xn * YZ) * 4) : OOB;
+      const unsigned offf = ok ? (unsigned)((xg[k] + (long)xf * YZ) * 4) : OOB;
+      xraw[k][0] = __builtin_amdgcn_raw_buffer_load_b128(rs_x, offn, 0, 0);
+      xraw[k][1] = __builtin_amdgcn_raw_buffer_load_b128(rs_x, offn + 16u, 0, 0);
+      xfar[k][0] = __builtin_amdgcn_raw_buffer_load_b128(rs_x, offf, 0, 0);
+      xfar[k][1] = __builtin_amdgcn_raw_buffer_load_b128(rs_x, offf + 16u, 0, 0);
+    } else {
     const unsigned off = ok ? (unsigned)((xg[k] + (long)px * YZ) * 4) : OOB;
     xraw[k][0] = __builtin_amdgcn_raw_buffer_load_b128(rs_x, off, 0, 0);
     xraw[k][1] = __builtin_amdgcn_raw_buffer_load_b128(rs_x, off + 16u, 0, 0);
+    }
   };
   auto xload = [&](int px) {
 #pragma unroll
@@ -1013,6 +1063,12 @@
       const bool ok = (xok >> k) & 1u;
 #pragma unroll
       for (int e = 0; e < 8; ++e) v[e] = ok ? v[e] * xas[k] + xab[k] : 0.f;
+    }
+    if constexpr (UPX) {
+      const float f[8] = {__uint_as_float(xfar[k][0].x), __uint_as_float(xfar[k][0].y), __uint_as_float(xfar[k][0].z), __uint_as_float(xfar[k][0].w),
+                          __uint_as_float(xfar[k][1].x), __uint_as_float(xfar[k][1].y), __uint_as_float(xfar[k][1].z), __uint_as_float(xfar[k][1].w)};
+#pragma unroll
+      for (int e = 0; e < 8; ++e) v[e] = __builtin_fmaf(0.25f, f[e], 0.75f * v[e]);
     }
     vu32x4 h, l;
     split8(v, h, l);
@@ -1481,8 +1537,14 @@
   a.N = d->N; a.Cin = Cin; a.Cout = Cout; a.X = d->in_sz[0]; a.Y = d->in_sz[1];
   a.ytiles = cdiv(a.Y, rows);
   a.XYZ = a.X * a.Y * Z;
+  a.Xin = a.X; a.XYZin = a.XYZ;
   a.sN_in = (long)(cin_total ? cin_total : Cin) * a.XYZ; a.sN_out = (long)Cout * a.XYZ;
   return a;
+}
+static void vox_args_upx(VoxArgs& a, int cin, int Z) {
+  a.Xin = a.X / 2;
+  a.XYZin = a.Xin * a.Y * Z;
+  a.sN_in = (long)cin * a.XYZin;
 }
 
 static int vox_blocks_target(int wgrad) {
@@ -1588,6 +1650,60 @@
     MUVO_CHECK_LAUNCH("vox_bf3_ps_kernel");
     return MUVO_OK;
   });
+}
+
+bool vox_upx_shape_ok(const muvo_conv_desc* d) {
+  if (!vox_geometry_ok(d) || d->in_sz[0] % 2) return false;
+  const int Z = d->in_sz[2];
+  return (d->Cin == 16 && d->Cout == 8) || (d->Cin == 32 && d->Cout == 16 && Z == 32);
+}
+template <int Z, bool CO8>
+static int launch_vox_bf3_ps_upx(const muvo_conv_desc* d, int Cout, const float* in, const float* wp, const float* bias, float* out, int act,
+                                 float slope, hipStream_t st, int cin_total, int accum, double* moments) {
+  constexpr int TY = VOX_PS_TY;
+  VoxArgs a = vox_args(d, 16, Cout, TY, Z, cin_total, nullptr);
+  vox_args_upx(a, cin_total ? cin_total : 16, Z);
+  a.moments = moments;
+  const int xseg = vox_xseg(a, 1, 0);
+  constexpr size_t lds = (size_t)2 * 2 * 2 * (TY + 2) * (Z + 2) * 16;
+  const dim3 grid((unsigned)((long)a.N * a.ytiles * cdiv(a.X, xseg)), cdiv(Cout, 16));
+  static bool lds_raised = false;
+  if constexpr (CO8) {
+    MUVO_CHECK_ARG(!accum && act <= MUVO_ACT_LEAKY, "vox_forward_upx: activation %d not served for <= 8 produced channels", act);
+    if (int rc = vox_raise_lds(lds_raised, "vox_bf3_ps_upx", lds, vox_bf3_ps_kernel<Z, TY, true, false, true>)) return rc;
+    hipLaunchKernelGGL((vox_bf3_ps_kernel<Z, TY, true, false, true>), grid, dim3(64 * TY), lds, st, a, in, (const vu32x4*)wp, bias, out, act, slope,
+                       xseg, accum);
+    MUVO_CHECK_LAUNCH("vox_bf3_ps_kernel (upx)");
+    return MUVO_OK;
+  } else {
+    if (int rc = vox_raise_lds(lds_raised, "vox_bf3_ps_upx", lds, vox_bf3_ps_kernel<Z, TY, false, false, true>,
+                               vox_bf3_ps_kernel<Z, TY, false, true, true>)) return rc;
+    return vox_with_bool(accum || act > MUVO_ACT_LEAKY, [&](auto generic) -> int {
+      hipLaunchKernelGGL((vox_bf3_ps_kernel<Z, TY, false, decltype(generic)::value, true>), grid, dim3(64 * TY), lds, st, a, in, (const vu32x4*)wp,
+                         bias, out, act, slope, xseg, accum);
+      MUVO_CHECK_LAUNCH("vox_bf3_ps_kernel (upx)");
+      return MUVO_OK;
+    });
+  }
+}
+int vox_forward_upx(const muvo_conv_desc* d, const float* xyz, const float* wp, const float* bias, float* y, int act, float slope,
+                    hipStream_t st, double* moments) {
+  if (!vox_upx_shape_ok(d)) { muvo_set_error("vox_forward_upx: shape not served"); return MUVO_ERR_INVALID_ARG; }
+  const int Z = d->in_sz[2], Cin = d->Cin, Cout = d->Cout;
+  const long XYZin = (long)(d->in_sz[0] / 2) * d->in_sz[1] * Z;
+  if (Cout == 8) {
+    if (Z == 64) return launch_vox_bf3_ps_upx<64, true>(d, Cout, xyz, wp, bias, y, act, slope, st, 0, 0, moments);
+    return launch_vox_bf3_ps_upx<32, true>(d, Cout, xyz, wp, bias, y, act, slope, st, 0, 0, moments);
+  }
+  const size_t wstep = (size_t)cdiv(Cout, 16) * 15 * 2 * 64 * 4;
+  const int npass = Cin / 16;
+  for (int ps = 0; ps < npass; ++ps) {
+    const bool last = ps == npass - 1;
+    const int rc = launch_vox_bf3_ps_upx<32, false>(d, Cout, xyz + (size_t)ps * 16 * XYZin, wp + ps * wstep, last ? bias : nullptr, y,
+                                                    last ? act : MUVO_ACT_NONE, last ? slope : 0.f, st, Cin, ps > 0, last ? moments : nullptr);
+    if (rc) return rc;
+  }
+  return MUVO_OK;
 }
 
 static int vox_conv_dispatch(const muvo_conv_desc* d, int Cin, int Cout, const float* in, const float* wp, const float* bias,
@@ -1695,6 +1811,30 @@
   return MUVO_OK;
 }
 
+template <int Z, bool CO8>
+static int launch_vox_bf3_wgrad_ps_upx(const muvo_conv_desc* d, const float* xyz, const float* dz, float* dw, float* dbias, hipStream_t st) {
+  constexpr int CI = 16, SW = CO8 ? VOX_WGPS_SW : 0;
+  constexpr int ZH = Z / 32, WROWS = 8 / ZH, ROWS = WROWS + 2;
+  constexpr size_t lds = (size_t)2 * 2 * CI * (ROWS * (Z + 16) * 2 + 16) + 64;
+  VoxArgs a = vox_args(d, d->Cin, d->Cout, WROWS, Z, 0, nullptr);
+  vox_args_upx(a, d->Cin, Z);
+  const int xseg = vox_xseg(a, (a.Cin / CI) * cdiv(a.Cout, 16), 1);
+  static bool lds_raised = false;
+  if (int rc = vox_raise_lds(lds_raised, "vox_bf3_wgrad_ps_upx", lds, vox_bf3_wgrad_ps_kernel<Z, CI, CO8, SW, true>)) return rc;
+  dim3 grid((unsigned)((long)a.N * a.ytiles * cdiv(a.X, xseg)), a.Cin / CI, cdiv(a.Cout, 16));
+  hipLaunchKernelGGL((vox_bf3_wgrad_ps_kernel<Z, CI, CO8, SW, true>), grid, dim3(512 + 64 * SW), lds, st, a, xyz, dz, dw, dbias, xseg);
+  MUVO_CHECK_LAUNCH("vox_bf3_wgrad_ps_kernel (upx)");
+  return MUVO_OK;
+}
+int vox_wgrad_upx(const muvo_conv_desc* d, const float* xyz, const float* dz, float* dw, float* dbias, hipStream_t st) {
+  if (!vox_upx_shape_ok(d)) { muvo_set_error("vox_wgrad_upx: shape not served"); return MUVO_ERR_INVALID_ARG; }
+  if (d->Cout == 8) {
+    if (d->in_sz[2] == 64) return launch_vox_bf3_wgrad_ps_upx<64, true>(d, xyz, dz, dw, dbias, st);
+    return launch_vox_bf3_wgrad_ps_upx<32, true>(d, xyz, dz, dw, dbias, st);
+  }
+  return launch_vox_bf3_wgrad_ps_upx<32, false>(d, xyz, dz, dw, dbias, st);
+}
+
 int vox_wgrad(const muvo_conv_desc* d, const float* x, const float* dz, float* dw, float* dbias, hipStream_t st, bool bf3,
               const float* aff) {
   if (aff && !vox_affine_ok(d)) { muvo_set_error("vox_wgrad: no affine staging for this shape"); return MUVO_ERR_INVALID_ARG; }
diff --git a/muvo_amd/csrc/elementwise.hip b/muvo_amd/csrc/elementwise.hip
--- a/muvo_amd/csrc/elementwise.hip
+++ b/muvo_amd/csrc/elementwise.hip
@@ -546,6 +546,109 @@
   }
 }
 
+__device__ __forceinline__ int up2_far(int o, int n) {
+  const int i = o >> 1;
+  return (o & 1) ? (i + 1 < n ? i + 1 : n - 1) : (i > 0 ? i - 1 : 0);
+}
+__global__ void upsample3d_yz_fwd_kernel(const float* __restrict__ x, float* __restrict__ y, long NCD, int H, int W) {
+  const int OH = 2 * H, OW = 2 * W;
+  const long total = NCD * OH * OW;
+  for (long idx = (long)blockIdx.x * 256 + threadIdx.x; idx < total; idx += (long)gridDim.x * 256) {
+    const int ow = (int)(idx % OW), oh = (int)((idx / OW) % OH);
+    const long p = idx / ((long)OW * OH);
+    const float* xp = x + p * H * W;
+    const int h0 = oh >> 1, h1 = up2_far(oh, H), w0 = ow >> 1, w1 = up2_far(ow, W);
+    const float a = 0.75f * xp[h0 * W + w0] + 0.25f * xp[h1 * W + w0];
+    const float b = 0.75f * xp[h0 * W + w1] + 0.25f * xp[h1 * W + w1];
+    y[idx] = 0.75f * a + 0.25f * b;
+  }
+}
+__global__ void upsample3d_yz_bwd_kernel(const float* __restrict__ dy, float* __restrict__ dx, long NCD, int H, int W) {
+  const int OH = 2 * H, OW = 2 * W;
+  const long total = NCD * H * W;
+  for (long idx = (long)blockIdx.x * 256 + threadIdx.x; idx < total; idx += (long)gridDim.x * 256) {
+    const int w = (int)(idx % W), h = (int)((idx / W) % H);
+    const long p = idx / ((long)W * H);
+    const float* gp = dy + p * OH * OW;
+    float wa[4], wb[4];
+    up2_bwd_weights(h, H, wa);
+    up2_bwd_weights(w, W, wb);
+    float acc = 0.f;
+#pragma unroll
+    for (int ia = 0; ia < 4; ++ia) {
+      const int r = 2 * h - 1 + ia;
+      if (r < 0 || r >= OH) continue;
+      float row = 0.f;
+#pragma unroll
+      for (int ib = 0; ib < 4; ++ib) {
+        const int c = 2 * w - 1 + ib;
+        if (c >= 0 && c < OW) row += wb[ib] * gp[(long)r * OW + c];
+      }
+      acc += wa[ia] * row;
+    }
+    dx[idx] = acc;
+  }
+}
+__global__ void __launch_bounds__(256) upsample3d_yz_fwd_row_kernel(const float* __restrict__ x, float* __restrict__ y, int D,
+                                                                    int H, int W) {
+  const int OH = 2 * H, OW = 2 * W, OQ = W / 2;
+  const int idx = blockIdx.x * 256 + threadIdx.x;
+  const bool live = idx < (H + 1) * OQ;
+  const int ph = live ? idx / OQ : 0, f = live ? idx - ph * OQ : 0;
+  const long p = (long)blockIdx.z * D + blockIdx.y;
+  const int h0 = ph > 0 ? ph - 1 : 0, h1 = ph < H ? ph : H - 1;
+  const float* xp = x + p * H * W + 4 * (f >> 1);
+  const float4 r0 = *(const float4*)(xp + h0 * W), r1 = *(const float4*)(xp + h1 * W);
+  typedef float nt_f4 __attribute__((ext_vector_type(4)));
+  const bool odd = f & 1;
+#pragma unroll
+  for (int b = 0; b < 2; ++b) {
+    const float wh0 = b ? 0.25f : 0.75f, wh1 = 1.f - wh0;
+    const float cx = wh0 * r0.x + wh1 * r1.x, cy = wh0 * r0.y + wh1 * r1.y;
+    const float cz = wh0 * r0.z + wh1 * r1.z, cw = wh0 * r0.w + wh1 * r1.w;
+    const float lft = __shfl_up(cw, 1), rgt = __shfl_down(cx, 1);
+    const float q0 = odd ? cy : (f > 0 ? lft : cx);
+    const float q1 = odd ? cz : cx;
+    const float q2 = odd ? cw : cy;
+    const float q3 = odd ? (f < OQ - 1 ? rgt : cw) : cz;
+    const int oh = 2 * ph - 1 + b;
+    if (live && oh >= 0 && oh < OH) {
+      float4* yp = (float4*)(y + (p * OH + oh) * (long)OW) + f;
+      __builtin_nontemporal_store((nt_f4){0.25f * q0 + 0.75f * q1, 0.75f * q1 + 0.25f * q2, 0.25f * q1 + 0.75f * q2, 0.75f * q2 + 0.25f * q3},
+                                  (nt_f4*)yp);
+    }
+  }
+}
+__global__ void __launch_bounds__(256) upsample3d_yz_bwd_row_kernel(const float* __restrict__ dy, float* __restrict__ dx, int D,
+                                                                    int H, int W) {
+  const int OH = 2 * H, OW = 2 * W, OQ = W / 2;
+  const int f = threadIdx.x % OQ;
+  const int hr = blockIdx.x * (256 / OQ) + threadIdx.x / OQ;
+  const bool live = hr < H;
+  const int h = live ? hr : H - 1;
+  const long p = (long)blockIdx.z * D + blockIdx.y;
+  float wb[4];
+  up2_bwd_weights(h, H, wb);
+  const float w1a = f > 0 ? 0.75f : 1.f, w2b = 2 * f + 1 < W - 1 ? 0.75f : 1.f, w2a = 2 * f < W - 1 ? 0.75f : 1.f;
+  const float* gp = dy + p * OH * OW + 4 * f;
+  float2 acc = make_float2(0.f, 0.f);
+  float4 g[4];
+#pragma unroll
+  for (int ib = 0; ib < 4; ++ib) {
+    int r = 2 * h - 1 + ib;
+    r = r < 0 ? 0 : (r > OH - 1 ? OH - 1 : r);
+    g[ib] = *(const float4*)(gp + (long)r * OW);
+  }
+#pragma unroll
+  for (int ib = 0; ib < 4; ++ib) {
+    const float lft = __shfl_up(g[ib].w, 1), rgt = __shfl_down(g[ib].x, 1);
+    const float gl = f > 0 ? lft : 0.f, gr = f < OQ - 1 ? rgt : 0.f;
+    acc.x += wb[ib] * ((0.25f * gl + w1a * g[ib].x) + (w2a * g[ib].y + 0.25f * g[ib].z));
+    acc.y += wb[ib] * ((0.25f * g[ib].y + 0.75f * g[ib].z) + (w2b * g[ib].w + 0.25f * gr));
+  }
+  *((float2*)(dx + (p * H + h) * (long)W) + f) = acc;
+}
+
 __global__ void preprocess_image_kernel(const uint8_t* __restrict__ img, float* __restrict__ label,
                                         float* __restrict__ norm, long NC, int C, int H, int W, int top, int left, int CH,
                                         int CW, float m0, float m1, float m2, float s0, float s1, float s2) {
@@ -960,6 +1063,34 @@
   MUVO_CHECK_LAUNCH("upsample3d_bwd");
   return MUVO_OK;
 }
+static bool upsample3d_yz_rows(const void* a, const void* b, int64_t NC, int D, int W) {
+  const int oq = W / 2;
+  return W % 4 == 0 && oq <= 64 && (oq & (oq - 1)) == 0 && D <= 65535 && NC <= 65535 && (((uintptr_t)a | (uintptr_t)b) & 15) == 0;
+}
+int muvo_upsample3d_yz_fwd(const float* x, float* y, int64_t NC, int D, int H, int W, void* stream) {
+  MUVO_CHECK_ARG(x && y && NC > 0 && D > 0 && H > 0 && W > 0, "upsample3d_yz_fwd: bad args");
+  if (upsample3d_yz_rows(x, y, NC, D, W)) {
+    dim3 grid(cdiv((long)(H + 1) * (W / 2), 256), D, (unsigned)NC);
+    hipLaunchKernelGGL(upsample3d_yz_fwd_row_kernel, grid, dim3(256), 0, ST, x, y, D, H, W);
+    MUVO_CHECK_LAUNCH("upsample3d_yz_fwd_row");
+    return MUVO_OK;
+  }
+  hipLaunchKernelGGL(upsample3d_yz_fwd_kernel, dim3(ew_grid(NC * D * H * W * 4)), dim3(256), 0, ST, x, y, (long)NC * D, H, W);
+  MUVO_CHECK_LAUNCH("upsample3d_yz_fwd");
+  return MUVO_OK;
+}
+int muvo_upsample3d_yz_bwd(const float* dy, float* dx, int64_t NC, int D, int H, int W, void* stream) {
+  MUVO_CHECK_ARG(dy && dx && NC > 0 && D > 0 && H > 0 && W > 0, "upsample3d_yz_bwd: bad args");
+  if (upsample3d_yz_rows(dy, dx, NC, D, W)) {
+    dim3 grid(cdiv(H, 256 / (W / 2)), D, (unsigned)NC);
+    hipLaunchKernelGGL(upsample3d_yz_bwd_row_kernel, grid, dim3(256), 0, ST, dy, dx, D, H, W);
+    MUVO_CHECK_LAUNCH("upsample3d_yz_bwd_row");
+    return MUVO_OK;
+  }
+  hipLaunchKernelGGL(upsample3d_yz_bwd_kernel, dim3(ew_grid(NC * D * H * W)), dim3(256), 0, ST, dy, dx, (long)NC * D, H, W);
+  MUVO_CHECK_LAUNCH("upsample3d_yz_bwd");
+  return MUVO_OK;
+}
 int muvo_preprocess_image(const uint8_t* img, float* label, float* norm, int64_t NC, int C, int H, int W, int top, int left,
                           int CH, int CW, const float* mean3, const float* std3, void* stream) {
   MUVO_CHECK_ARG(img && norm && mean3 && std3 && C == 3, "preprocess_image: bad args");
diff --git a/muvo_amd/models/common.py b/muvo_amd/models/common.py
--- a/muvo_amd/models/common.py
+++ b/muvo_amd/models/common.py
@@ -122,9 +122,18 @@
         self.conv_act = nn.Sequential(hnn.Conv3d(in_channels, out_channels, 3, 1, 1), hnn.Placeholder())
         self.adaptive_norm = AdaptiveInstanceNorm3d(latent_n_channels, out_channels)
 
-    def forward(self, x, w, lazy=None, next_conv=None):
-        moments = ops.conv_moments_buffer(x, self.conv_act[0].geom)
-        x = self.conv_act[0](x, act=ops.ACT_LEAKY, slope=0.2, act_bwd_fused=True, moments=moments, lazy=lazy)
+    def forward(self, x, w, lazy=None, next_conv=None, upsample=False):
+        conv = self.conv_act[0]
+        if upsample and lazy is None and ops.upsample_conv3d_supported(x, conv.geom):
+            n, c, d, h, ww = x.shape
+            moments = ops.conv_moments_buffer(x, conv.geom, shape=(n, c, 2 * d, 2 * h, 2 * ww))
+            x = ops.upsample_conv3d(x, conv.weight, conv.bias, conv.geom, conv._packed, act=ops.ACT_LEAKY, slope=0.2,
+                                    act_bwd_fused=True, moments=moments)
+        else:
+            if upsample:
+                x = ops.upsample3d_x2(x)
+            moments = ops.conv_moments_buffer(x, conv.geom)
+            x = conv(x, act=ops.ACT_LEAKY, slope=0.2, act_bwd_fused=True, moments=moments, lazy=lazy)
         if next_conv is not None and ops.conv_affine_supported(x, next_conv.geom, moments):
             an = self.adaptive_norm
             y, raw, aff = ops.adain_lazy(x, _style(an, w), an.epsilon, ops.ACT_LEAKY, 0.2, moments)
@@ -237,9 +246,7 @@
         self.conv2 = ConvInstanceNorm3d(out_channels, out_channels, latent_n_channels)
 
     def forward(self, x, w, head_conv=None):
-        if self.upsample:
-            x = ops.upsample3d_x2(x)
-        y, lazy = self.conv1(x, w, next_conv=self.conv2.conv_act[0])
+        y, lazy = self.conv1(x, w, next_conv=self.conv2.conv_act[0], upsample=self.upsample)
         if head_conv is not None:
             return self.conv2.forward_with_head(y, w, head_conv, lazy=lazy)
         return self.conv2(y, w, lazy=lazy)
diff --git a/muvo_amd/ops.py b/muvo_amd/ops.py
--- a/muvo_amd/ops.py
+++ b/muvo_amd/ops.py
@@ -77,6 +77,7 @@
     'muvo_flow_epe_ws_doubles', 'muvo_flow_epe',
     'muvo_raycast_brick_words', 'muvo_raycast_bricks_grid', 'muvo_raycast_bricks_logits', 'muvo_raycast', 'muvo_panel_voxel_view',
     'muvo_ray_iou_ws_doubles', 'muvo_ray_iou_counts',
+    'muvo_upsample3d_yz_fwd', 'muvo_upsample3d_yz_bwd', 'muvo_conv_upx_supported', 'muvo_conv_forward_upx', 'muvo_conv_wgrad_upx',
 ]
 
 
@@ -1195,8 +1196,8 @@
 CONV_MOMENTS = os.environ.get('MUVO_CONV_MOMENTS', '1') != '0'
 
 
-def conv_moments_buffer(x, geom):
-    if not CONV_MOMENTS or not geom.plan_for(x).supports('muvo_conv_forward_moments_supported'):
+def conv_moments_buffer(x, geom, shape=None):
+    if not CONV_MOMENTS or not geom.plan_for(x if shape is None else shape).supports('muvo_conv_forward_moments_supported'):
         return None
     n = x.shape[0]
     cache = geom.__dict__.setdefault('_moments', {})
@@ -1822,6 +1823,79 @@
     return Upsample3dFn.apply(x)
 
 
+VOX_UPX = os.environ.get('MUVO_VOX_UPX', '1') != '0'
+
+
+class UpsampleConv3dFn(torch.autograd.Function):
+
+    @staticmethod
+    def forward(ctx, x, weight, bias, geom, packed, act, slope, act_bwd_fused, moments):
+        x = x.contiguous()
+        n, c, d, h, w = x.shape
+        plan = geom.plan(n, (2 * d, 2 * h, 2 * w))
+        L = lib()
+        uyz = torch.empty(n, c, d, 2 * h, 2 * w, device=x.device, dtype=torch.float32)
+        _ck(L.muvo_upsample3d_yz_fwd(_f(x), _f(uyz), _i64(n * c), d, h, w, _st()))
+        wp = _packed_weight(plan, packed, weight, 0)
+        y = torch.empty(plan.oshape, device=x.device, dtype=torch.float32)
+        e1 = _bracket(plan, 'fwd') if KERNEL_TIMING is not None else None
+        _ck(L.muvo_conv_forward_upx(C.byref(plan.desc), _f(uyz), _f(wp), _f(bias), _f(y), act, _fl(slope), _p(moments), _st()))
+        if e1 is not None:
+            e1.record()
+        ctx.geom, ctx.packed, ctx.act, ctx.slope = geom, packed, act, slope
+        ctx.weight, ctx.bias, ctx.low_shape = weight, bias, tuple(x.shape)
+        ctx.use_act = act != ACT_NONE and not act_bwd_fused
+        ctx.save_for_backward(uyz, y if ctx.use_act else None)
+        return y
+
+    @staticmethod
+    def backward(ctx, dy):
+        uyz, y = ctx.saved_tensors
+        n, c, d, h, w = ctx.low_shape
+        plan = ctx.geom.plan(n, (2 * d, 2 * h, 2 * w))
+        L, desc = lib(), C.byref(plan.desc)
+        if not plan.supports('muvo_conv_upx_supported'):
+            raise RuntimeError('muvo_hip: the convolution mode changed between forward and backward of upsample_conv3d')
+        dy = dy.contiguous()
+        dz = dy
+        if ctx.use_act:
+            dz = torch.empty_like(dy)
+            _ck(L.muvo_act_bwd(_f(y), _f(dy), _f(dz), _i64(dy.numel()), ctx.act, _fl(ctx.slope), _st()))
+        dx = None
+        if ctx.needs_input_grad[0]:
+            wp = _packed_weight(plan, ctx.packed, ctx.weight, 1)
+            du = torch.empty(n, c, 2 * d, 2 * h, 2 * w, device=dz.device, dtype=torch.float32)
+            e1 = _bracket(plan, 'dgrad') if KERNEL_TIMING is not None else None
+            _ck(L.muvo_conv_dgrad(desc, _f(dz), _f(wp), _f(du), _p(None), 0, _st()))
+            if e1 is not None:
+                e1.record()
+            dx = torch.empty(ctx.low_shape, device=dz.device, dtype=torch.float32)
+            _ck(L.muvo_upsample3d_x2_bwd(_f(du), _f(dx), _i64(n * c), d, h, w, _st()))
+        if ctx.weight.requires_grad:
+            bias = ctx.bias
+            gw = grad_of(ctx.weight)
+            db = grad_of(bias) if bias is not None else None
+            with _on_wgrad_stream(wgrad_stream(dz.device), dz.device, (uyz, dz)):
+                e1 = _bracket(plan, 'wgrad') if KERNEL_TIMING is not None else None
+                _ck(L.muvo_conv_wgrad_upx(desc, _f(uyz), _f(dz), _f(gw), _f(db), _st()))
+                if e1 is not None:
+                    e1.record()
+        return (dx,) + (None,) * 8
+
+
+def upsample_conv3d_supported(x, geom):
+    if not VOX_UPX or x.dim() != 5 or geom.nd != 3 or not x.is_cuda:
+        return False
+    n, _, d, h, w = x.shape
+    return geom.plan(n, (2 * d, 2 * h, 2 * w)).supports('muvo_conv_upx_supported')
+
+
+def upsample_conv3d(x, weight, bias, geom, packed, act=ACT_NONE, slope=0.0, act_bwd_fused=False, moments=None):
+    if upsample_conv3d_supported(x, geom):
+        return UpsampleConv3dFn.apply(x, weight, bias, geom, packed, act, slope, act_bwd_fused, moments)
+    return conv(upsample3d_x2(x), weight, bias, geom, packed, act, slope, act_bwd_fused, moments)
+
+
 class AttentionFn(torch.autograd.Function):
 
     @staticmethod
```
